# google/libultrahdr

Measured on AMD Instinct MI355X. Metric: Mpixels/s encode+decode (API-1 P010+YUV420, 4K), device-resident round trip, higher is better.
Workload: dtype f32; 1 GPU; API-1 3840x2160 round trip per step: encode (P010 HLG + YCbCr420 -> two-pass 3-ch gain map at scale 1, FDCT q95, Huffman: two JPEG scans) + decode (Huffman, IDCT, applyGainMap -> RGBA_F16 linear); frames resident in HBM

## Files before the change

libultrahdr_amd/csrc/api_context.cpp:

```cpp
#include "api_internal.h"

#include <sys/mman.h>
#include <mutex>
#include <algorithm>

namespace uhdr_api {
uhdr_error_info_t ensure(DeviceBuf& b, size_t bytes) {
  if (b.cap >= bytes) return ok_status();
  if (b.p) (void)hipFree(b.p);
  b.p = nullptr;
  b.cap = 0;
  size_t want = bytes + (bytes >> 3) + 256;
  HIP_TRY(hipMalloc(&b.p, want));
  b.cap = want;
  return ok_status();
}


size_t bytes_per_sample(int fmt) {
  switch (fmt) {
    case UHDR_IMG_FMT_24bppYCbCrP010:
    case UHDR_IMG_FMT_30bppYCbCr444: return 2;
    case UHDR_IMG_FMT_24bppRGB888: return 3;
    case UHDR_IMG_FMT_32bppRGBA8888:
// ... 440 lines not shown
         fmt == UHDR_IMG_FMT_32bppRGBA1010102;
}

uhdr_error_info_t validate_apply(const uhdr_raw_image_t* sdr, const uhdr_raw_image_t* gm,
                                 const uhdr_gainmap_metadata_t* md, uhdr_color_transfer_t out_ct,
                                 const uhdr_raw_image_t* dest) {
  if (dest == nullptr || dest->planes[UHDR_PLANE_PACKED] == nullptr)
    return err_status(UHDR_CODEC_INVALID_PARAM, "apply gainmap method received nullptr for destination image or plane pointer");
  if (dest->stride[UHDR_PLANE_PACKED] < dest->w)
    return err_status(UHDR_CODEC_INVALID_PARAM, "destination stride (%u) cannot be less than image width (%u)",
                      dest->stride[UHDR_PLANE_PACKED], dest->w);
  if (out_ct != UHDR_CT_LINEAR && out_ct != UHDR_CT_HLG && out_ct != UHDR_CT_PQ)
    return err_status(UHDR_CODEC_INVALID_PARAM,
                      "apply gainmap method expects output color transfer to be one of {UHDR_CT_LINEAR, UHDR_CT_HLG, UHDR_CT_PQ}. Received %d", out_ct);
  if ((out_ct == UHDR_CT_LINEAR && dest->fmt != UHDR_IMG_FMT_64bppRGBAHalfFloat) ||
      ((out_ct == UHDR_CT_HLG || out_ct == UHDR_CT_PQ) && dest->fmt != UHDR_IMG_FMT_32bppRGBA1010102))
    return err_status(UHDR_CODEC_INVALID_PARAM, "unsupported destination pixel format %d for output color transfer %d", dest->fmt, out_ct);
  UHDR_TRY(validate_metadata(md));
  if (!sdr || !gm) return err_status(UHDR_CODEC_INVALID_PARAM, "received nullptr for base image or gainmap image");
  if (sdr->fmt != UHDR_IMG_FMT_24bppYCbCr444 && sdr->fmt != UHDR_IMG_FMT_16bppYCbCr422 &&
      sdr->fmt != UHDR_IMG_FMT_12bppYCbCr420 && sdr->fmt != UHDR_IMG_FMT_24bppRGB888 &&
      sdr->fmt != UHDR_IMG_FMT_32bppRGBA8888)
    return err_status(UHDR_CODEC_UNSUPPORTED_FEATURE, "apply gainmap method expects base image color format to be one of "
                      "{UHDR_IMG_FMT_24bppYCbCr444, UHDR_IMG_FMT_16bppYCbCr422, UHDR_IMG_FMT_12bppYCbCr420, "
                      "UHDR_IMG_FMT_24bppRGB888, UHDR_IMG_FMT_32bppRGBA8888}. Received %d", sdr->fmt);
  if (gm->fmt != UHDR_IMG_FMT_8bppYCbCr400 && gm->fmt != UHDR_IMG_FMT_24bppRGB888 && gm->fmt != UHDR_IMG_FMT_32bppRGBA8888)
    return err_status(UHDR_CODEC_UNSUPPORTED_FEATURE, "apply gainmap method expects gainmap image color format to be one of "
                      "{UHDR_IMG_FMT_8bppYCbCr400, UHDR_IMG_FMT_24bppRGB888, UHDR_IMG_FMT_32bppRGBA8888}. Received %d", gm->fmt);
  return ok_status();
}

uhdr_error_info_t get_apply_tables(uhdr_hip_ctx* c, const uhdr_gainmap_metadata_t& md, float weight,
                                   int idw_scale, const float** d_out) {
  std::string key((const char*)&md, sizeof md);
  key.append((const char*)&weight, sizeof weight);
  key.append((const char*)&idw_scale, sizeof idw_scale);
  for (int i = 0; i < kTableSlots; i++)
    if (c->tab_cap[i] && c->tab_key[i] == key) { *d_out = c->d_tab[i]; return ok_status(); }
  const int slot = c->tab_next;
  c->tab_next = (c->tab_next + 1) % kTableSlots;
  std::vector<float> t;
  host::build_apply_tables(md, weight, idw_scale, &t);
  const size_t bytes = t.size() * sizeof(float);
  if (c->tab_cap[slot]) HIP_TRY(hipEventSynchronize(c->tab_ev[slot]));
  if (c->tab_cap[slot] < bytes) {
    HIP_TRY(hipStreamSynchronize(c->stream));
    if (c->h_tab[slot]) (void)hipHostFree(c->h_tab[slot]);
    if (c->d_tab[slot]) (void)hipFree(c->d_tab[slot]);
    c->h_tab[slot] = nullptr; c->d_tab[slot] = nullptr; c->tab_cap[slot] = 0;
    HIP_TRY(hipHostMalloc((void**)&c->h_tab[slot], bytes, hipHostMallocDefault));
    HIP_TRY(hipMalloc((void**)&c->d_tab[slot], bytes));
    if (!c->tab_ev[slot]) HIP_TRY(hipEventCreateWithFlags(&c->tab_ev[slot], hipEventDisableTiming));
    c->tab_cap[slot] = bytes;
  }
  memcpy(c->h_tab[slot], t.data(), bytes);
  HIP_TRY(hipMemcpyAsync(c->d_tab[slot], c->h_tab[slot], bytes, hipMemcpyHostToDevice, c->stream));
  HIP_TRY(hipEventRecord(c->tab_ev[slot], c->stream));
  c->tab_key[slot] = key;
  *d_out = c->d_tab[slot];
  return ok_status();
}
}


const char* uhdr_hip_version(void) { return "libuhdr_hip 0.3 (gfx950; reference libultrahdr 2.0.2 hot path)"; }

int uhdr_hip_device_count(void) {
  int n = 0;
  if (hipGetDeviceCount(&n) != hipSuccess) return 0;
  return n;
}

int uhdr_hip_current_device(void) {
  int d = -1;
  if (hipGetDevice(&d) != hipSuccess) return -1;
  return d;
}

uhdr_hip_ctx_t* uhdr_hip_create(int device, uhdr_error_info_t* err) {
  auto fail = [&](const char* what, hipError_t e) -> uhdr_hip_ctx_t* {
    if (err) *err = err_status(UHDR_CODEC_ERROR, "uhdr_hip_create: %s failed: %s (no CPU fallback exists behind this library)",
                               what, hipGetErrorString(e));
    return nullptr;
  };
  if (err) *err = ok_status();
  int n = 0;
  hipError_t e = hipGetDeviceCount(&n);
  if (e != hipSuccess || n == 0) return fail("hipGetDeviceCount", e == hipSuccess ? hipErrorNoDevice : e);
  if (device < 0) {
    e = hipGetDevice(&device);
    if (e != hipSuccess) return fail("hipGetDevice", e);
  }
  if (device >= n) return fail("device index", hipErrorInvalidDevice);
  e = hipSetDevice(device);
  if (e != hipSuccess) return fail("hipSetDevice", e);
  uhdr_hip_ctx* c = new uhdr_hip_ctx();
  c->device = device;
  {
    const char* e = getenv("UHDR_HIP_HUFF_TWO_PASS");
    c->huff_two_pass = e && atoi(e) != 0;
    e = getenv("UHDR_HIP_HUFF_ROUTE_LOG");
    c->huff_route_log = e && atoi(e) != 0;
  }
  e = hipStreamCreateWithFlags(&c->own_stream, hipStreamNonBlocking);
  if (e != hipSuccess) { delete c; return fail("hipStreamCreate", e); }
  c->stream = c->own_stream;
  uhdr_error_info_t st = upload_lut(&c->d_srgb, host::srgb_inv_oetf_lut(), c->stream);
  if (st.error_code != UHDR_CODEC_OK) {
    if (err) *err = st;
    (void)hipStreamDestroy(c->own_stream);
    delete c;
    return nullptr;
  }
  return c;
}

void uhdr_hip_destroy(uhdr_hip_ctx_t* c) {
  if (!c) return;
  (void)hipSetDevice(c->device);
  (void)hipStreamSynchronize(c->stream);
  for (auto& e : c->prof_entries) { (void)hipEventDestroy(e.a); (void)hipEventDestroy(e.b); }
  float* luts[] = {c->d_srgb, c->d_hlg_inv, c->d_pq_inv, c->d_hlg_oetf, c->d_pq_oetf, c->d_hlg_inv_ootf, (float*)c->d_math,
                   c->d_hlg_buckets, c->d_pq_buckets, c->d_hlg_buckets_pre, c->d_pq_buckets_pre};
  for (float* p : luts) if (p) (void)hipFree(p);
  for (int i = 0; i < kTableSlots; i++) {
    if (c->h_tab[i]) (void)hipHostFree(c->h_tab[i]);
    if (c->d_tab[i]) (void)hipFree(c->d_tab[i]);
    if (c->tab_ev[i]) (void)hipEventDestroy(c->tab_ev[i]);
  }
  for (auto& b : c->scratch) if (b.p) (void)hipFree(b.p);
  for (auto& b : c->jpg) if (b.p) (void)hipFree(b.p);
  for (auto& b : c->enc) if (b.p) (void)hipFree(b.p);
  if (c->huff_slots.p) (void)hipFree(c->huff_slots.p);
  for (auto& r : c->resident) if (r.buf.p) (void)hipFree(r.buf.p);
  if (c->pending.buf.p) (void)hipFree(c->pending.buf.p);
  if (c->pending.tmp.p) (void)hipFree(c->pending.tmp.p);
  if (c->minmax.p) (void)hipFree(c->minmax.p);
  if (c->d_coef_src) (void)hipFree(c->d_coef_src);
  if (c->d_huff) (void)hipFree(c->d_huff);
  if (c->d_srgb8) (void)hipFree(c->d_srgb8);
  for (float* q : c->d_lin10) if (q) (void)hipFree(q);
  for (auto& g : c->gain_tabs) if (g.d) (void)hipFree(g.d);
  uhdr_hip_comm_destroy(c);
  aux_worker_destroy(c);
  if (c->aux) uhdr_hip_destroy(c->aux);
  if (c->exchange.p) (void)hipFree(c->exchange.p);
  if (c->affine.p) (void)hipFree(c->affine.p);
  if (c->d_srgb_of_byte) (void)hipFree(c->d_srgb_of_byte);
  if (c->h_mm) (void)hipHostFree(c->h_mm);
  if (c->aux_ev) (void)hipEventDestroy(c->aux_ev);
  if (c->aux_ev2) (void)hipEventDestroy(c->aux_ev2);
  if (c->md_ev) (void)hipEventDestroy(c->md_ev);
  if (c->md_stream) (void)hipStreamDestroy(c->md_stream);
  if (c->h_flags) (void)hipHostFree(c->h_flags);
  if (c->pin.p) (void)hipHostFree(c->pin.p);
  if (c->pin.ev) (void)hipEventDestroy(c->pin.ev);
  if (c->huff_tabs.dev.p) (void)hipFree(c->huff_tabs.dev.p);
  if (c->own_stream) (void)hipStreamDestroy(c->own_stream);
  delete c;
}

int uhdr_hip_recycle(uhdr_hip_ctx_t* c, size_t keep_bytes) {
  if (!c) return -1;
  (void)hipSetDevice(c->device);
  (void)hipStreamSynchronize(c->stream);
  uhdr_hip_resident_forget(c);
  uhdr_hip_resident_begin(c);
  uhdr_hip_resident_end(c);
  c->sticky = ok_status();
  for (auto& h : c->huff_hint) h = uhdr_hip_ctx::HuffHint();
  c->stats = uhdr_hip_stats_t();
  c->deferred_md.valid = false;
  c->huff_slots_refused = 0;
  std::vector<DeviceBuf*> bufs;
  for (auto& b : c->scratch) bufs.push_back(&b);
  for (auto& b : c->jpg) bufs.push_back(&b);
  for (auto& b : c->enc) bufs.push_back(&b);
  bufs.push_back(&c->huff_slots);
  for (auto& r : c->resident) bufs.push_back(&r.buf);
  bufs.push_back(&c->pending.buf);
  bufs.push_back(&c->pending.tmp);
  size_t total = c->pin.cap;
  for (DeviceBuf* b : bufs) total += b->p ? b->cap : 0;
  std::sort(bufs.begin(), bufs.end(), [](const DeviceBuf* a, const DeviceBuf* b) { return (a->p ? a->cap : 0) > (b->p ? b->cap : 0); });
  for (DeviceBuf* b : bufs) {
    if (total <= keep_bytes) break;
    if (!b->p) continue;
    (void)hipFree(b->p);
    total -= b->cap;
    b->p = nullptr;
    b->cap = 0;
  }
  if (total > keep_bytes && c->pin.p) {
    if (c->pin.ev_pending && c->pin.ev) (void)hipEventSynchronize(c->pin.ev);
    (void)hipHostFree(c->pin.p);
    c->pin.p = nullptr;
    c->pin.cap = c->pin.off = 0;
    c->pin.ev_pending = false;
  }
  if (c->aux) (void)uhdr_hip_recycle(c->aux, keep_bytes);
  return c->device;
}

uhdr_error_info_t uhdr_hip_set_stream(uhdr_hip_ctx_t* c, void* hip_stream) {
  if (!c) return err_status(UHDR_CODEC_INVALID_PARAM, "received nullptr for uhdr_hip context");
  HIP_TRY(hipStreamSynchronize(c->stream));
  c->stream = hip_stream ? (hipStream_t)hip_stream : c->own_stream;
  return ok_status();
}

void* uhdr_hip_get_stream(uhdr_hip_ctx_t* c) { return c ? (void*)c->stream : nullptr; }

uhdr_error_info_t uhdr_hip_synchronize(uhdr_hip_ctx_t* c) {
  if (!c) return err_status(UHDR_CODEC_INVALID_PARAM, "received nullptr for uhdr_hip context");
  HIP_TRY(hipStreamSynchronize(c->stream));
  return ok_status();
}

void uhdr_hip_get_stats(uhdr_hip_ctx_t* c, uhdr_hip_stats_t* out) {
  if (!out) return;
  if (!c) { memset(out, 0, sizeof *out); return; }
  *out = c->stats;
}

namespace {
std::mutex g_seam_mu;
std::vector<uhdr_hip_seam_stage_t> g_seam_rows;
unsigned long long g_seam_seq = 0;
void seam_dump_at_exit() {
  const char* path = getenv("UHDR_HIP_SEAM_STATS_FILE");
  FILE* f = path ? fopen(path, "w") : nullptr;
  if (!f) return;
  std::lock_guard<std::mutex> lk(g_seam_mu);
  fprintf(f, "{");
  for (size_t i = 0; i < g_seam_rows.size(); i++) {
    const auto& r = g_seam_rows[i];
    fprintf(f, "%s\"%s\": {\"device\": %llu, \"reference\": %llu, \"device_ms\": %.3f, \"first_seq\": %llu}", i ? ", " : "", r.name, r.device_calls,
            r.reference_calls, r.device_ms, r.first_seq);
  }
  fprintf(f, "}\n");
  fclose(f);
}
}

void uhdr_hip_seam_note(const char* stage, int on_device, double ms) {
  if (!stage) return;
  static const bool dump = [] { return getenv("UHDR_HIP_SEAM_STATS_FILE") ? (atexit(seam_dump_at_exit), true) : false; }();
  (void)dump;
  std::lock_guard<std::mutex> lk(g_seam_mu);
  uhdr_hip_seam_stage_t* row = nullptr;
  for (auto& r : g_seam_rows)
    if (!strncmp(r.name, stage, sizeof r.name - 1)) { row = &r; break; }
  if (!row) {
    if (g_seam_rows.size() >= 64) return;
    uhdr_hip_seam_stage_t r;
    memset(&r, 0, sizeof r);
    strncpy(r.name, stage, sizeof r.name - 1);
    r.first_seq = g_seam_seq;
    g_seam_rows.push_back(r);
    row = &g_seam_rows.back();
  }
  g_seam_seq++;
  if (on_device) { row->device_calls++; row->device_ms += ms; }
  else row->reference_calls++;
  row->last_ms = ms;
}

int uhdr_hip_seam_stats(uhdr_hip_seam_stage_t* out, int capacity) {
  std::lock_guard<std::mutex> lk(g_seam_mu);
  const int n = (int)g_seam_rows.size();
  for (int i = 0; out && i < n && i < capacity; i++) out[i] = g_seam_rows[i];
  return n;
}

void uhdr_hip_seam_stats_reset(void) {
  std::lock_guard<std::mutex> lk(g_seam_mu);
  g_seam_rows.clear();
  g_seam_seq = 0;
}

void uhdr_hip_profile_enable(uhdr_hip_ctx_t* c, int enable) {
  if (c) c->prof = enable != 0;
}

int uhdr_hip_profile_read(uhdr_hip_ctx_t* c, const char* family, double* total_ms, int reset) {
  if (!c) return 0;
  (void)hipStreamSynchronize(c->stream);
  int n = 0;
  double tot = 0.0;
  std::vector<ProfEntry> keep;
  for (auto& e : c->prof_entries) {
    const bool match = !family || e.family == family;
    if (match) {
      float ms = 0.0f;
      if (hipEventElapsedTime(&ms, e.a, e.b) == hipSuccess) { tot += ms; n++; }
    }
    if (match && reset) { (void)hipEventDestroy(e.a); (void)hipEventDestroy(e.b); }
    else keep.push_back(e);
  }
  if (reset) c->prof_entries.swap(keep);
  if (total_ms) *total_ms = tot;
  return n;
}

void uhdr_hip_profile_mark(uhdr_hip_ctx_t* c) {
  if (!c) return;
// ... 101 lines not shown
```

libultrahdr_amd/csrc/api_entropy.cpp:

```cpp
#include "api_internal.h"

#include <condition_variable>
#include <functional>
#include <mutex>

uhdr_error_info_t uhdr_api::check_scan(const uhdr_hip_jpeg_scan_t* sc, bool need_coef, int* mcus_per_row, int* mcu_rows, int* blocks_per_mcu) {
  if (!sc) return err_status(UHDR_CODEC_INVALID_PARAM, "received nullptr for the scan description");
  if (sc->num_components != 1 && sc->num_components != 3)
    return err_status(UHDR_CODEC_INVALID_PARAM, "a scan has 1 or 3 components, received %d", sc->num_components);
  if (sc->w == 0 || sc->h == 0 || sc->w > 65535 || sc->h > 65535)
    return err_status(UHDR_CODEC_INVALID_PARAM, "image dimensions %ux%u are outside JPEG's 1..65535", sc->w, sc->h);
  int hmax = 1, vmax = 1, bpm = 0;
  for (int i = 0; i < sc->num_components; i++) {
    const int hs = sc->num_components == 1 ? 1 : sc->h_samp[i], vs = sc->num_components == 1 ? 1 : sc->v_samp[i];
    if (hs < 1 || hs > 2 || vs < 1 || vs > 2) return err_status(UHDR_CODEC_INVALID_PARAM, "component %d: sampling factors %dx%d not in {1, 2}", i, hs, vs);
    if (hs > hmax) hmax = hs;
    if (vs > vmax) vmax = vs;
    bpm += hs * vs;
    if (need_coef && (!sc->coef[i] || ((uintptr_t)sc->coef[i] & 15)))
      return err_status(UHDR_CODEC_INVALID_PARAM, "coefficient buffer %d is null or not 16-byte aligned", i);
    if (sc->blocks_w[i] < 1 || sc->blocks_h[i] < 1) return err_status(UHDR_CODEC_INVALID_PARAM, "component %d: empty block grid", i);
  }
  if (sc->num_components == 1) {
    *mcus_per_row = sc->blocks_w[0];
    *mcu_rows = sc->blocks_h[0];
    if ((unsigned)sc->blocks_w[0] != (sc->w + 7) / 8 || (unsigned)sc->blocks_h[0] != (sc->h + 7) / 8)
      return err_status(UHDR_CODEC_INVALID_PARAM, "a %dx%d block grid does not match a %ux%u image", sc->blocks_w[0], sc->blocks_h[0], sc->w, sc->h);
  } else {
    *mcus_per_row = (int)((sc->w + 8u * hmax - 1) / (8u * hmax));
    *mcu_rows = (int)((sc->h + 8u * vmax - 1) / (8u * vmax));
    for (int i = 0; i < 3; i++) {
      const unsigned cw = (sc->w * sc->h_samp[i] + hmax - 1) / hmax, chh = (sc->h * sc->v_samp[i] + vmax - 1) / vmax;
      const int min_w = (int)((cw + 7) / 8), min_h = (int)((chh + 7) / 8);
      if (sc->blocks_w[i] < min_w || sc->blocks_w[i] > *mcus_per_row * sc->h_samp[i] || sc->blocks_h[i] < min_h ||
          sc->blocks_h[i] > *mcu_rows * sc->v_samp[i])
        return err_status(UHDR_CODEC_INVALID_PARAM, "component %d: a %dx%d block grid does not match a %ux%u image at %dx%d sampling", i,
                          sc->blocks_w[i], sc->blocks_h[i], sc->w, sc->h, sc->h_samp[i], sc->v_samp[i]);
    }
  }
  *blocks_per_mcu = bpm;
  return ok_status();
}

static hipError_t wait_stream(uhdr_hip_ctx* c) {
  static const int spin_us = [] { const char* e = getenv("UHDR_HIP_SYNC_SPIN_US"); return e ? atoi(e) : 2000; }();
  if (spin_us > 0) {
    const auto t0 = std::chrono::steady_clock::now();
    for (;;) {
      const hipError_t q = hipStreamQuery(c->stream);
      if (q == hipSuccess) return hipSuccess;
      if (q != hipErrorNotReady) return q;
      if (std::chrono::steady_clock::now() - t0 > std::chrono::microseconds(spin_us)) break;
    }
  }
  return hipStreamSynchronize(c->stream);
}


uhdr_error_info_t uhdr_hip_huffman_encode_dev(uhdr_hip_ctx_t* c, const uhdr_hip_jpeg_scan_t* sc, uint8_t* out, size_t out_capacity,
                                              size_t* out_bytes) {
  if (!c) return err_status(UHDR_CODEC_INVALID_PARAM, "received nullptr for uhdr_hip context");
  if (!out || !out_bytes) return err_status(UHDR_CODEC_INVALID_PARAM, "received nullptr for the output buffer or size");
  int mpr = 0, mrows = 0, bpm = 0;
  UHDR_TRY(check_scan(sc, true, &mpr, &mrows, &bpm));
  const bool stream = sc->restart_interval == 0;
  if (!stream && (sc->restart_interval < 1 || sc->restart_interval > 65535 || sc->restart_interval * bpm > 64))
    return err_status(UHDR_CODEC_UNSUPPORTED_FEATURE, "restart_interval must be 0 (no markers) or in 1..%d for %d blocks per MCU (one wavefront "
                      "encodes one restart interval of at most 64 blocks); received %d", 64 / bpm, bpm, sc->restart_interval);
  if (stream && 2 * bpm > 64) return err_status(UHDR_CODEC_UNSUPPORTED_FEATURE, "%d blocks per MCU: outside the HIP path", bpm);
  HIP_TRY(hipSetDevice(c->device));
  if (!c->d_huff) {
    std::vector<uint32_t> blob(host::jpeg_huff_code_tables());
    blob.resize((size_t)host::kHuffTabWords + 16);
    memcpy(blob.data() + host::kHuffTabWords, host::jpeg_zigzag_to_natural(), 64);
    HIP_TRY(hipMalloc((void**)&c->d_huff, blob.size() * sizeof(uint32_t)));
    HIP_TRY(hipMemcpyAsync(c->d_huff, blob.data(), blob.size() * sizeof(uint32_t), hipMemcpyHostToDevice, c->stream));
    HIP_TRY(hipStreamSynchronize(c->stream));
  }
  HuffArgs a;
  memset(&a, 0, sizeof a);
  a.ncomp = sc->num_components;
  for (int i = 0; i < a.ncomp; i++) {
    a.coef[i] = sc->coef[i];
    a.bw[i] = sc->blocks_w[i]; a.bh[i] = sc->blocks_h[i];
    a.hs[i] = a.ncomp == 1 ? 1 : sc->h_samp[i]; a.vs[i] = a.ncomp == 1 ? 1 : sc->v_samp[i];
  }
  a.mcus_per_row = mpr;
  a.total_mcus = mpr * mrows;
  a.ri = stream ? huff_stream_segment_mcus(bpm) : sc->restart_interval;
  a.blocks_per_mcu = bpm;
  a.nseg = (a.total_mcus + a.ri - 1) / a.ri;
  a.tables = c->d_huff;
  a.zigzag = (const uint8_t*)(c->d_huff + host::kHuffTabWords);
  if (stream) {
    if (out_capacity > 0xFFFFFFF0u) out_capacity = 0xFFFFFFF0u;
    HuffStream t;
    memset(&t, 0, sizeof t);
    t.raw_words = ((uint64_t)out_capacity + 3) / 4 + 1;
    const uint64_t worst_words = (uint64_t)a.total_mcus * bpm * 52 + 2;
    if (t.raw_words > worst_words) t.raw_words = worst_words;
    const int nchunks = huff_stuff_chunks(t.raw_words * 4u);
    UHDR_TRY(ensure(c->scratch[4], (size_t)t.raw_words * 4));
    UHDR_TRY(ensure(c->scratch[5], ((size_t)a.nseg + 2) * sizeof(uint64_t) + (4 + (size_t)a.nseg + (size_t)nchunks) * sizeof(uint32_t)));
    t.raw = (uint32_t*)c->scratch[4].p;
    t.seg_start = (uint64_t*)c->scratch[5].p;
    uint64_t* d_total = t.seg_start + (size_t)a.nseg + 1;
    t.meta = (uint32_t*)(d_total + 1);
    t.seg_bits = t.meta + 4;
    uint32_t* chunk_counts = t.seg_bits + a.nseg;
    if (!c->huff_two_pass) {
      const size_t need = huff_stream_slot_bytes(a.nseg);
      if (c->huff_slots.cap >= need || !c->huff_slots_refused || need < c->huff_slots_refused) {
        if (ensure(c->huff_slots, need).error_code == UHDR_CODEC_OK) {
          t.slots = (uint32_t*)c->huff_slots.p;
        } else {
          (void)hipGetLastError();
          c->huff_slots_refused = need;
          fprintf(stderr, "uhdr_hip: no device memory for %zu bytes of Huffman segment slots: marker-less scans of that size take the two-pass route\n", need);
        }
      }
    }
    if (c->huff_route_log) fprintf(stderr, "uhdr_hip: huffman_encode stream route=%s nseg=%d\n", t.slots ? "one_walk" : "two_pass", a.nseg);
    {
      ProfScope ps(c, "huffman_encode");
      HIP_TRY(launch_huffman_encode_stream(a, t, chunk_counts, d_total, out, (uint64_t)out_capacity, c->stream));
    }
    c->stats.entropy_encode_stream++;
    if (!c->h_flags) HIP_TRY(hipHostMalloc((void**)&c->h_flags, 64 * sizeof(uint32_t), hipHostMallocDefault));
    uint32_t* hp = c->h_flags + 48;
    HIP_TRY(hipMemcpyAsync(hp, d_total, sizeof(uint64_t) + 4 * sizeof(uint32_t), hipMemcpyDeviceToHost, c->stream));
    HIP_TRY(wait_stream(c));
    uint64_t total = 0;
    uint32_t meta[4] = {0, 0, 0, 0};
    memcpy(&total, hp, sizeof total);
    memcpy(meta, hp + 2, sizeof meta);
    if (meta[2]) return err_status(UHDR_CODEC_INVALID_PARAM, "coefficients outside the baseline range (DC difference beyond 11 bits / AC beyond 10 bits)");
    const uint64_t raw_bytes = ((((uint64_t)meta[1] << 32) | meta[0]) + 7) / 8;
    if (raw_bytes > t.raw_words * 4u) total = raw_bytes + raw_bytes / 64 + 64;
    *out_bytes = (size_t)total;
    if (total > out_capacity)
      return err_status(UHDR_CODEC_MEM_ERROR, "entropy-coded data needs %llu bytes, the output buffer holds %zu", (unsigned long long)total, out_capacity);
    return ok_status();
  }
  a.slot_stride = huff_slot_stride();
  UHDR_TRY(ensure(c->scratch[4], (size_t)a.nseg * a.slot_stride));
  const size_t meta = (size_t)a.nseg * sizeof(uint32_t) + 16 + ((size_t)a.nseg + 1) * sizeof(uint64_t) + 16;
  UHDR_TRY(ensure(c->scratch[5], meta));
  a.slots = (uint8_t*)c->scratch[4].p;
  uint64_t* offsets = (uint64_t*)c->scratch[5].p;
  uint32_t* status = (uint32_t*)(offsets + (size_t)a.nseg + 1);
  a.seg_bytes = status + 2;
  {
    ProfScope ps(c, "huffman_encode");
    HIP_TRY(launch_huffman_encode(a, offsets, status, out, (uint64_t)out_capacity, c->stream));
  }
  c->stats.entropy_encode_intervals++;
  uint64_t total = 0;
  uint32_t bad = 0;
  HIP_TRY(hipMemcpyAsync(&total, offsets + a.nseg, sizeof total, hipMemcpyDeviceToHost, c->stream));
  HIP_TRY(hipMemcpyAsync(&bad, status, sizeof bad, hipMemcpyDeviceToHost, c->stream));
  HIP_TRY(wait_stream(c));
  if (bad) return err_status(UHDR_CODEC_INVALID_PARAM, "coefficients outside the baseline range (DC difference beyond 11 bits / AC beyond 10 bits)");
  *out_bytes = (size_t)total;
  if (total > out_capacity)
    return err_status(UHDR_CODEC_MEM_ERROR, "entropy-coded data needs %llu bytes, the output buffer holds %zu", (unsigned long long)total, out_capacity);
  return ok_status();
}

static bool make_dec_table(const uint8_t bits[17], const uint8_t vals[256], HuffDecTable* t) {
  memset(t, 0, sizeof *t);
  int nsym = 0;
  for (int l = 1; l <= 16; l++) nsym += bits[l];
  if (nsym > 256) return false;
  int code = 0, k = 0;
  for (int l = 1; l <= 16; l++) {
    if (bits[l]) {
      t->valoff[l] = k - code;
      for (int i = 0; i < bits[l]; i++, k++, code++) {
        if (code >= (1 << l)) return false;
        if (l <= 9) {
          const int lo = code << (9 - l);
          for (int x = 0; x < (1 << (9 - l)); x++) t->lut[lo + x] = (uint16_t)((l << 8) | vals[k]);
        }
      }
      t->maxcode[l] = code - 1;
    } else {
      t->maxcode[l] = -1;
    }
    code <<= 1;
  }
  t->maxcode[17] = 0x7fffffff;
  memcpy(t->vals, vals, 256);
  return true;
}

static bool make_fast_table(const uint8_t bits[17], const uint8_t vals[256], HuffFastTable* t, int* nsub_out = nullptr) {
  memset(t, 0, sizeof *t);
  int code = 0, k = 0, nsub = 0;
  int sub_of[512];
  for (int i = 0; i < 512; i++) sub_of[i] = -1;
  for (int l = 1; l <= 16; l++) {
    for (int i = 0; i < bits[l]; i++, k++, code++) {
      if (code >= (1 << l) || k >= 256) return false;
      if (l <= 9) {
        const int lo = code << (9 - l);
        for (int x = 0; x < (1 << (9 - l)); x++) t->l1[lo + x] = (uint16_t)((l << 8) | vals[k]);
      } else {
        const int prefix = code >> (l - 9);
// ... 1 lines not shown
          if (nsub >= kHuffL2Max) return false;
          sub_of[prefix] = nsub++;
          t->l1[prefix] = (uint16_t)(0x8000u | (unsigned)sub_of[prefix]);
        }
        const int rest = (code << (16 - l)) & 127;
        for (int x = 0; x < (1 << (16 - l)); x++) t->l2[sub_of[prefix]][rest + x] = (uint16_t)((l << 8) | vals[k]);
      }
    }
    code <<= 1;
  }
  if (nsub_out) *nsub_out = nsub;
  return true;
}

static void make_track_table(const HuffFastTable& f, bool is_dc, HuffFastTable* t) {
  auto conv = [&](uint16_t e) -> uint16_t {
    if (e & 0x8000u) return e;
    unsigned adv, kinc;
    if (e == 0) {
      adv = 16;
      kinc = is_dc ? 1 : 64;
    } else {
      const unsigned len = (e >> 8) & 31u, rs = e & 255u;
      if (is_dc) {
        const unsigned sz = rs > 15u ? 0u : rs;
        adv = len + sz;
        kinc = 1;
      } else {
        const unsigned sz = rs & 15u, run = rs >> 4;
        adv = len + sz;
        kinc = sz ? run + 1 : (run == 15u ? 16u : 64u);
      }
    }
    return (uint16_t)(adv | (kinc << 5));
  };
  for (int i = 0; i < 512; i++) t->l1[i] = conv(f.l1[i]);
  for (int s = 0; s < kHuffL2Max; s++)
    for (int i = 0; i < 128; i++) t->l2[s][i] = conv(f.l2[s][i]);
}

static void make_value_table(const HuffFastTable& f, bool is_dc, uint32_t* out ) {
  auto conv = [&](uint16_t e, bool first_level) -> uint32_t {
    if (first_level && (e & 0x8000u)) return 0x80000000u | (e & 31u);
    unsigned adv, kinc, sz = 0, bad = 0;
    if (e == 0) {
      adv = 16;
      kinc = is_dc ? 1 : 64;
      bad = 1;
    } else {
      const unsigned len = (e >> 8) & 31u, rs = e & 255u;
      if (is_dc) {
        if (rs > 15u) bad = 1; else sz = rs;
        adv = len + sz;
        kinc = 1;
      } else {
        sz = rs & 15u;
        const unsigned run = rs >> 4;
        adv = len + sz;
        kinc = sz ? run + 1 : (run == 15u ? 16u : 64u);
      }
    }
    return adv | (kinc << 5) | (sz << 12) | (bad << 16);
  };
  for (int i = 0; i < 512; i++) out[i] = conv(f.l1[i], true);
  for (int s = 0; s < kHuffL2Max; s++)
    for (int i = 0; i < 128; i++) out[512 + s * 128 + i] = conv(f.l2[s][i], false);
}

static void make_pair_table(const HuffFastTable& f, const HuffFastTable& t, const HuffFastTable& f_ac, const HuffFastTable& t_ac, int l2_base, uint32_t* out ) {
  constexpr int B = kHuffPairBits;
  for (int idx = 0; idx < kHuffPairWords; idx++) {
    const int p9 = idx >> (B - 9);
    const uint16_t e = f.l1[p9];
    uint32_t first;
    bool defined;
    if (e & 0x8000u) {
      const int sub = e & 31, rest = (idx & ((1 << (B - 9)) - 1)) << (16 - B);
      const uint16_t e2 = f.l2[sub][rest];
      if (e2 == 0 || (int)((e2 >> 8) & 31u) > B) {
        out[idx] = 0x80000000u | (uint32_t)(l2_base + sub);
        continue;
      }
      first = t.l2[sub][rest];
      defined = true;
    } else {
      first = t.l1[p9];
      defined = e != 0;
    }
    uint32_t word = first & 0xfffu;
    const int adv1 = (int)(first & 31u), kinc1 = (int)((first >> 5) & 127u);
    if (defined && kinc1 < 64 && adv1 < B) {
      const int r = B - adv1;
      const int next9 = ((idx << adv1) & (kHuffPairWords - 1)) >> (B - 9);
      const uint16_t n = f_ac.l1[next9];
      if (n != 0 && !(n & 0x8000u) && (int)((n >> 8) & 31u) <= r) {
        const uint32_t second = t_ac.l1[next9];
        word |= (second & 31u) << 12 | ((second >> 5) & 127u) << 17;
      }
    }
    out[idx] = word;
  }
}

static void make_pair_value_table(const HuffFastTable& f, const uint32_t* v, const HuffFastTable& f_ac, const uint32_t* v_ac, int l2_base, uint32_t* out ) {
  constexpr int B = kHuffPairBits;
  for (int idx = 0; idx < kHuffPairWords; idx++) {
    const int p9 = idx >> (B - 9);
    const uint16_t e = f.l1[p9];
    uint32_t first;
    bool defined;
    if (e & 0x8000u) {
      const int sub = e & 31, rest = (idx & ((1 << (B - 9)) - 1)) << (16 - B);
      const uint16_t e2 = f.l2[sub][rest];
      if (e2 == 0 || (int)((e2 >> 8) & 31u) > B) {
        out[2 * idx] = 0x80000000u | (uint32_t)(l2_base + sub);
        out[2 * idx + 1] = 0;
        continue;
      }
      first = v[512 + sub * 128 + rest];
      defined = true;
    } else {
      first = v[p9];
      defined = e != 0;
    }
    uint32_t second = 0;
    const int adv1 = (int)(first & 31u), kinc1 = (int)((first >> 5) & 127u);
    if (defined && !((first >> 16) & 1u) && kinc1 < 64 && adv1 < B) {
      const int r = B - adv1;
      const int next9 = ((idx << adv1) & (kHuffPairWords - 1)) >> (B - 9);
      const uint16_t n = f_ac.l1[next9];
      if (n != 0 && !(n & 0x8000u) && (int)((n >> 8) & 31u) <= r) second = v_ac[next9];
    }
    out[2 * idx] = first;
    out[2 * idx + 1] = second;
  }
}

uhdr_error_info_t uhdr_hip_huffman_decode_dev(uhdr_hip_ctx_t* c, const uhdr_hip_jpeg_scan_t* sc, const uhdr_hip_huff_tables_t* tables,
                                              const uint8_t* data, size_t data_bytes) {
  if (!c) return err_status(UHDR_CODEC_INVALID_PARAM, "received nullptr for uhdr_hip context");
  if (!data || data_bytes == 0 || data_bytes > 0xFFFFFFF0ull) return err_status(UHDR_CODEC_INVALID_PARAM, "received no (or more than 4 GiB of) entropy-coded data");
  int mpr = 0, mrows = 0, bpm = 0;
  UHDR_TRY(check_scan(sc, true, &mpr, &mrows, &bpm));
  if (sc->restart_interval < 0 || sc->restart_interval > 65535) return err_status(UHDR_CODEC_INVALID_PARAM, "restart_interval %d out of range", sc->restart_interval);
  HIP_TRY(hipSetDevice(c->device));
  if (!c->d_huff) {
    std::vector<uint32_t> blob(host::jpeg_huff_code_tables());
    blob.resize((size_t)host::kHuffTabWords + 16);
    memcpy(blob.data() + host::kHuffTabWords, host::jpeg_zigzag_to_natural(), 64);
    HIP_TRY(hipMalloc((void**)&c->d_huff, blob.size() * sizeof(uint32_t)));
    HIP_TRY(hipMemcpyAsync(c->d_huff, blob.data(), blob.size() * sizeof(uint32_t), hipMemcpyHostToDevice, c->stream));
    HIP_TRY(hipStreamSynchronize(c->stream));
  }
  const DbgClock dbg;
  constexpr size_t kTabDec = 0, kTabFast = (sizeof(HuffDecTable) * 4 + 255) & ~(size_t)255,
                   kTabVal = (kTabFast + sizeof(HuffFastTable) * 8 + 255) & ~(size_t)255, kTabPair = kTabVal + (size_t)4 * kHuffValWords * 4,
                   kTabPairVal = kTabPair + (size_t)kHuffPairBlobWords * 4, kTabBytes = kTabPairVal + (size_t)kHuffPairValBlobWords * 4;
  {
    uint8_t key[4 * (17 + 256)];
    for (int t = 0; t < 4; t++) {
      uint8_t* bits = key + (size_t)t * (17 + 256);
      uint8_t* vals = bits + 17;
      if (tables) {
        memcpy(bits, tables->bits[t], 17);
        memcpy(vals, tables->vals[t], 256);
      } else {
        memset(bits, 0, 17 + 256);
        host::jpeg_std_huff_table(t & 1, t >> 1, bits, vals);
      }
    }
    uhdr_hip_ctx::HuffTabCache& hc = c->huff_tabs;
    if (!hc.valid || memcmp(hc.key, key, sizeof key) != 0) {
      hc.valid = false;
      std::vector<HuffDecTable> tabs(4);
      std::vector<HuffFastTable> ftabs(8);
      std::vector<uint32_t> vtabs((size_t)4 * kHuffValWords), ptabs((size_t)kHuffPairBlobWords), pvtabs((size_t)kHuffPairValBlobWords);
      bool fast_ok = true;
      int l2_count[4] = {0, 0, 0, 0};
      for (int t = 0; t < 4; t++) {
        const uint8_t* bits = key + (size_t)t * (17 + 256);
        if (!make_dec_table(bits, bits + 17, &tabs[(size_t)t])) return err_status(UHDR_CODEC_INVALID_PARAM, "Huffman table %d is not a valid DHT table", t);
        fast_ok = make_fast_table(bits, bits + 17, &ftabs[(size_t)t], &l2_count[t]) && fast_ok;
      }
      int l2_base[4] = {0, 0, 0, 0};
      for (int t = 1; t < 4; t++) l2_base[t] = l2_base[t - 1] + l2_count[t - 1];
      if (l2_base[3] + l2_count[3] > kHuffL2Total) fast_ok = false;
      if (fast_ok)
        for (int t = 0; t < 4; t++) {
          make_track_table(ftabs[(size_t)t], (t & 1) == 0, &ftabs[(size_t)t + 4]);
          make_value_table(ftabs[(size_t)t], (t & 1) == 0, vtabs.data() + (size_t)t * kHuffValWords);
        }
      if (fast_ok)
        for (int t = 0; t < 4; t++)
        {
          make_pair_table(ftabs[(size_t)t], ftabs[(size_t)t + 4], ftabs[(size_t)(t | 1)], ftabs[(size_t)(t | 1) + 4], l2_base[t], ptabs.data() + (size_t)t * kHuffPairWords);
          make_pair_value_table(ftabs[(size_t)t], vtabs.data() + (size_t)t * kHuffValWords, ftabs[(size_t)(t | 1)], vtabs.data() + (size_t)(t | 1) * kHuffValWords,
                                l2_base[t], pvtabs.data() + (size_t)t * 2 * kHuffPairWords);
          uint16_t* l2t = (uint16_t*)(ptabs.data() + (size_t)4 * kHuffPairWords) + (size_t)l2_base[t] * 128;
          uint16_t* l2v = (uint16_t*)(pvtabs.data() + (size_t)8 * kHuffPairWords) + (size_t)l2_base[t] * 128;
          for (int i = 0; i < l2_count[t] * 128; i++) {
            l2t[i] = ftabs[(size_t)t + 4].l2[i / 128][i % 128];
            const uint32_t v = vtabs[(size_t)t * kHuffValWords + 512 + (size_t)i];
            l2v[i] = (uint16_t)(((v >> 16) & 1u) ? 0u : (v & 0xffffu));
          }
        }
      UHDR_TRY(ensure(hc.dev, kTabBytes));
      HIP_TRY(hipStreamSynchronize(c->stream));
      HIP_TRY(hipMemcpy((uint8_t*)hc.dev.p + kTabDec, tabs.data(), sizeof(HuffDecTable) * 4, hipMemcpyHostToDevice));
      HIP_TRY(hipMemcpy((uint8_t*)hc.dev.p + kTabFast, ftabs.data(), sizeof(HuffFastTable) * 8, hipMemcpyHostToDevice));
      HIP_TRY(hipMemcpy((uint8_t*)hc.dev.p + kTabVal, vtabs.data(), vtabs.size() * 4, hipMemcpyHostToDevice));
      HIP_TRY(hipMemcpy((uint8_t*)hc.dev.p + kTabPair, ptabs.data(), ptabs.size() * 4, hipMemcpyHostToDevice));
      HIP_TRY(hipMemcpy((uint8_t*)hc.dev.p + kTabPairVal, pvtabs.data(), pvtabs.size() * 4, hipMemcpyHostToDevice));
      memcpy(hc.key, key, sizeof key);
      hc.fast_ok = fast_ok;
      hc.valid = true;
    }
  }
  const bool fast_ok = c->huff_tabs.fast_ok;
  const uint8_t* tabs_dev = (const uint8_t*)c->huff_tabs.dev.p;
  if (!c->h_flags) HIP_TRY(hipHostMalloc((void**)&c->h_flags, 64 * sizeof(uint32_t), hipHostMallocDefault));
  HuffDecArgs a;
  memset(&a, 0, sizeof a);
  a.ncomp = sc->num_components;
  size_t zero_bytes[3] = {0, 0, 0};
  for (int i = 0; i < a.ncomp; i++) {
    a.coef[i] = const_cast<int16_t*>(sc->coef[i]);
    a.bw[i] = sc->blocks_w[i]; a.bh[i] = sc->blocks_h[i];
    a.hs[i] = a.ncomp == 1 ? 1 : sc->h_samp[i]; a.vs[i] = a.ncomp == 1 ? 1 : sc->v_samp[i];
    zero_bytes[i] = (size_t)a.bw[i] * a.bh[i] * 64 * sizeof(int16_t);
  }
  a.mcus_per_row = mpr;
  a.total_mcus = mpr * mrows;
  a.ri = sc->restart_interval;
  a.nseg = a.ri > 0 ? (a.total_mcus + a.ri - 1) / a.ri : 1;
  a.data = data;
  a.nbytes = (uint32_t)data_bytes;
  a.zigzag = (const uint8_t*)(c->d_huff + host::kHuffTabWords);
  const int nchunks = huff_marker_chunks(data_bytes);
  const size_t need = 16 + ((size_t)nchunks + 2 * (size_t)a.nseg) * sizeof(uint32_t);
  UHDR_TRY(ensure(c->scratch[5], need));
  uint8_t* base = (uint8_t*)c->scratch[5].p;
  a.tabs = (const HuffDecTable*)(tabs_dev + kTabDec);
  a.status = (uint32_t*)base;
  uint32_t* counts = a.status + 4;
  uint32_t* starts = counts + nchunks;
  uint32_t* ends = starts + a.nseg;
  a.starts = starts;
  a.ends = ends;
  dbg.mark("huffman_decode_dev: tables ready");
  const bool rst_sync = a.nseg > 1 && data_bytes / (size_t)a.nseg >= 320 && !getenv("UHDR_HIP_HUFF_RST_INTERVALS");
  const bool try_sync = (a.nseg == 1 || rst_sync) && data_bytes >= 4096 && data_bytes < ((size_t)1 << 29) && fast_ok && !getenv("UHDR_HIP_HUFF_SERIAL") && bpm <= 16;
  const int write_form = [] { const char* e = getenv("UHDR_HIP_HUFF_WRITE"); return e ? atoi(e) : 2; }();
  const bool form2 = try_sync && !rst_sync && write_form != 1;
  bool coef_zeroed = !form2;
  if (!form2)
    for (int i = 0; i < a.ncomp; i++) HIP_TRY(hipMemsetAsync(a.coef[i], 0, zero_bytes[i], c->stream));
  bool sync_done = false;
  if (try_sync) {
    struct Attempt { uint32_t sub_bits; int levels; };
    std::vector<Attempt> attempts;
    bool sparse = false;
    {
      const char* eb = getenv("UHDR_HIP_HUFF_SUB_BITS");
      const char* el = getenv("UHDR_HIP_HUFF_LEVELS");
      const int vb = eb ? atoi(eb) : 0;
      const bool vb_ok = vb >= 256 && vb <= 4096 && (vb & (vb - 1)) == 0;
      if (vb_ok || el) {
        const uint32_t sbits = vb_ok ? (uint32_t)vb : 1024u;
        const int lv = el ? atoi(el) : (sbits <= 512 ? 7 : 4);
        if (lv >= 1 && lv <= 15 && bpm * (lv + 1) <= kHuffHypSlots) attempts.push_back({sbits, lv});
        attempts.push_back({sbits, 0});
      } else {
        const uint64_t bits_per_block = (uint64_t)data_bytes * 8u / (uint64_t)((uint64_t)a.total_mcus * (uint64_t)bpm);
        const int lv_fit = kHuffHypSlots / bpm - 1;
        const int lv = lv_fit >= 15 ? 15 : (lv_fit >= 11 ? 11 : (lv_fit >= 7 ? 7 : (lv_fit >= 4 ? 4 : 0)));
        sparse = bits_per_block < 64;
        uint32_t first = bits_per_block < 64 ? 1024u : (bits_per_block < 200 ? 512u : (bits_per_block < 400 ? 2048u : 4096u));
        const uhdr_hip_ctx::HuffHint& hint = c->huff_hint[bpm & 15];
        if (hint.sub_bits > first && bits_per_block * 4 >= hint.bits_per_block * 3 && bits_per_block * 4 <= hint.bits_per_block * 5) first = hint.sub_bits;
        if (lv > 0)
          for (uint32_t sbits = first; sbits <= 4096u; sbits <<= 1) attempts.push_back({sbits, lv});
        attempts.push_back({1024u, 0});
      }
    }
    uint32_t sub_bits = attempts[0].sub_bits;
    bool use_hyp = false;
    for (const Attempt& t : attempts) { if (t.sub_bits < sub_bits) sub_bits = t.sub_bits; use_hyp = use_hyp || t.levels > 0; }
    const int max_rounds = 40;
    const int nch = huff_sync_chunks(data_bytes);
    const uint32_t nsub = huff_sync_max_subsequences(data_bytes, sub_bits);
    const uint32_t total_blocks = (uint32_t)a.total_mcus * (uint32_t)bpm;
    size_t off = 0;
    auto take = [&](size_t bytes) { const size_t o = off; off += (bytes + 255) & ~(size_t)255; return o; };
    const size_t rst_words = data_bytes / 32 + 2;
    const size_t o_clean = take(data_bytes + 16), o_cnt = take((size_t)nch * 4);
    const size_t o_flags = take(128), o_nblk = take((size_t)nsub * 4 + 4), o_dcd = take((size_t)total_blocks * 4), o_rm = rst_sync ? take(rst_words * 4) : 0;
    const size_t zero_bytes_sync = off - o_flags;
    const size_t o_s0 = take((size_t)nsub * 8), o_hm = use_hyp ? take((size_t)nsub * kHuffHypSlots) : 0;
    const size_t ff_bytes = off - o_s0;
    const size_t o_s1 = take((size_t)nsub * 8), o_c0 = take(nsub), o_c1 = take(nsub), o_dcp = take((size_t)((total_blocks + 255) / 256) * 12 + 16),
                 o_ft = take(sizeof(HuffFastTable) * 8),
                 o_st = take(((size_t)nsub / 2048 + 2) * 4), o_vt = take((size_t)4 * kHuffValWords * 4);
    const size_t o_hs = use_hyp ? take((size_t)nsub * kHuffHypSlots * 8) : 0, o_hc = use_hyp ? take((size_t)nsub * kHuffHypSlots * 2) : 0;
    size_t chain_tiles_off = 0;
    const size_t o_ch = use_hyp ? take(huff_hyp_chain_bytes(data_bytes, sub_bits, &chain_tiles_off)) : 0;
    (void)chain_tiles_off;
    const size_t o_ds = rst_sync ? take((size_t)a.nseg * 12) : 0, o_rp = rst_sync ? take((size_t)nch * 12) : 0;
    const size_t o_sl = use_hyp ? take((size_t)nsub * (size_t)bpm * 8) : 0;
    const int max_pieces = [&] {
      const char* e = getenv("UHDR_HIP_HUFF_PIECES");
      const int v = e ? atoi(e) : 4;
      return (use_hyp && form2 && !rst_sync && v >= 1 && v <= 4) ? v : 1;
    }();
    const size_t o_ms = max_pieces > 1 ? take((size_t)nsub * kHuffHypSlots * (size_t)(max_pieces - 1) * 8) : 0;
    const size_t o_mc = max_pieces > 1 ? take((size_t)nsub * kHuffHypSlots * (size_t)(max_pieces - 1) * 2) : 0;
    const size_t o_pe = max_pieces > 1 ? take((size_t)nsub * (size_t)max_pieces * 8 + 64) : 0;
    const size_t o_pc = max_pieces > 1 ? take(((size_t)nsub * (size_t)max_pieces + 4) * 4) : 0;
    const size_t o_st2 = max_pieces > 1 ? take(((size_t)nsub * (size_t)max_pieces / 2048 + 4) * 4) : 0;
    const size_t scan_bytes = form2 ? (size_t)total_blocks * 64 * sizeof(int16_t) : 0;
    const size_t o_cs = form2 ? take(scan_bytes + 256) : 0;
    UHDR_TRY(ensure(c->scratch[6], off));
    uint8_t* sb = (uint8_t*)c->scratch[6].p;
    HuffSyncArgs y;
    memset(&y, 0, sizeof y);
    y.clean = sb + o_clean;
    y.nbytes = (uint32_t)data_bytes;
    y.flags = (uint32_t*)(sb + o_flags);
    y.nstuffed = y.flags + 8;
    y.sub_bits = sub_bits;
    y.state[0] = (uint64_t*)(sb + o_s0); y.state[1] = (uint64_t*)(sb + o_s1);
    y.changed[0] = sb + o_c0; y.changed[1] = sb + o_c1;
    y.nblk = (uint32_t*)(sb + o_nblk);
    y.scan_tmp = (uint32_t*)(sb + o_st);
    y.dcd = (int*)(sb + o_dcd);
    y.total_blocks = total_blocks;
    y.blocks_per_mcu = bpm; y.ncomp = a.ncomp; y.mcus_per_row = a.mcus_per_row;
    uint32_t* rst_map = nullptr;
    if (rst_sync) {
      rst_map = (uint32_t*)(sb + o_rm);
      y.rst_map = rst_map;
      y.rst_blocks = (uint32_t)a.ri * (uint32_t)bpm;
      y.dc_seg = (int*)(sb + o_ds);
      y.rst_partial = (uint32_t*)(sb + o_rp);
      y.rst_chunks = (uint32_t)nch;
    }
    int j = 0;
    for (int i = 0; i < a.ncomp; i++) {
      y.bw[i] = a.bw[i]; y.bh[i] = a.bh[i]; y.hs[i] = a.hs[i]; y.vs[i] = a.vs[i]; y.coef[i] = a.coef[i];
      y.first_blk[i] = j;
      for (int k = 0; k < a.hs[i] * a.vs[i] && j < 16; k++) y.comp_of[j++] = (uint8_t)i;
    }
    y.ftabs = (const HuffFastTable*)(tabs_dev + kTabFast);
    y.ttabs = y.ftabs + 4;
    y.vtabs = (const uint32_t*)(tabs_dev + kTabVal);
    y.ptabs = (const uint32_t*)(tabs_dev + kTabPair);
    y.pvtabs = (const uint32_t*)(tabs_dev + kTabPairVal);
    y.zigzag = a.zigzag;
    (void)o_ft; (void)o_vt;
    if (use_hyp) {
      y.strag_list = (uint32_t*)(sb + o_sl);
      y.strag_cap = nsub * (uint32_t)bpm;
    }
    if (form2) y.coef_scan = (int16_t*)(sb + o_cs);
    const int main_levels_env = [&] { const char* e = getenv("UHDR_HIP_HUFF_MAIN_LEVELS"); return e ? atoi(e) : (sparse ? 1 : 2); }();
    if (j == bpm && bpm <= 16) {
      const bool fills_in_unstuff = attempts[0].levels > 0 && zero_bytes_sync % 16 == 0 && ff_bytes % 16 == 0 && zero_bytes_sync / 16 < 0xFFFFFFFFull &&
                                    ff_bytes / 16 < 0xFFFFFFFFull && !getenv("UHDR_HIP_HUFF_FILL_LAUNCHES");
      HuffInitFill init_fill;
      memset(&init_fill, 0, sizeof init_fill);
      if (fills_in_unstuff) {
        init_fill.zero_ptr = (uint4*)y.flags;
        init_fill.zero_vec = (uint32_t)(zero_bytes_sync / 16);
        init_fill.ff_ptr = (uint4*)y.state[0];
        init_fill.ff_vec = (uint32_t)(ff_bytes / 16);
      } else {
        HIP_TRY(hipMemsetAsync(y.flags, 0, zero_bytes_sync, c->stream));
      }
      auto pass0_zeroes = [&](const Attempt& t) { return form2 && t.levels > 0 && scan_bytes % 16 == 0 && scan_bytes / 16 < 0xFFFFFFFFull; };
      if (form2 && !pass0_zeroes(attempts[0])) HIP_TRY(hipMemsetAsync(y.coef_scan, 0, scan_bytes, c->stream));
      dbg.mark("huffman_decode_dev: fills enqueued");
      int final_buf = 0;
      uint32_t* fl = c->h_flags;
      for (int q = 0; q < 24; q++) fl[q] = 0;
      bool hyp_done = false, unstuffed = false, rounds_ran = false;
      auto start_over = [&](const Attempt& next) -> uhdr_error_info_t {
        HIP_TRY(hipMemsetAsync(y.flags, 0, 32, c->stream));
        HIP_TRY(hipMemsetAsync(y.flags + kHuffFlagStragglers, 0, 4, c->stream));
        HIP_TRY(hipMemsetAsync(y.nblk, 0, (size_t)nsub * 4 + 4, c->stream));
        if (form2) {
          if (!pass0_zeroes(next)) HIP_TRY(hipMemsetAsync(y.coef_scan, 0, scan_bytes, c->stream));
        } else {
          HIP_TRY(hipMemsetAsync(y.dcd, 0, (size_t)total_blocks * 4, c->stream));
          for (int i = 0; i < a.ncomp; i++) HIP_TRY(hipMemsetAsync(a.coef[i], 0, zero_bytes[i], c->stream));
        }
        return ok_status();
      };
      for (size_t ti = 0; ti < attempts.size() && !hyp_done && !rounds_ran; ti++) {
        const Attempt& t = attempts[ti];
        if (ti > 0) UHDR_TRY(start_over(t));
        y.sub_bits = t.sub_bits;
        y.zero_ptr = pass0_zeroes(t) ? (uint4*)y.coef_scan : nullptr;
        y.zero_vec = pass0_zeroes(t) ? (uint32_t)(scan_bytes / 16) : 0u;
        const uint32_t nsub_t = huff_sync_max_subsequences(data_bytes, t.sub_bits);
        if (t.levels > 0) {
          y.hyp_h = bpm;
          y.hyp_levels = t.levels;
          y.hyp_main_levels = rst_sync ? 0 : main_levels_env;
          y.strag_levels = [&] { const char* e = getenv("UHDR_HIP_HUFF_STRAG_LEVELS"); return e ? atoi(e) : t.levels; }();
          y.hyp_state = (uint64_t*)(sb + o_hs);
          y.hyp_map = sb + o_hm;
          y.hyp_cnt = (uint16_t*)(sb + o_hc);
          y.hyp_hist = getenv("UHDR_HIP_HUFF_DEBUG") ? 1 : 0;
          {
            int q = t.sub_bits >= 1024u ? (int)(t.sub_bits / 256u) : 1;
            if (getenv("UHDR_HIP_HUFF_PIECES_ALL")) q = (int)(t.sub_bits / 256u);
            if (q > max_pieces) q = max_pieces;
            if (q < 1) q = 1;
            while (q > 1 && (t.sub_bits % (uint32_t)q || (t.sub_bits / (uint32_t)q) % 32u)) q--;
            if (q == 3) q = 2;
            if (getenv("UHDR_HIP_HUFF_QMERGE") && atoi(getenv("UHDR_HIP_HUFF_QMERGE")) == 0) q = 1;
            y.pieces = q;
            y.mid_state = q > 1 ? (uint64_t*)(sb + o_ms) : nullptr;
            y.mid_cnt = q > 1 ? (uint16_t*)(sb + o_mc) : nullptr;
            y.pend = q > 1 ? (uint64_t*)(sb + o_pe) : nullptr;
            y.pcnt = q > 1 ? (uint32_t*)(sb + o_pc) : nullptr;
            y.scan_tmp = q > 1 ? (uint32_t*)(sb + o_st2) : (uint32_t*)(sb + o_st);
          }
          if (!(fills_in_unstuff && ti == 0)) HIP_TRY(hipMemsetAsync(y.state[0], 0xff, ff_bytes, c->stream));
          size_t tiles_off = 0;
          (void)huff_hyp_chain_bytes(data_bytes, t.sub_bits, &tiles_off);
          {
            ProfScope ps(c, "huffman_decode");
            if (!unstuffed)
              HIP_TRY(launch_huffman_unstuff(data, (uint32_t)data_bytes, (uint32_t*)(sb + o_cnt), y.flags + 8, sb + o_clean, c->stream, rst_map, y.rst_partial,
                                             fills_in_unstuff && ti == 0 ? &init_fill : nullptr));
            unstuffed = true;
            HIP_TRY(launch_huffman_decode_hyp(y, (int*)(sb + o_dcp), sb + o_ch, sb + o_ch + tiles_off, c->stream));
          }
          dbg.mark("huffman_decode_dev: hypothesis attempt enqueued");
          HIP_TRY(hipMemcpyAsync(fl, y.flags, 24 * sizeof(uint32_t), hipMemcpyDeviceToHost, c->stream));
          HIP_TRY(wait_stream(c));
          dbg.mark("huffman_decode_dev: hypothesis attempt finished");
          hyp_done = fl[2] == 0;
          if (hyp_done && ti > 0) {
            uhdr_hip_ctx::HuffHint& hint = c->huff_hint[bpm & 15];
            hint.sub_bits = t.sub_bits;
            hint.bits_per_block = (uint32_t)((uint64_t)data_bytes * 8u / ((uint64_t)a.total_mcus * (uint64_t)bpm));
          }
          if (getenv("UHDR_HIP_HUFF_DEBUG")) {
            uint32_t hist[32] = {};
            (void)hipMemcpy(hist, y.flags, sizeof hist, hipMemcpyDeviceToHost);
            fprintf(stderr, "uhdr_hip: hypothesis decode of %zu bytes, %u subsequences of %u bits x %d: merges per level %u %u %u %u %u %u+, %u paths unmerged after %d levels (%d in lockstep, %u paths handed to the straggler waves), true path %s\n",
                    data_bytes, nsub_t, t.sub_bits, bpm, hist[10], hist[11], hist[12], hist[13], hist[14], hist[15], fl[3], t.levels, y.hyp_main_levels, fl[kHuffFlagStragglers], hyp_done ? "resolved" : "LOST (next attempt)");
            fprintf(stderr, "uhdr_hip: the stragglers' merges at level 2 .. 10, 11+: %u %u %u %u %u %u %u %u %u %u\n", hist[22], hist[23], hist[24], hist[25], hist[26], hist[27], hist[28], hist[29],
                    hist[30], hist[31]);
          }
        } else {
          y.pieces = 1;
          y.scan_tmp = (uint32_t*)(sb + o_st);
          {
            ProfScope ps(c, "huffman_decode");
            if (!unstuffed) HIP_TRY(launch_huffman_unstuff(data, (uint32_t)data_bytes, (uint32_t*)(sb + o_cnt), y.flags + 8, sb + o_clean, c->stream, rst_map, y.rst_partial));
            unstuffed = true;
            HIP_TRY(launch_huffman_decode_sync(y, max_rounds, (int*)(sb + o_dcp), &final_buf, c->stream));
          }
          HIP_TRY(hipMemcpyAsync(fl, y.flags, 24 * sizeof(uint32_t), hipMemcpyDeviceToHost, c->stream));
          HIP_TRY(wait_stream(c));
          rounds_ran = true;
        }
      }
      const bool settled = hyp_done || fl[4 + max_rounds % 3] == 0;
      if (rst_sync && getenv("UHDR_HIP_HUFF_DEBUG"))
        fprintf(stderr, "uhdr_hip: restart file through the parallel decoder: %s, status bits %#x, %u markers dropped (%d expected), sequence sums %s\n",
                settled ? "settled" : "NOT settled", fl[1], fl[9], a.nseg - 1, fl[0] == fl[16] && fl[7] == fl[17] ? "equal" : "DIFFERENT");
      if (settled && rst_sync && ((fl[1] & 14u) != 0 || fl[9] != (uint32_t)(a.nseg - 1) || fl[0] != fl[16] || fl[7] != fl[17])) {
        for (int i = 0; i < a.ncomp; i++) HIP_TRY(hipMemsetAsync(a.coef[i], 0, zero_bytes[i], c->stream));
        coef_zeroed = true;
      } else if (settled) {
        if (fl[1] & 8u) return err_status(UHDR_CODEC_INVALID_PARAM, "corrupt entropy-coded data (the scan ends before its last block)");
        if (fl[1] & 2u) return err_status(UHDR_CODEC_INVALID_PARAM, "corrupt entropy-coded data (undefined Huffman code or a run past the end of a block)");
        sync_done = true;
      } else {
        if (a.nseg == 1 && !c->huff_serial_ok && data_bytes > (256u << 10)) {
          c->stats.entropy_decode_declined++;
          return err_status(UHDR_CODEC_UNSUPPORTED_FEATURE, "the parallel entropy decode did not settle in %d rounds; %zu bytes on one lane would take longer than the CPU", max_rounds, data_bytes);
        }
        for (int i = 0; i < a.ncomp; i++) HIP_TRY(hipMemsetAsync(a.coef[i], 0, zero_bytes[i], c->stream));
        coef_zeroed = true;
      }
    }
  }
  if (sync_done) {
    c->stats.entropy_decode_parallel++;
    return ok_status();
  }
  if (a.nseg == 1 && !c->huff_serial_ok && data_bytes > (256u << 10)) {
    c->stats.entropy_decode_declined++;
    return err_status(UHDR_CODEC_UNSUPPORTED_FEATURE, "a %zu-byte scan without restart markers that the parallel decoder does not take (Huffman tables outside its two-level form)", data_bytes);
  }
  if (!coef_zeroed)
    for (int i = 0; i < a.ncomp; i++) HIP_TRY(hipMemsetAsync(a.coef[i], 0, zero_bytes[i], c->stream));
  HIP_TRY(hipMemsetAsync(a.status, 0, 16, c->stream));
  {
    ProfScope ps(c, "huffman_decode");
    HIP_TRY(launch_huffman_decode(a, counts, starts, ends, c->stream));
  }
  if (a.nseg == 1) c->stats.entropy_decode_single_lane++;
  else c->stats.entropy_decode_intervals++;
  uint32_t st[2] = {0, 0};
  HIP_TRY(hipMemcpyAsync(st, a.status, sizeof st, hipMemcpyDeviceToHost, c->stream));
  HIP_TRY(wait_stream(c));
  if (st[1] != (uint32_t)(a.nseg - 1))
    return err_status(UHDR_CODEC_INVALID_PARAM, "found %u restart markers, a restart interval of %d MCUs over %d MCUs needs %d", st[1], a.ri,
                      a.total_mcus, a.nseg - 1);
  if (st[0] & 4u) return err_status(UHDR_CODEC_INVALID_PARAM, "restart markers out of sequence");
  if (st[0] & 2u) return err_status(UHDR_CODEC_INVALID_PARAM, "corrupt entropy-coded data (undefined Huffman code or a run past the end of a block)");
  return ok_status();
}

uhdr_error_info_t uhdr_api::aux_context(uhdr_hip_ctx* c, uhdr_hip_ctx** out) {
  if (!c->aux) {
    uhdr_error_info_t e = ok_status();
    c->aux = uhdr_hip_create(c->device, &e);
    if (!c->aux) return e.error_code != UHDR_CODEC_OK ? e : err_status(UHDR_CODEC_ERROR, "could not create the auxiliary context");
  }
  c->aux->prof = c->prof;
  c->aux->huff_serial_ok = c->huff_serial_ok;
  c->aux->huff_route_log = c->huff_route_log;
  c->aux->huff_two_pass = c->huff_two_pass;
  *out = c->aux;
  return ok_status();
}
void uhdr_api::aux_merge(uhdr_hip_ctx* c) {
  if (!c->aux) return;
  uhdr_hip_ctx* x = c->aux;
  c->stats.entropy_decode_parallel += x->stats.entropy_decode_parallel;
  c->stats.entropy_decode_intervals += x->stats.entropy_decode_intervals;
  c->stats.entropy_decode_single_lane += x->stats.entropy_decode_single_lane;
  c->stats.entropy_decode_declined += x->stats.entropy_decode_declined;
  c->stats.entropy_encode_stream += x->stats.entropy_encode_stream;
  c->stats.entropy_encode_intervals += x->stats.entropy_encode_intervals;
  x->stats = uhdr_hip_stats_t();
  for (auto& e : x->prof_entries) c->prof_entries.push_back(e);
  x->prof_entries.clear();
}

struct AuxWorker {
  static constexpr int kSpinUs = 300;
  std::thread th;
  std::mutex mu;
  std::condition_variable cv;
  std::function<void()> job;
  std::atomic<int> state{0};
  std::atomic<bool> busy{false};
  static bool spin_until(const std::function<bool()>& pred, int us) {
    const auto t0 = std::chrono::steady_clock::now();
    while (!pred()) {
      if (std::chrono::steady_clock::now() - t0 > std::chrono::microseconds(us)) return pred();
#if defined(__x86_64__)
      __builtin_ia32_pause();
#endif
    }
    return true;
  }
  AuxWorker() {
    th = std::thread([this] {
      for (;;) {
        if (!spin_until([this] { return state.load(std::memory_order_acquire) != 0; }, kSpinUs)) {
          std::unique_lock<std::mutex> lk(mu);
          cv.wait(lk, [this] { return state.load(std::memory_order_acquire) != 0; });
        }
        if (state.load(std::memory_order_acquire) == 2) return;
        std::function<void()> j;
        {
          std::lock_guard<std::mutex> lk(mu);
          j = std::move(job);
          state.store(0, std::memory_order_release);
        }
        j();
        {
          std::lock_guard<std::mutex> lk(mu);
          busy.store(false, std::memory_order_release);
        }
        cv.notify_all();
      }
    });
  }
  void run(std::function<void()> j) {
    {
      std::lock_guard<std::mutex> lk(mu);
      job = std::move(j);
      busy.store(true, std::memory_order_release);
      state.store(1, std::memory_order_release);
    }
    cv.notify_all();
  }
  void wait() {
    if (spin_until([this] { return !busy.load(std::memory_order_acquire); }, kSpinUs)) return;
    std::unique_lock<std::mutex> lk(mu);
    cv.wait(lk, [this] { return !busy.load(std::memory_order_acquire); });
  }
  ~AuxWorker() {
    {
      std::lock_guard<std::mutex> lk(mu);
      state.store(2, std::memory_order_release);
    }
    cv.notify_all();
    if (th.joinable()) th.join();
  }
};
void aux_worker_destroy(uhdr_hip_ctx* c) {
  if (c && c->aux_worker) {
    delete c->aux_worker;
    c->aux_worker = nullptr;
  }
}
bool uhdr_api::aux_post(uhdr_hip_ctx* c, std::function<void()> job) {
  static const bool no_thread = getenv("UHDR_HIP_NO_AUX_THREAD") != nullptr;
  if (no_thread) return false;
  if (!c->aux_worker) {
    try {
      c->aux_worker = new AuxWorker();
    } catch (...) {
      c->aux_worker = nullptr;
    }
  }
  if (!c->aux_worker) return false;
  c->aux_worker->run(std::move(job));
  return true;
}
void uhdr_api::aux_wait(uhdr_hip_ctx* c) {
  if (c->aux_worker) c->aux_worker->wait();
}
namespace {
template <typename FA, typename FB>
void run_pair(uhdr_hip_ctx* c, FA&& job_a, FB&& job_b) {
  static const bool no_thread = getenv("UHDR_HIP_NO_AUX_THREAD") != nullptr;
  if (!c->aux_worker && !no_thread) {
    try {
      c->aux_worker = new AuxWorker();
    } catch (...) {
      c->aux_worker = nullptr;
    }
  }
  if (c->aux_worker) {
    c->aux_worker->run(job_b);
    job_a();
    c->aux_worker->wait();
  } else {
    job_a();
    job_b();
  }
}
}

uhdr_error_info_t uhdr_hip_huffman_encode2_dev(uhdr_hip_ctx_t* c, const uhdr_hip_jpeg_scan_t* scan_a, uint8_t* out_a, size_t cap_a, size_t* bytes_a,
                                               const uhdr_hip_jpeg_scan_t* scan_b, uint8_t* out_b, size_t cap_b, size_t* bytes_b) {
  if (!c) return err_status(UHDR_CODEC_INVALID_PARAM, "received nullptr for uhdr_hip context");
  HIP_TRY(hipSetDevice(c->device));
  uhdr_hip_ctx* x = nullptr;
  UHDR_TRY(aux_context(c, &x));
  if (!c->aux_ev) HIP_TRY(hipEventCreateWithFlags(&c->aux_ev, hipEventDisableTiming));
  HIP_TRY(hipEventRecord(c->aux_ev, c->stream));
  HIP_TRY(hipStreamWaitEvent(x->stream, c->aux_ev, 0));
  uhdr_error_info_t ra = ok_status(), rb = ok_status();
  const int dev = c->device;
  run_pair(c, [&] { ra = uhdr_hip_huffman_encode_dev(c, scan_a, out_a, cap_a, bytes_a); },
           [&, dev] { (void)hipSetDevice(dev); rb = uhdr_hip_huffman_encode_dev(x, scan_b, out_b, cap_b, bytes_b); });
  aux_merge(c);
  return ra.error_code != UHDR_CODEC_OK ? ra : rb;
}

uhdr_error_info_t uhdr_hip_huffman_decode2_dev(uhdr_hip_ctx_t* c, const uhdr_hip_jpeg_scan_t* scan_a, const uhdr_hip_huff_tables_t* tables_a, const uint8_t* data_a,
                                               size_t bytes_a, const uhdr_hip_jpeg_scan_t* scan_b, const uhdr_hip_huff_tables_t* tables_b,
                                               const uint8_t* data_b, size_t bytes_b) {
  if (!c) return err_status(UHDR_CODEC_INVALID_PARAM, "received nullptr for uhdr_hip context");
  HIP_TRY(hipSetDevice(c->device));
  uhdr_hip_ctx* x = nullptr;
  UHDR_TRY(aux_context(c, &x));
  if (!c->aux_ev) HIP_TRY(hipEventCreateWithFlags(&c->aux_ev, hipEventDisableTiming));
  HIP_TRY(hipEventRecord(c->aux_ev, c->stream));
  HIP_TRY(hipStreamWaitEvent(x->stream, c->aux_ev, 0));
// ... 8 lines not shown
```

libultrahdr_amd/csrc/api_internal.h:

```cpp
#ifndef UHDR_HIP_API_INTERNAL_H
#define UHDR_HIP_API_INTERNAL_H

#pragma GCC visibility push(default)
#include "uhdr_hip.h"
#pragma GCC visibility pop

#include <cfloat>
#include <chrono>
#include <cmath>
#include <cstdarg>
#include <cstdio>
#include <cstring>
#include <atomic>
#include <functional>
#include <map>
#include <memory>
#include <string>
#include <thread>
#include <vector>
#include "exact_math.h"
#include "host_tables.h"
#include "uhdr_types.h"
#include "rccl_bind.h"

using namespace uhdr;

inline uhdr_error_info_t ok_status() {
  uhdr_error_info_t s;
  s.error_code = UHDR_CODEC_OK;
  s.has_detail = 0;
  s.detail[0] = 0;
  return s;
}
inline uhdr_error_info_t err_status(uhdr_codec_err_t code, const char* fmt, ...) {
  uhdr_error_info_t s;
  s.error_code = code;
  s.has_detail = 1;
  va_list ap;
  va_start(ap, fmt);
  vsnprintf(s.detail, sizeof s.detail, fmt, ap);
  va_end(ap);
  return s;
}
#define HIP_TRY(expr)                                                                      \
  do {                                                                                     \
    hipError_t e_ = (expr);                                                                \
    if (e_ != hipSuccess)                                                                  \
      return err_status(e_ == hipErrorOutOfMemory ? UHDR_CODEC_MEM_ERROR : UHDR_CODEC_ERROR, \
                        "HIP error '%s' at %s:%d", hipGetErrorString(e_), __FILE__, __LINE__); \
  } while (0)
#define UHDR_TRY(expr)                                 \
  do {                                                 \
    uhdr_error_info_t s_ = (expr);                     \
    if (s_.error_code != UHDR_CODEC_OK) return s_;     \
  } while (0)

struct DbgClock {
  bool on;
  std::chrono::steady_clock::time_point t0;
  DbgClock() : on(getenv("UHDR_HIP_CLOCK_DEBUG") != nullptr), t0(std::chrono::steady_clock::now()) {}
  void mark(const char* what) const {
    if (on) fprintf(stderr, "uhdr_hip:   [%7.1f us] %s\n", std::chrono::duration<double, std::micro>(std::chrono::steady_clock::now() - t0).count(), what);
  }
};

struct ProfEntry {
  hipEvent_t a, b;
  std::string family;
};

constexpr int kTableSlots = 4;

struct DeviceBuf {
  void* p = nullptr;
  size_t cap = 0;
};

struct uhdr_hip_ctx {
  int device = 0;
  hipStream_t own_stream = nullptr;
  hipStream_t stream = nullptr;
  float* d_srgb = nullptr;
  float* d_hlg_inv = nullptr;
  float* d_pq_inv = nullptr;
  float* d_hlg_oetf = nullptr;
  float* d_pq_oetf = nullptr;
  float* d_hlg_buckets = nullptr;
  float* d_pq_buckets = nullptr;
  float* d_hlg_buckets_pre = nullptr;
  float* d_pq_buckets_pre = nullptr;
  float* d_hlg_inv_ootf = nullptr;
  double* d_math = nullptr;
  float* h_tab[kTableSlots] = {};
  float* d_tab[kTableSlots] = {};
  size_t tab_cap[kTableSlots] = {};
  hipEvent_t tab_ev[kTableSlots] = {};
  std::string tab_key[kTableSlots];
  int tab_next = 0;
  DeviceBuf scratch[8];
  uhdr_hip_stats_t stats = {};
  bool huff_serial_ok = true;
  DeviceBuf huff_slots;
  bool huff_two_pass = false;
  bool huff_route_log = false;
  size_t huff_slots_refused = 0;
  DeviceBuf enc[3];
  uhdr_hip_ctx* aux = nullptr;
  struct AuxWorker* aux_worker = nullptr;
  DeviceBuf jpg[6];
  struct Resident {
    DeviceBuf buf;
    bool valid = false;
    uhdr_img_fmt_t fmt = UHDR_IMG_FMT_UNSPECIFIED;
    unsigned int w = 0, h = 0;
    const void* host[3] = {};
    unsigned int host_stride[3] = {};
    size_t off[3] = {};
    unsigned int dev_stride[3] = {};
    unsigned int prows[3] = {}, pcols[3] = {};
    bool host_unwritten = false;
    bool adopted = false;
    void* adopt_dst = nullptr;
    unsigned int adopt_stride = 0, adopt_w = 0, adopt_h = 0;
    bool adopt_expand = false;
  } resident[2];
  struct HuffHint { uint32_t sub_bits = 0, bits_per_block = 0; } huff_hint[16];
  struct HuffTabCache {
    bool valid = false, fast_ok = false;
    uint8_t key[4 * (17 + 256)] = {};
    DeviceBuf dev;
  } huff_tabs;
  struct PinArena {
    void* p = nullptr;
    size_t cap = 0, off = 0;
    hipEvent_t ev = nullptr;
    bool ev_pending = false;
  } pin;
  uint32_t* h_flags = nullptr;
  bool resident_on = false;
  bool resident_lazy = false;
  uhdr_error_info_t sticky = {};
  unsigned int resident_next = 0;
  struct PendingCopy {
    DeviceBuf buf;
    bool on = false;
    size_t off = 0, pitch = 0, dst_pitch = 0;
    unsigned int w = 0, h = 0, bps = 0;
    bool expand = false;
    void* dst = nullptr;
    DeviceBuf tmp;
  } pending;
  struct MallEntry { const void* p; uint64_t stamp; };
  std::vector<MallEntry> mall;
  uint64_t mall_clock = 0;
  DeviceBuf minmax;
  uint32_t* d_huff = nullptr;
  CoefSrc* d_coef_src = nullptr;
  unsigned int coef_src_next = 0;
  CoefSrc* coef_src_last_slot = nullptr;
  std::vector<uint8_t> coef_src_last;
  float* d_srgb8 = nullptr;
  StepTab srgb8_meta = {};
  float* d_lin10[5] = {};
  struct GainTab { float mn, mx; float* d; StepTab meta; };
  std::vector<GainTab> gain_tabs;
  void* comm = nullptr;
  int comm_rank = 0, comm_size = 0;
  bool comm_custom = false;
  uhdr_hip_comm_ops_t comm_ops = {};
  DeviceBuf exchange;
  DeviceBuf affine;
  float* d_srgb_of_byte = nullptr;
  float* h_mm = nullptr;
  bool defer_md = false;
  hipStream_t md_stream = nullptr;
  hipEvent_t md_ev = nullptr;
  std::function<void()> on_side_launched;
  bool side_job_posted = false;
  struct DeferredMd { bool valid = false, run = false; uhdr_hip_encode_cfg_t cfg; uhdr_color_transfer_t hdr_ct; int use_base_cg = 1; } deferred_md;
  hipEvent_t aux_ev = nullptr;
  hipEvent_t aux_ev2 = nullptr;
  bool prof = false;
  std::vector<ProfEntry> prof_entries;
};

struct ProfScope {
  uhdr_hip_ctx* c;
  ProfEntry e;
  bool on;
  ProfScope(uhdr_hip_ctx* ctx, const char* family) : c(ctx), on(ctx->prof) {
    if (!on) return;
    e.family = family;
    if (hipEventCreate(&e.a) != hipSuccess || hipEventCreate(&e.b) != hipSuccess) { on = false; return; }
    (void)hipEventRecord(e.a, c->stream);
  }
  ~ProfScope() {
    if (!on) return;
    (void)hipEventRecord(e.b, c->stream);
    c->prof_entries.push_back(e);
  }
};

namespace uhdr_api {
uhdr_error_info_t ensure(DeviceBuf& b, size_t bytes);
size_t bytes_per_sample(int fmt);
bool plane_geom(const uhdr_raw_image_t* im, int pl, size_t* rows, size_t* width);
size_t plane_bytes(const uhdr_raw_image_t* im, int pl);
uhdr_error_info_t validate_image(const uhdr_raw_image_t* im, const char* what);
ImageView view_of(const uhdr_raw_image_t* im);
ImageViewMut view_mut_of(const uhdr_raw_image_t* im);
uhdr_error_info_t adopted_copy_out(uhdr_hip_ctx* c, const void* src, size_t src_pitch, unsigned int bps, bool expand, unsigned int w, unsigned int h,
                                   void* dst, size_t dst_pitch);
uhdr_error_info_t resident_write_back(uhdr_hip_ctx* c, uhdr_hip_ctx::Resident& r);
uhdr_error_info_t resident_write_back_all(uhdr_hip_ctx* c);
void resident_retire(uhdr_hip_ctx* c, uhdr_hip_ctx::Resident& r, bool host_is_rewritten);
void resident_drop(uhdr_hip_ctx* c, const void* host_plane);
uhdr_error_info_t fast_h2d(uhdr_hip_ctx* c, void* dst, const void* src, size_t bytes);
uhdr_error_info_t stage_in(uhdr_hip_ctx* c, int slot, const uhdr_raw_image_t* host, uhdr_raw_image_t* dev, bool upload);
bool resident_keeps(int fmt);
uhdr_error_info_t resident_keep(uhdr_hip_ctx* c, const uhdr_raw_image_t* dev, const uhdr_raw_image_t* host, bool host_unwritten = false);
uhdr_error_info_t stage_out(uhdr_hip_ctx* c, const uhdr_raw_image_t* dev, uhdr_raw_image_t* host);
uhdr_error_info_t upload_lut(float** dst, const std::vector<float>& src, hipStream_t s);
uhdr_error_info_t upload_math(uhdr_hip_ctx* c);
uhdr_error_info_t upload_step_table(const host::OetfBuckets& b, float** slot, StepTab* meta, hipStream_t s);
uhdr_error_info_t gain_step_table(uhdr_hip_ctx* c, const GenParams& p, StepTab* out);
uhdr_error_info_t select_hdr_lut(uhdr_hip_ctx* c, uhdr_color_transfer_t ct, const float** lut, int* n);
uhdr_error_info_t validate_metadata(const uhdr_gainmap_metadata_t* m);
bool is_rgb_fmt_host(int fmt);
uhdr_error_info_t validate_apply(const uhdr_raw_image_t* sdr, const uhdr_raw_image_t* gm, const uhdr_gainmap_metadata_t* md, uhdr_color_transfer_t out_ct,
                                 const uhdr_raw_image_t* dest);
uhdr_error_info_t get_apply_tables(uhdr_hip_ctx* c, const uhdr_gainmap_metadata_t& md, float weight, int idw_scale, const float** d_out);
uhdr_error_info_t fill_gen_params(uhdr_hip_ctx* c, const uhdr_raw_image_t* sdr, const uhdr_raw_image_t* hdr, const uhdr_hip_encode_cfg_t* cfg, GenParams* p,
                                  int* use_base_cg, float* hdr_white_nits_out, bool sdr_in_registers = false);
void fill_finalize(MinmaxTableParams* t, const uhdr_hip_encode_cfg_t* cfg);
void fill_gainmap_desc(const uhdr_raw_image_t* hdr, const GenParams& p, uhdr_raw_image_t* gm);
uhdr_error_info_t generate_gainmap_finalize_md(const uhdr_hip_encode_cfg_t* cfg, uhdr_color_transfer_t hdr_ct, int use_base_cg, const float mm[6], uhdr_gainmap_metadata_t* md);
void note_table_stats(uhdr_hip_ctx* c, const uhdr_hip_encode_cfg_t* cfg);
uhdr_error_info_t two_pass_tail(uhdr_hip_ctx* c, const GenParams& p, int n_partials, const uhdr_hip_encode_cfg_t* cfg, uhdr_raw_image_t* gm);
uhdr_error_info_t fill_tone_map_params(uhdr_hip_ctx* c, const uhdr_raw_image_t* hdr, ToneMapParams* pp);
uhdr_error_info_t comm_all_reduce_min(uhdr_hip_ctx* c, float* buf, size_t n);
uhdr_error_info_t check_scan(const uhdr_hip_jpeg_scan_t* sc, bool need_coef, int* mcus_per_row, int* mcu_rows, int* blocks_per_mcu);
uhdr_error_info_t aux_context(uhdr_hip_ctx* c, uhdr_hip_ctx** out);
void aux_merge(uhdr_hip_ctx* c);
bool aux_post(uhdr_hip_ctx* c, std::function<void()> job);
void aux_wait(uhdr_hip_ctx* c);
}
using namespace uhdr_api;

void aux_worker_destroy(uhdr_hip_ctx* c);

#endif
```

libultrahdr_amd/csrc/api_jpeg.cpp:

```cpp
#include "api_internal.h"

void uhdr_hip_jpeg_quant_table(int quality, int is_chroma, uint16_t qt[64]) { host::jpeg_quant_table(quality, is_chroma, qt); }

int uhdr_hip_oetf_code_thresholds(uhdr_color_transfer_t ct, float thresholds[1024]) {
  if ((ct != UHDR_CT_HLG && ct != UHDR_CT_PQ) || !thresholds) return -1;
  const std::vector<float>& t = host::oetf_code_thresholds(ct);
  for (int i = 0; i < 1024; i++) thresholds[i] = t[(size_t)i];
  return 0;
}

uhdr_error_info_t uhdr_hip_selftest(uhdr_hip_ctx_t* c, int which, unsigned int arg0, unsigned int arg1, unsigned int seed, const float mm[6],
                                    unsigned long long out[8]) {
  if (!c) return err_status(UHDR_CODEC_INVALID_PARAM, "received nullptr for uhdr_hip context");
  if (!out || which < 0 || which > 4 || (which == 4 && (!mm || arg0 > 2 || arg1 < 1 || arg1 > 3 || arg0 >= arg1)) || (which == 2 && (arg0 < 1 || arg1 > 254 || arg0 > arg1)))
    return err_status(UHDR_CODEC_INVALID_PARAM, "bad self-test arguments");
  HIP_TRY(hipSetDevice(c->device));
  UHDR_TRY(upload_math(c));
  UHDR_TRY(ensure(c->affine, kAffineDevBytes));
  UHDR_TRY(ensure(c->exchange, 256));
  unsigned long long* d_out = (unsigned long long*)c->exchange.p;
  HIP_TRY(hipMemsetAsync(d_out, 0, 64, c->stream));
  if (which == 4) {
    MinmaxTableParams t;
    memset(&t, 0, sizeof t);
// ... 988 lines not shown
    rgb.w = sc.w;
    rgb.h = sc.h;
    const size_t pitch_px = ((size_t)sc.w + 63) & ~(size_t)63;
    UHDR_TRY(ensure(*out_buf, pitch_px * (size_t)out_channels * sc.h));
    rgb.planes[0] = out_buf->p;
    rgb.stride[0] = (unsigned int)pitch_px;
    UHDR_TRY(uhdr_hip_idct_dequant_rgb_dev(c, sc.coef[0], sc.coef[1], sc.coef[2], sc.blocks_w[0], sc.blocks_h[0], hdr->qtable[0], hdr->qtable[1], variant, &rgb));
    if (!lazy)
      HIP_TRY(hipMemcpy2DAsync(planes[0], (size_t)hstride[0] * out_channels, out_buf->p, pitch_px * out_channels, (size_t)sc.w * out_channels, sc.h,
                               hipMemcpyDeviceToHost, c->stream));
    if (res) {
      res->fmt = rgb.fmt; res->w = sc.w; res->h = sc.h;
      res->host[0] = planes[0]; res->host_stride[0] = hstride[0]; res->off[0] = 0; res->dev_stride[0] = (unsigned int)pitch_px;
      res->prows[0] = sc.h; res->pcols[0] = sc.w;
      res->valid = true;
      res->host_unwritten = lazy;
    }
  }
  if (lazy) c->stats.lazy_downloads_skipped++;
  dbg.mark("jpeg_decode_scan: IDCT (and download) enqueued");
  if (!lazy) HIP_TRY(hipStreamSynchronize(c->stream));
  dbg.mark("jpeg_decode_scan: done");
  return ok_status();
}

static bool is_420(const uhdr_hip_jpeg_scan_t& sc) {
  return sc.num_components == 3 && sc.h_samp[0] == 2 && sc.v_samp[0] == 2 && sc.h_samp[1] == 1 && sc.v_samp[1] == 1 && sc.h_samp[2] == 1 &&
         sc.v_samp[2] == 1;
}

static uhdr_error_info_t idct_upsample_rgb_impl(uhdr_hip_ctx_t* c, const int16_t* const coef[3], const int bw[3], const int bh[3],
                                                const uint16_t* const qt[3], int variant, uhdr_raw_image_t* rgb) {
  if (bw[1] != bw[2] || bh[1] != bh[2]) return err_status(UHDR_CODEC_UNSUPPORTED_FEATURE, "Cb and Cr block grids differ");
  for (int k = 0; k < 3; k++)
    for (int i = 0; i < 64; i++)
      if (qt[k][i] == 0) return err_status(UHDR_CODEC_INVALID_PARAM, "quantization table %d entry %d is zero", k, i);
  uint8_t* scratch = nullptr;
  if (variant == 0) {
    UHDR_TRY(ensure(c->jpg[5], upsample420_scratch_bytes(bw, bh)));
    scratch = (uint8_t*)c->jpg[5].p;
  }
  rgb->range = UHDR_CR_FULL_RANGE;
  ProfScope ps(c, "idct_upsample_rgb");
  HIP_TRY(launch_idct_upsample_rgb(coef, bw, bh, qt, variant, view_mut_of(rgb), scratch, c->stream));
  return ok_status();
}

uhdr_error_info_t uhdr_hip_idct_upsample_rgb_dev(uhdr_hip_ctx_t* c, const int16_t* coef_y, const int16_t* coef_cb, const int16_t* coef_cr,
                                                 unsigned int w, unsigned int h, const uint16_t qt_y[64], const uint16_t qt_cb[64],
                                                 const uint16_t qt_cr[64], int variant, uhdr_raw_image_t* rgb) {
  if (!c) return err_status(UHDR_CODEC_INVALID_PARAM, "received nullptr for uhdr_hip context");
  if (!coef_y || !coef_cb || !coef_cr || !qt_y || !qt_cb || !qt_cr || !rgb || !rgb->planes[0])
    return err_status(UHDR_CODEC_INVALID_PARAM, "received bad argument for idct_upsample_rgb");
  if (rgb->fmt != UHDR_IMG_FMT_24bppRGB888 && rgb->fmt != UHDR_IMG_FMT_32bppRGBA8888)
    return err_status(UHDR_CODEC_UNSUPPORTED_FEATURE, "idct_upsample_rgb expects UHDR_IMG_FMT_24bppRGB888 or UHDR_IMG_FMT_32bppRGBA8888. Received %d", rgb->fmt);
  if (variant != 0 && variant != 1) return err_status(UHDR_CODEC_INVALID_PARAM, "unknown libjpeg variant %d", variant);
  if (w == 0 || h == 0 || w > 65535 || h > 65535) return err_status(UHDR_CODEC_INVALID_PARAM, "image dimensions %ux%u are outside JPEG's 1..65535", w, h);
  if (rgb->w != w || rgb->h != h) return err_status(UHDR_CODEC_INVALID_PARAM, "destination is %ux%u, the image %ux%u", rgb->w, rgb->h, w, h);
  if (rgb->stride[0] < w) return err_status(UHDR_CODEC_INVALID_PARAM, "stride (%u) cannot be less than width (%u)", rgb->stride[0], w);
  if (((uintptr_t)coef_y | (uintptr_t)coef_cb | (uintptr_t)coef_cr) & 15)
    return err_status(UHDR_CODEC_INVALID_PARAM, "coefficient buffers must be 16-byte aligned");
  HIP_TRY(hipSetDevice(c->device));
  const int16_t* coef[3] = {coef_y, coef_cb, coef_cr};
  const int bw[3] = {(int)((w + 7) / 8), (int)((w + 15) / 16), (int)((w + 15) / 16)};
  const int bh[3] = {(int)((h + 7) / 8), (int)((h + 15) / 16), (int)((h + 15) / 16)};
  const uint16_t* qt[3] = {qt_y, qt_cb, qt_cr};
  return idct_upsample_rgb_impl(c, coef, bw, bh, qt, variant, rgb);
}

static uhdr_error_info_t jpeg_decode_rgb_impl(uhdr_hip_ctx_t* c, const uhdr_hip_jpeg_header_t* hdr, const uint8_t* scan_data, size_t scan_bytes,
                                              int out_channels, int variant, uint8_t* rgb, unsigned int stride_px) {
  if (!c) return err_status(UHDR_CODEC_INVALID_PARAM, "received nullptr for uhdr_hip context");
  if (!hdr || !scan_data || !rgb) return err_status(UHDR_CODEC_INVALID_PARAM, "received nullptr argument for jpeg_decode_rgb");
  if (out_channels != 3 && out_channels != 4) return err_status(UHDR_CODEC_INVALID_PARAM, "out_channels is 3 (RGB888) or 4 (RGBA8888), received %d", out_channels);
  if (variant != 0 && variant != 1) return err_status(UHDR_CODEC_INVALID_PARAM, "unknown libjpeg variant %d", variant);
  uhdr_hip_jpeg_scan_t sc = hdr->scan;
  int mpr = 0, mrows = 0, bpm = 0;
  UHDR_TRY(check_scan(&sc, false, &mpr, &mrows, &bpm));
  if (stride_px < sc.w) return err_status(UHDR_CODEC_INVALID_PARAM, "stride (%u) cannot be less than width (%u)", stride_px, sc.w);
  const bool s444 = sc.num_components == 3 && sc.h_samp[0] == 1 && sc.v_samp[0] == 1 && sc.h_samp[1] == 1 && sc.v_samp[1] == 1 &&
                    sc.h_samp[2] == 1 && sc.v_samp[2] == 1;
  if (s444) {
    uint8_t* planes[3] = {rgb, nullptr, nullptr};
    const unsigned int hs[3] = {stride_px, 0, 0}, vs[3] = {sc.h, 0, 0};
    return jpeg_decode_scan_impl(c, hdr, scan_data, scan_bytes, out_channels, variant, planes, hs, vs);
  }
  if (!is_420(sc))
    return err_status(UHDR_CODEC_UNSUPPORTED_FEATURE, "RGB output on the device takes 4:2:0 or 4:4:4 files; received %d components at %dx%d / %dx%d / %dx%d",
                      sc.num_components, sc.h_samp[0], sc.v_samp[0], sc.h_samp[1], sc.v_samp[1], sc.h_samp[2], sc.v_samp[2]);
  if (sc.blocks_w[1] != sc.blocks_w[2] || sc.blocks_h[1] != sc.blocks_h[2]) return err_status(UHDR_CODEC_UNSUPPORTED_FEATURE, "Cb and Cr block grids differ");
  const DbgClock dbg;
  UHDR_TRY(jpeg_scan_to_coefficients(c, hdr, scan_data, scan_bytes, dbg, sc));
  resident_drop(c, rgb);
  uhdr_raw_image_t img;
  memset(&img, 0, sizeof img);
  img.fmt = out_channels == 3 ? UHDR_IMG_FMT_24bppRGB888 : UHDR_IMG_FMT_32bppRGBA8888;
  img.w = sc.w;
  img.h = sc.h;
  const size_t pitch_px = ((size_t)sc.w + 63) & ~(size_t)63;
  UHDR_TRY(ensure(c->jpg[4], pitch_px * (size_t)out_channels * sc.h));
  img.planes[0] = c->jpg[4].p;
  img.stride[0] = (unsigned int)pitch_px;
  const uint16_t* qt[3] = {hdr->qtable[0], hdr->qtable[1], hdr->qtable[2]};
  UHDR_TRY(idct_upsample_rgb_impl(c, sc.coef, sc.blocks_w, sc.blocks_h, qt, variant, &img));
  HIP_TRY(hipMemcpy2DAsync(rgb, (size_t)stride_px * out_channels, c->jpg[4].p, pitch_px * out_channels, (size_t)sc.w * out_channels, sc.h,
                           hipMemcpyDeviceToHost, c->stream));
  HIP_TRY(hipStreamSynchronize(c->stream));
  dbg.mark("jpeg_decode_rgb: done");
  return ok_status();
}

uhdr_error_info_t uhdr_hip_jpeg_decode_rgb(uhdr_hip_ctx_t* c, const uhdr_hip_jpeg_header_t* hdr, const uint8_t* scan_data, size_t scan_bytes,
                                           int out_channels, int variant, uint8_t* rgb, unsigned int stride_px) {
  const auto t0 = std::chrono::steady_clock::now();
  const uhdr_error_info_t r = jpeg_decode_rgb_impl(c, hdr, scan_data, scan_bytes, out_channels, variant, rgb, stride_px);
  if (c) c->stats.last_jpeg_decode_rgb_ns = (unsigned long long)std::chrono::duration_cast<std::chrono::nanoseconds>(std::chrono::steady_clock::now() - t0).count();
  return r;
}

uhdr_error_info_t uhdr_hip_decode_api1_scans_dev(uhdr_hip_ctx_t* c, const uhdr_hip_jpeg_header_t* base, const uint8_t* base_data, size_t base_bytes,
                                                 uhdr_color_gamut_t base_cg, const uhdr_hip_jpeg_header_t* map, const uint8_t* map_data, size_t map_bytes,
                                                 uhdr_color_gamut_t map_cg, int libjpeg_variant, const uhdr_gainmap_metadata_t* md,
                                                 uhdr_color_transfer_t output_ct, uhdr_img_fmt_t output_format, float max_display_boost,
                                                 uhdr_raw_image_t* dest) {
  if (!c) return err_status(UHDR_CODEC_INVALID_PARAM, "received nullptr for uhdr_hip context");
  if (!base || !base_data || !map || !map_data || !md || !dest) return err_status(UHDR_CODEC_INVALID_PARAM, "received nullptr argument for decode_api1_scans");
  if (libjpeg_variant != 0 && libjpeg_variant != 1) return err_status(UHDR_CODEC_INVALID_PARAM, "unknown libjpeg variant %d", libjpeg_variant);
  uhdr_hip_jpeg_scan_t sb = base->scan, sm = map->scan;
  int mpr = 0, mrows = 0, bpm = 0;
  UHDR_TRY(check_scan(&sb, false, &mpr, &mrows, &bpm));
  if (sb.num_components != 3 || sb.h_samp[0] != 2 || sb.v_samp[0] != 2 || sb.h_samp[1] != 1 || sb.v_samp[1] != 1 || sb.h_samp[2] != 1 || sb.v_samp[2] != 1)
    return err_status(UHDR_CODEC_UNSUPPORTED_FEATURE, "decode_api1_scans takes a 4:2:0 base image (the form JpegR writes); decode the scans with uhdr_hip_jpeg_decode_scan");
  UHDR_TRY(check_scan(&sm, false, &mpr, &mrows, &bpm));
  const int nm = sm.num_components;
  if (nm == 3 && (bpm != 3 || memcmp(map->qtable[1], map->qtable[2], sizeof map->qtable[1])))
    return err_status(UHDR_CODEC_UNSUPPORTED_FEATURE, "a three-channel gain map is a 4:4:4 scan with one chroma quantization table here");
  if (base_bytes == 0 || map_bytes == 0 || base_bytes > 0xFFFFFFF0ull || map_bytes > 0xFFFFFFF0ull) return err_status(UHDR_CODEC_INVALID_PARAM, "received no (or too much) entropy-coded data");
  HIP_TRY(hipSetDevice(c->device));
  for (int i = 0; i < 3; i++) {
    UHDR_TRY(ensure(c->jpg[1 + i], (size_t)sb.blocks_w[i] * sb.blocks_h[i] * 128));
    sb.coef[i] = (const int16_t*)c->jpg[1 + i].p;
  }
  size_t off = 0, o_map[3] = {0, 0, 0};
  for (int i = 0; i < nm; i++) { o_map[i] = off; off += ((size_t)sm.blocks_w[i] * sm.blocks_h[i] * 128 + 255) & ~(size_t)255; }
  UHDR_TRY(ensure(c->enc[0], off));
  for (int i = 0; i < nm; i++) sm.coef[i] = (const int16_t*)((const uint8_t*)c->enc[0].p + o_map[i]);
  c->huff_serial_ok = false;
  auto tables_of = [](const uhdr_hip_jpeg_header_t* h) -> const uhdr_hip_huff_tables_t* {
    for (int t = 0; t < 4; t++)
      for (int l = 0; l < 17; l++)
        if (h->tables.bits[t][l]) return &h->tables;
    return nullptr;
  };
  const uhdr_error_info_t hs = uhdr_hip_huffman_decode2_dev(c, &sb, tables_of(base), base_data, base_bytes, &sm, tables_of(map), map_data, map_bytes);
  c->huff_serial_ok = true;
  if (hs.error_code != UHDR_CODEC_OK) return hs;
  uhdr_raw_image_t gm;
  memset(&gm, 0, sizeof gm);
  gm.cg = map_cg;
  gm.ct = UHDR_CT_UNSPECIFIED;
  gm.range = UHDR_CR_FULL_RANGE;
  gm.w = sm.w;
  gm.h = sm.h;
  const size_t pitch_px = ((size_t)sm.w + 63) & ~(size_t)63;
  if (nm == 3) {
    gm.fmt = UHDR_IMG_FMT_32bppRGBA8888;
    UHDR_TRY(ensure(c->jpg[4], pitch_px * 4 * sm.h));
    gm.planes[0] = c->jpg[4].p;
    gm.stride[0] = (unsigned int)pitch_px;
    UHDR_TRY(uhdr_hip_idct_dequant_rgb_dev(c, sm.coef[0], sm.coef[1], sm.coef[2], sm.blocks_w[0], sm.blocks_h[0], map->qtable[0], map->qtable[1], libjpeg_variant, &gm));
  } else {
    gm.fmt = UHDR_IMG_FMT_8bppYCbCr400;
    const size_t pitch = ((size_t)sm.blocks_w[0] * 8 + 63) & ~(size_t)63;
    UHDR_TRY(ensure(c->jpg[4], pitch * (size_t)sm.blocks_h[0] * 8));
    gm.planes[0] = c->jpg[4].p;
    gm.stride[0] = (unsigned int)pitch;
    UHDR_TRY(uhdr_hip_idct_dequant_dev(c, sm.coef[0], sm.blocks_w[0], sm.blocks_h[0], map->qtable[0], (uint8_t*)c->jpg[4].p, pitch));
  }
  uhdr_hip_jpeg_coefficients_t bc;
  memset(&bc, 0, sizeof bc);
  for (int i = 0; i < 3; i++) {
    bc.coef[i] = sb.coef[i];
    bc.blocks_w[i] = sb.blocks_w[i];
    bc.blocks_h[i] = sb.blocks_h[i];
    memcpy(bc.qtable[i], base->qtable[i], sizeof bc.qtable[i]);
  }
  uhdr_error_info_t ap = uhdr_hip_apply_gainmap_coef_dev(c, &bc, sb.w, sb.h, base_cg, &gm, md, output_ct, output_format, max_display_boost, dest);
  if (ap.error_code != UHDR_CODEC_UNSUPPORTED_FEATURE) return ap;
  size_t ppitch[3], poff[3], total = 0;
  for (int i = 0; i < 3; i++) {
    ppitch[i] = ((size_t)sb.blocks_w[i] * 8 + 63) & ~(size_t)63;
    poff[i] = total;
    total += ppitch[i] * (size_t)sb.blocks_h[i] * 8;
  }
  UHDR_TRY(ensure(c->jpg[0], total));
  uhdr_raw_image_t bi;
  memset(&bi, 0, sizeof bi);
  bi.fmt = UHDR_IMG_FMT_12bppYCbCr420;
  bi.cg = base_cg;
  bi.ct = UHDR_CT_SRGB;
  bi.range = UHDR_CR_FULL_RANGE;
  bi.w = sb.w;
  bi.h = sb.h;
  for (int i = 0; i < 3; i++) {
    uint8_t* d = (uint8_t*)c->jpg[0].p + poff[i];
    UHDR_TRY(uhdr_hip_idct_dequant_dev(c, sb.coef[i], sb.blocks_w[i], sb.blocks_h[i], base->qtable[i], d, ppitch[i]));
    bi.planes[i] = d;
    bi.stride[i] = (unsigned int)ppitch[i];
  }
  return uhdr_hip_apply_gainmap_dev(c, &bi, &gm, md, output_ct, output_format, max_display_boost, dest, 0, 0);
}

size_t uhdr_hip_jpeg_assemble(const uhdr_hip_jpeg_scan_t* sc, const uint16_t qt_luma[64], const uint16_t qt_chroma[64], const uint8_t* scan_data,
                              size_t scan_bytes, uint8_t* out, size_t cap) {
  int mpr = 0, mrows = 0, bpm = 0;
  if (check_scan(sc, false, &mpr, &mrows, &bpm).error_code != UHDR_CODEC_OK || !qt_luma || !scan_data || !out) return 0;
  if (sc->num_components > 1 && !qt_chroma) return 0;
  const int nc = sc->num_components, ntab = nc > 1 ? 2 : 1;
  const uint8_t* zz = host::jpeg_zigzag_to_natural();
  std::vector<uint8_t> v;
  v.reserve(scan_bytes + 1024);
  auto put = [&](unsigned b) { v.push_back((uint8_t)b); };
  auto put16 = [&](unsigned x) { put(x >> 8); put(x & 0xff); };
  put(0xff); put(0xd8);
  put(0xff); put(0xe0); put16(16); for (char ch : {'J', 'F', 'I', 'F'}) put((unsigned char)ch); put(0); put(1); put(1); put(0); put16(1); put16(1); put(0); put(0);
  for (int t = 0; t < ntab; t++) {
    const uint16_t* q = t ? qt_chroma : qt_luma;
    put(0xff); put(0xdb); put16(67); put(t);
    for (int i = 0; i < 64; i++) {
      if (q[zz[i]] == 0 || q[zz[i]] > 255) return 0;
      put(q[zz[i]]);
    }
  }
  put(0xff); put(0xc0); put16(8 + 3 * nc); put(8); put16(sc->h); put16(sc->w); put(nc);
  for (int i = 0; i < nc; i++) { put(i + 1); put(((nc == 1 ? 1 : sc->h_samp[i]) << 4) | (nc == 1 ? 1 : sc->v_samp[i])); put(i ? 1 : 0); }
  for (int t = 0; t < ntab; t++) {
    for (int ac = 0; ac < 2; ac++) {
      uint8_t bits[17], vals[256];
      const int nv = host::jpeg_std_huff_table(ac, t, bits, vals);
      put(0xff); put(0xc4); put16(2 + 1 + 16 + nv); put((ac << 4) | t);
      for (int i = 1; i <= 16; i++) put(bits[i]);
      for (int i = 0; i < nv; i++) put(vals[i]);
    }
  }
  if (sc->restart_interval > 0) { put(0xff); put(0xdd); put16(4); put16((unsigned)sc->restart_interval); }
  put(0xff); put(0xda); put16(6 + 2 * nc); put(nc);
  for (int i = 0; i < nc; i++) { put(i + 1); put(i ? 0x11 : 0x00); }
  put(0); put(63); put(0);
  v.insert(v.end(), scan_data, scan_data + scan_bytes);
  put(0xff); put(0xd9);
  if (v.size() > cap) return 0;
  memcpy(out, v.data(), v.size());
  return v.size();
}
```

libultrahdr_amd/csrc/huffman_decode_sync.hip:

```cpp
#include <cstdio>
#include <cstdlib>
#include <cstring>

#include "lds_copy.h"
#include "wg_scan.h"
#include "uhdr_types.h"

namespace uhdr {
namespace {

constexpr int kChunk = 4096;
constexpr int kSyncBlock = 64;

__device__ __forceinline__ uint32_t rst_weight1(uint32_t at) { return (at * 2654435761u + 0x9e3779b9u) | 1u; }
__device__ __forceinline__ uint32_t rst_weight2(uint32_t at) { return ((at ^ (at >> 15)) * 0x85ebca6bu + 0xc2b2ae35u) | 1u; }
__device__ __forceinline__ bool is_stuffed(const uint8_t* __restrict__ d, uint32_t i) { return i > 0 && d[i] == 0 && d[i - 1] == 0xffu; }
__device__ __forceinline__ bool is_rst_first(const uint8_t* __restrict__ d, uint32_t i, uint32_t n) {
  return d[i] == 0xffu && i + 1 < n && (d[i + 1] & 0xf8u) == 0xd0u;
}
template <bool RST>
__device__ __forceinline__ bool is_dropped(const uint8_t* __restrict__ d, uint32_t i, uint32_t n) {
  if (is_stuffed(d, i)) return true;
  if (!RST) return false;
  return is_rst_first(d, i, n) || (i > 0 && (d[i] & 0xf8u) == 0xd0u && d[i - 1] == 0xffu);
// ... 1202 lines not shown
__device__ __forceinline__ void chain_entry_walk(const HuffSyncArgs& a, const uint8_t* __restrict__ tile_map, uint8_t* __restrict__ tile_entry,
                                                 uint8_t (*s_tiles)[kMapPitch], uint8_t (*s_gmap)[kMapPitch], uint32_t* s_gentry ) {
  const int tid = (int)threadIdx.x;
  const uint32_t nclean = a.nbytes - *a.nstuffed, nbits = nclean * 8u;
  const int nlinks = (int)((nbits + a.sub_bits - 1) / a.sub_bits) - 1;
  const int ntiles = (nlinks + kChainTile - 1) / kChainTile;
  const int grp = tid / kHuffHypSlots, s = tid - grp * kHuffHypSlots;
  uint32_t carry = 0;
  for (int c0 = 0; c0 < ntiles; c0 += kChainTile) {
    chain_stage_rows(s_tiles, tid, tile_map, c0, ntiles);
    __syncthreads();
    {
      uint32_t cur = (uint32_t)s;
#pragma unroll
      for (int k = 0; k < kChainGroup; k++) cur = chain_step(s_tiles[grp * kChainGroup + k], cur);
      s_gmap[grp][s] = (uint8_t)cur;
    }
    __syncthreads();
    if (tid == 0) {
      uint32_t c = carry;
      for (int g = 0; g < kChainGroups; g++) {
        s_gentry[g] = c;
        c = chain_step(s_gmap[g], c);
      }
      s_gentry[kChainGroups] = c;
    }
    __syncthreads();
    if (tid < kChainGroups) {
      uint32_t cur = s_gentry[tid];
      for (int k = 0; k < kChainGroup; k++) {
        const int tl = c0 + tid * kChainGroup + k;
        if (tl < ntiles) tile_entry[tl] = (uint8_t)cur;
        cur = chain_step(s_tiles[tid * kChainGroup + k], cur);
      }
    }
    carry = s_gentry[kChainGroups];
    __syncthreads();
  }
}
__global__ __launch_bounds__(kChainWg) void hyp_chain_tiles_kernel(const HuffSyncArgs a, uint8_t* __restrict__ prefix ,
                                                                   uint8_t* __restrict__ tile_map ) {
  __shared__ __attribute__((aligned(16))) uint8_t s_links[kChainTile][kMapPitch];
  __shared__ __attribute__((aligned(16))) uint8_t s_gmap[kChainGroups][kMapPitch];
  __shared__ __attribute__((aligned(16))) uint8_t s_gpre[kChainGroups][kMapPitch];
  const int tid = (int)threadIdx.x;
  const uint32_t nclean = a.nbytes - *a.nstuffed, nbits = nclean * 8u;
  const int nsub = (int)((nbits + a.sub_bits - 1) / a.sub_bits);
  const int nlinks = nsub - 1;
  const int base = (int)blockIdx.x * kChainTile;
  if (base < nlinks) {
    chain_stage_rows(s_links, tid, a.hyp_map, base, nlinks);
    __syncthreads();
    const int grp = tid / kHuffHypSlots, s = tid - grp * kHuffHypSlots;
    {
      uint32_t cur = (uint32_t)s;
#pragma unroll
      for (int k = 0; k < kChainGroup; k++) cur = chain_step(s_links[grp * kChainGroup + k], cur);
      s_gmap[grp][s] = (uint8_t)cur;
    }
    __syncthreads();
    if (tid < kHuffHypSlots) {
      uint32_t c = (uint32_t)tid;
#pragma unroll
      for (int g = 0; g < kChainGroups; g++) {
        s_gpre[g][tid] = (uint8_t)c;
        c = chain_step(s_gmap[g], c);
      }
      tile_map[(size_t)blockIdx.x * kHuffHypSlots + tid] = (uint8_t)c;
    }
    __syncthreads();
    uint32_t cur = s_gpre[grp][s];
#pragma unroll
    for (int k = 0; k < kChainGroup; k++) {
      const int link = grp * kChainGroup + k, i = base + link;
      if (i < nlinks) prefix[(size_t)i * kHuffHypSlots + s] = (uint8_t)cur;
      cur = chain_step(s_links[link], cur);
    }
  }
}
__global__ __launch_bounds__(kChainWg) void hyp_chain_entry_kernel(const HuffSyncArgs a, const uint8_t* __restrict__ tile_map, uint8_t* __restrict__ tile_entry) {
  __shared__ __attribute__((aligned(16))) uint8_t s_tiles[kChainTile][kMapPitch];
  __shared__ __attribute__((aligned(16))) uint8_t s_gmap[kChainGroups][kMapPitch];
  __shared__ uint32_t s_gentry[kChainGroups + 1];
  chain_entry_walk(a, tile_map, tile_entry, s_tiles, s_gmap, s_gentry);
}
__global__ __launch_bounds__(kChainThreads) void hyp_chain_walk_kernel(const HuffSyncArgs a, const uint8_t* __restrict__ prefix,
                                                                       const uint8_t* __restrict__ tile_entry) {
  const int tid = (int)threadIdx.x;
  const uint32_t nclean = a.nbytes - *a.nstuffed, nbits = nclean * 8u;
  const int nsub = (int)((nbits + a.sub_bits - 1) / a.sub_bits);
  const int nlinks = nsub - 1;
  const int i = (int)blockIdx.x * kChainTile + tid;
  bool lost = false;
  if (i < nlinks) {
    uint32_t g = tile_entry[blockIdx.x];
    if (g != 0xffu) g = prefix[(size_t)i * kHuffHypSlots + g];
    if (g == 0xffu) {
      lost = true;
    } else {
      const size_t at = (size_t)i * kHuffHypSlots + g;
      const uint64_t end_i = a.hyp_state[at];
      const uint32_t cnt_next = a.hyp_cnt[at];
      a.state[0][i] = end_i;
      a.nblk[i + 1] = cnt_next;
      if (a.pieces > 1) {
        const uint32_t Q = (uint32_t)a.pieces;
        a.pend[(size_t)i * Q + (Q - 1u)] = end_i;
        const size_t mo = at * (size_t)(Q - 1u);
        uint32_t sum = 0;
        for (uint32_t q = 0; q + 1u < Q; q++) {
          const uint32_t cq = a.mid_cnt[mo + q];
          a.pend[(size_t)(i + 1) * Q + q] = a.mid_state[mo + q];
          a.pcnt[(size_t)(i + 1) * Q + q] = cq;
          sum += cq;
        }
        a.pcnt[(size_t)(i + 1) * Q + (Q - 1u)] = cnt_next - sum;
      }
      if (i == nlinks - 1 && a.hyp_map[at] == 0xffu) lost = true;
    }
  }
  const uint64_t m = __builtin_amdgcn_ballot_w64(lost);
  if (m != 0 && (uint32_t)(tid & 63) == (uint32_t)__builtin_ctzll(m)) atomicOr(a.flags + 2, 1u);
}

__device__ __forceinline__ void dc_block_scan(int v[3], int* s_sum , int) {
  int x[3] = {v[0], v[1], v[2]}, all[3];
  wg_incl_scan<1024, 3>(x, s_sum, all);
  v[0] = x[0]; v[1] = x[1]; v[2] = x[2];
}
__global__ __launch_bounds__(1024) void dc_partial_kernel(const HuffSyncArgs a, int* __restrict__ partial) {
  __shared__ int s_sum[3 * 16];
  const int tid = (int)threadIdx.x;
  const uint32_t t = blockIdx.x * 1024u + (uint32_t)tid;
  int v[3] = {0, 0, 0};
  if (t < a.total_blocks) v[a.comp_of[t % (uint32_t)a.blocks_per_mcu]] = a.dcd[t];
  dc_block_scan(v, s_sum, tid);
  if (tid == 1023) { partial[blockIdx.x * 3] = v[0]; partial[blockIdx.x * 3 + 1] = v[1]; partial[blockIdx.x * 3 + 2] = v[2]; }
}
constexpr int kPlaceChunk = 256;
__device__ __forceinline__ void dc_chunk_scan(int v[3], int* s_sum , int) {
  int x[3] = {v[0], v[1], v[2]}, all[3];
  wg_incl_scan<kPlaceChunk, 3>(x, s_sum, all);
  v[0] = x[0]; v[1] = x[1]; v[2] = x[2];
}
__global__ __launch_bounds__(kPlaceChunk) void dc_partial2_kernel(const HuffSyncArgs a, int* __restrict__ partial) {
  __shared__ int s_sum[3 * (kPlaceChunk / 64)];
  const int tid = (int)threadIdx.x;
  const uint32_t t = blockIdx.x * (uint32_t)kPlaceChunk + (uint32_t)tid;
  int v[3] = {0, 0, 0};
  if (t < a.total_blocks) v[a.comp_of[t % (uint32_t)a.blocks_per_mcu]] = a.coef_scan[(size_t)t * 64];
  dc_chunk_scan(v, s_sum, tid);
  if (tid == kPlaceChunk - 1) { partial[blockIdx.x * 3] = v[0]; partial[blockIdx.x * 3 + 1] = v[1]; partial[blockIdx.x * 3 + 2] = v[2]; }
}
constexpr int kPlaceSelfPrefix = 4096;
__global__ __launch_bounds__(kPlaceChunk) void coef_place_kernel(const HuffSyncArgs a, const int* __restrict__ partial, int self_prefix) {
  __shared__ int s_sum[3 * (kPlaceChunk / 64)];
  __shared__ int16_t s_dc[kPlaceChunk];
  __shared__ uint32_t s_dst[kPlaceChunk];
  __shared__ uint8_t s_inv[64];
  const int tid = (int)threadIdx.x;
  const uint32_t t0 = blockIdx.x * (uint32_t)kPlaceChunk, t = t0 + (uint32_t)tid;
  const uint32_t bpm = (uint32_t)a.blocks_per_mcu;
  if (tid < 64) s_inv[a.zigzag[tid]] = (uint8_t)tid;
  int v[3] = {0, 0, 0};
  int c = 0;
  uint32_t where = 0xffffffffu;
  if (t < a.total_blocks) {
    const uint32_t m = t / bpm, j = t - m * bpm;
    c = a.comp_of[j];
    v[c] = a.coef_scan[(size_t)t * 64];
    const int my = (int)(m / (uint32_t)a.mcus_per_row), mx = (int)(m - (uint32_t)my * (uint32_t)a.mcus_per_row);
    const int jj = (int)j - a.first_blk[c];
    const int by = my * a.vs[c] + jj / a.hs[c], bx = mx * a.hs[c] + jj % a.hs[c];
    if (by < a.bh[c] && bx < a.bw[c]) where = ((uint32_t)c << 30) | ((uint32_t)by * (uint32_t)a.bw[c] + (uint32_t)bx);
  }
  s_dst[tid] = where;
  int carry[3];
  if (self_prefix) {
    int part[3] = {0, 0, 0};
    for (uint32_t i = (uint32_t)tid; i < blockIdx.x; i += (uint32_t)kPlaceChunk) {
      part[0] += partial[i * 3];
      part[1] += partial[i * 3 + 1];
      part[2] += partial[i * 3 + 2];
    }
    wg_incl_scan<kPlaceChunk, 3>(part, s_sum, carry);
  } else {
    carry[0] = partial[blockIdx.x * 3];
    carry[1] = partial[blockIdx.x * 3 + 1];
    carry[2] = partial[blockIdx.x * 3 + 2];
  }
  dc_chunk_scan(v, s_sum, tid);
  s_dc[tid] = (int16_t)((c == 0 ? carry[0] : (c == 1 ? carry[1] : carry[2])) + v[c]);
  __syncthreads();
  const uint32_t lane = (uint32_t)tid & 63u, wv = (uint32_t)tid >> 6;
  const uint32_t half = lane >> 5, n0 = (lane & 31u) * 2u;
  const uint32_t z0 = s_inv[n0], z1 = s_inv[n0 + 1u];
  int16_t* const c0 = a.coef[0];
  int16_t* const c1 = a.coef[1];
  int16_t* const c2 = a.coef[2];
#pragma unroll 4
  for (uint32_t s = 0; s < 32u; s++) {
    const uint32_t loc = wv * 64u + s * 2u + half;
    const uint32_t ent = s_dst[loc];
    if (ent == 0xffffffffu) continue;
    const int16_t* src = a.coef_scan + (size_t)(t0 + loc) * 64;
    uint32_t lo = (uint16_t)src[z0];
    const uint32_t hi = (uint16_t)src[z1];
    if (n0 == 0) lo = (uint16_t)s_dc[loc];
    const uint32_t cc = ent >> 30;
    int16_t* base = cc == 0 ? c0 : (cc == 1 ? c1 : c2);
    uint32_t* dst = (uint32_t*)(base + (size_t)(ent & 0x3fffffffu) * 64);
    dst[lane & 31u] = lo | (hi << 16);
  }
}
__global__ __launch_bounds__(1024) void dc_scan_partials_kernel(int* __restrict__ partial, int nchunks) {
  __shared__ int s_sum[3 * 16];
  const int tid = (int)threadIdx.x;
  const int per = (nchunks + 1023) / 1024, lo = min(tid * per, nchunks), hi = min(lo + per, nchunks);
  int v[3] = {0, 0, 0};
  for (int i = lo; i < hi; i++)
    for (int c = 0; c < 3; c++) v[c] += partial[i * 3 + c];
  int own[3] = {v[0], v[1], v[2]};
  dc_block_scan(v, s_sum, tid);
  int run[3] = {v[0] - own[0], v[1] - own[1], v[2] - own[2]};
  for (int i = lo; i < hi; i++)
    for (int c = 0; c < 3; c++) {
      const int x = partial[i * 3 + c];
      partial[i * 3 + c] = run[c];
      run[c] += x;
    }
}
__global__ __launch_bounds__(1024) void dc_apply_kernel(const HuffSyncArgs a, const int* __restrict__ partial) {
  __shared__ int s_sum[3 * 16];
  const int tid = (int)threadIdx.x;
  const uint32_t t = blockIdx.x * 1024u + (uint32_t)tid;
  const uint32_t bpm = (uint32_t)a.blocks_per_mcu;
  int v[3] = {0, 0, 0};
  int c = 0;
  uint32_t m = 0, j = 0;
  if (t < a.total_blocks) {
    m = t / bpm;
    j = t - m * bpm;
    c = a.comp_of[j];
    v[c] = a.dcd[t];
  }
  dc_block_scan(v, s_sum, tid);
  if (t >= a.total_blocks) return;
  const int dc = partial[blockIdx.x * 3 + c] + v[c];
  if (a.rst_map) {
    a.dcd[t] = dc;
    if ((t + 1u) % a.rst_blocks == 0 && t + 1u < a.total_blocks) {
      int* g = a.dc_seg + (size_t)((t + 1u) / a.rst_blocks) * 3;
      for (int cc = 0; cc < 3; cc++) g[cc] = partial[blockIdx.x * 3 + cc] + v[cc];
    }
    return;
  }
  const int my = (int)(m / (uint32_t)a.mcus_per_row), mx = (int)(m - (uint32_t)my * (uint32_t)a.mcus_per_row);
  const int jj = (int)j - a.first_blk[c];
  const int by = my * a.vs[c] + jj / a.hs[c], bx = mx * a.hs[c] + jj % a.hs[c];
  if (by < a.bh[c] && bx < a.bw[c]) a.coef[c][((size_t)by * a.bw[c] + bx) * 64] = (int16_t)dc;
}
__global__ __launch_bounds__(256) void dc_restart_kernel(const HuffSyncArgs a) {
  if (blockIdx.x == 0) {
    __shared__ uint32_t s_acc[3];
    if (threadIdx.x < 3) s_acc[threadIdx.x] = 0;
    __syncthreads();
    uint32_t v[3] = {0, 0, 0};
    for (uint32_t i = threadIdx.x; i < a.rst_chunks; i += 256u)
      for (int k = 0; k < 3; k++) v[k] += a.rst_partial[i * 3 + k];
    for (int k = 0; k < 3; k++)
      if (v[k]) atomicAdd(&s_acc[k], v[k]);
    __syncthreads();
    if (threadIdx.x == 0) { a.flags[9] = s_acc[0]; a.flags[16] = s_acc[1]; a.flags[17] = s_acc[2]; }
  }
  const uint32_t t = blockIdx.x * 256u + threadIdx.x;
  if (t >= a.total_blocks) return;
  const uint32_t bpm = (uint32_t)a.blocks_per_mcu;
  const uint32_t m = t / bpm, j = t - m * bpm, seg = t / a.rst_blocks;
  const int c = a.comp_of[j];
  const int dc = a.dcd[t] - (seg ? a.dc_seg[(size_t)seg * 3 + c] : 0);
  const int my = (int)(m / (uint32_t)a.mcus_per_row), mx = (int)(m - (uint32_t)my * (uint32_t)a.mcus_per_row);
  const int jj = (int)j - a.first_blk[c];
  const int by = my * a.vs[c] + jj / a.hs[c], bx = mx * a.hs[c] + jj % a.hs[c];
  if (by < a.bh[c] && bx < a.bw[c]) a.coef[c][((size_t)by * a.bw[c] + bx) * 64] = (int16_t)dc;
}

}

static void launch_write(const HuffSyncArgs& a, uint32_t nsub, int final_buf, hipStream_t s) {
  const size_t per_wave = (size_t)64 * ((a.sub_bits >> 3) + 4) + 64;
  const int waves = per_wave * 4 <= (20u << 10) ? 4 : (per_wave * 2 <= (20u << 10) ? 2 : 1);
  const size_t lds = per_wave * waves;
  const int threads = 64 * waves;
  const int grid = (int)((nsub + threads - 1) / threads);
  if (lds > (20u << 10)) (void)hipFuncSetAttribute((const void*)sync_write_kernel, hipFuncAttributeMaxDynamicSharedMemorySize, (int)lds);
  hipLaunchKernelGGL(sync_write_kernel, dim3(grid), dim3(threads), lds, s, a, final_buf);
}

int huff_sync_chunks(uint64_t nbytes) { return (int)((nbytes + kChunk - 1) / kChunk); }

namespace {
__global__ __launch_bounds__(256) void stray_marker_kernel(const uint8_t* __restrict__ data, uint32_t n, uint32_t* __restrict__ flag) {
  const uint32_t base = (blockIdx.x * 256u + threadIdx.x) * 16u;
  if (base >= n) return;
  bool found = false;
  if (base + 17u <= n && ((uintptr_t)(data + base) & 15u) == 0) {
    const uint4 v = *(const uint4*)(data + base);
    const uint32_t w[5] = {v.x, v.y, v.z, v.w, (uint32_t)data[base + 16u]};
#pragma unroll
    for (uint32_t i = 0; i < 16; i++) {
      const uint32_t c0 = (w[i >> 2] >> (8u * (i & 3u))) & 0xffu, c1 = (w[(i + 1u) >> 2] >> (8u * ((i + 1u) & 3u))) & 0xffu;
      found = found || (c0 == 0xffu && c1 != 0u && c1 != 0xffu && (c1 & 0xf8u) != 0xd0u);
    }
  } else {
    for (uint32_t i = base; i < base + 16u && i + 1u < n; i++) {
      const uint32_t c0 = data[i], c1 = data[i + 1u];
      found = found || (c0 == 0xffu && c1 != 0u && c1 != 0xffu && (c1 & 0xf8u) != 0xd0u);
    }
  }
  if (found) *(volatile uint32_t*)flag = 1u;
}
}
hipError_t launch_stray_marker_check(const uint8_t* data, uint32_t nbytes, uint32_t* flag, hipStream_t s) {
  const int grid = (int)((nbytes + 4095u) / 4096u);
  hipLaunchKernelGGL(stray_marker_kernel, dim3(grid), dim3(256), 0, s, data, nbytes, flag);
  return hipGetLastError();
}

hipError_t launch_huffman_unstuff(const uint8_t* data, uint32_t nbytes, uint32_t* chunk_counts, uint32_t* nstuffed_dev, uint8_t* clean, hipStream_t s,
                                  uint32_t* rst_map, uint32_t* rst_partial, const HuffInitFill* fill) {
  const int nchunks = huff_sync_chunks(nbytes);
  HuffInitFill f;
  memset(&f, 0, sizeof f);
  if (fill) f = *fill;
  if (rst_map) hipLaunchKernelGGL(unstuff_count_kernel<true>, dim3(nchunks), dim3(256), 0, s, data, nbytes, chunk_counts, f);
  else hipLaunchKernelGGL(unstuff_count_kernel<false>, dim3(nchunks), dim3(256), 0, s, data, nbytes, chunk_counts, f);
  uint32_t* total = nstuffed_dev;
  if (nchunks > kUnstuffSelfPrefix) {
    hipLaunchKernelGGL(sync_scan_kernel, dim3(1), dim3(1024), 0, s, chunk_counts, nchunks, nstuffed_dev);
    total = nullptr;
  }
  if (rst_map) hipLaunchKernelGGL(unstuff_compact_kernel<true>, dim3(nchunks), dim3(256), 0, s, data, nbytes, (const uint32_t*)chunk_counts, clean, rst_map, rst_partial, total);
  else hipLaunchKernelGGL(unstuff_compact_kernel<false>, dim3(nchunks), dim3(256), 0, s, data, nbytes, (const uint32_t*)chunk_counts, clean, rst_map, rst_partial, total);
  return hipGetLastError();
}
static void launch_write2(const HuffSyncArgs& a, uint32_t nsub, int final_buf, hipStream_t s) {
  const size_t per_wave = (size_t)64 * ((a.sub_bits >> 3) + 4) + 64;
  const int waves = per_wave * 4 <= (20u << 10) ? 4 : (per_wave * 2 <= (20u << 10) ? 2 : 1);
  const size_t lds = sizeof(Write2Lds) + per_wave * waves;
  const int threads = 64 * waves;
  const int grid = (int)((nsub + threads - 1) / threads);
  static size_t opted = 0;
  if (lds > opted) {
    (void)hipFuncSetAttribute((const void*)sync_write2_kernel, hipFuncAttributeMaxDynamicSharedMemorySize, (int)lds);
    opted = lds;
  }
  hipLaunchKernelGGL(sync_write2_kernel, dim3(grid), dim3(threads), lds, s, a, final_buf);
}
static void launch_place(const HuffSyncArgs& a, int* dc_partial, hipStream_t s) {
  const int nch = (int)((a.total_blocks + kPlaceChunk - 1) / kPlaceChunk);
  hipLaunchKernelGGL(dc_partial2_kernel, dim3(nch), dim3(kPlaceChunk), 0, s, a, dc_partial);
  const int self_prefix = nch <= kPlaceSelfPrefix ? 1 : 0;
  if (!self_prefix) hipLaunchKernelGGL(dc_scan_partials_kernel, dim3(1), dim3(1024), 0, s, dc_partial, nch);
  hipLaunchKernelGGL(coef_place_kernel, dim3(nch), dim3(kPlaceChunk), 0, s, a, (const int*)dc_partial, self_prefix);
}
int huff_place_chunk() { return kPlaceChunk; }
static void launch_dc(const HuffSyncArgs& a, int* dc_partial, hipStream_t s) {
  const int nch = (int)((a.total_blocks + 1023) / 1024);
  hipLaunchKernelGGL(dc_partial_kernel, dim3(nch), dim3(1024), 0, s, a, dc_partial);
  hipLaunchKernelGGL(dc_scan_partials_kernel, dim3(1), dim3(1024), 0, s, dc_partial, nch);
  hipLaunchKernelGGL(dc_apply_kernel, dim3(nch), dim3(1024), 0, s, a, (const int*)dc_partial);
  if (a.rst_map) hipLaunchKernelGGL(dc_restart_kernel, dim3((a.total_blocks + 255) / 256), dim3(256), 0, s, a);
}

uint32_t huff_sync_max_subsequences(uint64_t nbytes, uint32_t sub_bits) { return (uint32_t)((nbytes * 8 + sub_bits - 1) / sub_bits); }

hipError_t launch_huffman_decode_sync(const HuffSyncArgs& a, int max_rounds, int* dc_partial, int* final_buf, hipStream_t s) {
  const uint32_t nsub = huff_sync_max_subsequences(a.nbytes, a.sub_bits);
  const int grid = (int)((nsub + kSyncBlock - 1) / kSyncBlock);
  const size_t lds = (size_t)kSyncBlock * ((a.sub_bits >> 3) + 4) + 64;
  for (int r = 0; r <= max_rounds; r++) hipLaunchKernelGGL(sync_round_kernel, dim3(grid), dim3(kSyncBlock), lds, s, a, r);
  *final_buf = 0;
  {
    const int nt = (int)((nsub + kScanTile - 1) / kScanTile);
    hipLaunchKernelGGL(scan_tiles_kernel, dim3(nt), dim3(kScanThreads), 0, s, a.nblk, (int)nsub, a.scan_tmp);
  }
  if (a.coef_scan && !a.rst_map) {
    launch_write2(a, nsub, *final_buf, s);
    launch_place(a, dc_partial, s);
  } else {
    launch_write(a, nsub, *final_buf, s);
    launch_dc(a, dc_partial, s);
  }
  return hipGetLastError();
}

size_t huff_hyp_chain_bytes(uint64_t nbytes, uint32_t sub_bits, size_t* tiles_offset) {
  const size_t nsub = huff_sync_max_subsequences(nbytes, sub_bits), ntiles = (nsub + kChainTile - 1) / kChainTile;
  const size_t pre = ntiles * kChainThreads * kHuffHypSlots;
  if (tiles_offset) *tiles_offset = pre;
  return pre + ntiles * kHuffHypSlots + ((ntiles + 255) & ~(size_t)255);
}

hipError_t launch_huffman_decode_hyp(const HuffSyncArgs& a, int* dc_partial, uint8_t* chain_prefix, uint8_t* chain_tiles, hipStream_t s) {
  const uint32_t nsub = huff_sync_max_subsequences(a.nbytes, a.sub_bits);
  const int grid = (int)((nsub + 63) / 64);
  const int threads = 64 * a.hyp_h;
  const size_t lds0 = (size_t)64 * ((a.sub_bits >> 3) + 4) + 64;
  const size_t lds1_stage = ((((size_t)(64 + a.hyp_levels) * ((a.sub_bits >> 3) + 4) + 16 + 7) >> 2) + 1 & ~(size_t)1) * 4;
  const size_t lds1 = lds1_stage + (size_t)threads * 10 + 16;
  {
    static size_t opted = 0;
    if (lds1 + sizeof(PairLds) + 64 > (64u << 10) && lds1 > opted) {
      const hipError_t e1 = hipFuncSetAttribute((const void*)hyp_pass1q_kernel, hipFuncAttributeMaxDynamicSharedMemorySize, (int)lds1);
      if (e1 != hipSuccess) return e1;
      opted = lds1;
    }
  }
  const bool dbg = getenv("UHDR_HIP_HUFF_DEBUG") != nullptr;
  hipEvent_t ev[9];
  int nev = 0;
  auto mark = [&]() {
    if (dbg && nev < 9) {
      (void)hipEventCreate(&ev[nev]);
      (void)hipEventRecord(ev[nev], s);
      nev++;
    }
  };
  mark();
  static const bool qmerge = !(getenv("UHDR_HIP_HUFF_QMERGE") && atoi(getenv("UHDR_HIP_HUFF_QMERGE")) == 0);
  static const bool no_fused = getenv("UHDR_HIP_HUFF_NO_FUSED_PASSES") != nullptr;
  const size_t lds01 = (((((size_t)64 * ((a.sub_bits >> 3) + 4) + 16 + 7) >> 2) + 1) & ~(size_t)1) * 4 + (size_t)64 * a.hyp_h * 8 + (size_t)threads * 2 + 16;
  if (qmerge && !no_fused && a.hyp_main_levels == 1 && a.hyp_levels > 1 && !a.rst_map && lds01 + sizeof(PairLds) + 64 <= (64u << 10)) {
    hipLaunchKernelGGL(hyp_pass01_kernel, dim3((nsub + kFusedStride - 1) / kFusedStride), dim3(threads), lds01, s, a);
    mark();
  } else {
    hipLaunchKernelGGL(hyp_pass0_kernel, dim3(grid), dim3(threads), lds0, s, a);
    mark();
    if (qmerge) hipLaunchKernelGGL(hyp_pass1q_kernel, dim3(grid), dim3(threads), lds1, s, a);
    else hipLaunchKernelGGL(hyp_pass1_kernel, dim3(grid), dim3(threads), lds1, s, a);
  }
  {
    const hipError_t e1 = hipGetLastError();
    if (e1 != hipSuccess) return e1;
  }
  if (qmerge && a.hyp_main_levels > 0 && a.hyp_main_levels < a.hyp_levels) {
    static const int smul = [] { const char* e = getenv("UHDR_HIP_HUFF_STRAG_MUL"); const int v = e ? atoi(e) : 1; return v >= 1 && v <= 16 ? v : 1; }();
    int sgrid = (int)((nsub * (uint32_t)a.hyp_h / 16u + kStragWaves - 1) / kStragWaves) * smul;
    if (sgrid < 64) sgrid = 64;
    if (sgrid > 4096) sgrid = 4096;
    hipLaunchKernelGGL(hyp_straggler_kernel, dim3(sgrid), dim3(64 * kStragWaves), 0, s, a);
  }
  mark();
  const int ntiles = (int)((nsub + kChainTile - 1) / kChainTile);
  uint8_t* chain_entry = chain_tiles + (size_t)ntiles * kHuffHypSlots;
  hipLaunchKernelGGL(hyp_chain_tiles_kernel, dim3(ntiles), dim3(kChainWg), 0, s, a, chain_prefix, chain_tiles);
  hipLaunchKernelGGL(hyp_chain_entry_kernel, dim3(1), dim3(kChainWg), 0, s, a, (const uint8_t*)chain_tiles, chain_entry);
  hipLaunchKernelGGL(hyp_chain_walk_kernel, dim3(ntiles), dim3(kChainThreads), 0, s, a, (const uint8_t*)chain_prefix, (const uint8_t*)chain_entry);
  mark();
  HuffSyncArgs w = a;
  uint32_t nw = nsub;
  if (a.pieces > 1 && a.coef_scan && !a.rst_map) {
    w.sub_bits = a.sub_bits / (uint32_t)a.pieces;
    w.state[0] = a.pend;
    w.nblk = a.pcnt;
    nw = nsub * (uint32_t)a.pieces;
  }
  {
    const int nt = (int)((nw + kScanTile - 1) / kScanTile);
    hipLaunchKernelGGL(scan_tiles_kernel, dim3(nt), dim3(kScanThreads), 0, s, w.nblk, (int)nw, w.scan_tmp);
  }
  mark();
  if (a.coef_scan && !a.rst_map) {
    launch_write2(w, nw, 0, s);
    mark();
    launch_place(a, dc_partial, s);
  } else {
    launch_write(a, nsub, 0, s);
    mark();
    launch_dc(a, dc_partial, s);
  }
  mark();
  if (dbg) {
    (void)hipStreamSynchronize(s);
    static const char* names[] = {"pass0", "pass1 (+ stragglers)", "chain x3", "nblk scan", "write", "dc x3 / place", "-"};
    fprintf(stderr, "uhdr_hip: hypothesis decode kernels:");
    for (int i = 0; i + 1 < nev; i++) {
      float ms = 0;
      (void)hipEventElapsedTime(&ms, ev[i], ev[i + 1]);
      fprintf(stderr, " %s %.0f us,", names[i], ms * 1e3f);
    }
    fprintf(stderr, "\n");
    for (int i = 0; i < nev; i++) (void)hipEventDestroy(ev[i]);
  }
  return hipGetLastError();
}

}
```

libultrahdr_amd/csrc/idct_core.h:

```cpp
#pragma once
#include "uhdr_types.h"

namespace uhdr {
namespace idct {

#define FIX_0_298631336 2446
#define FIX_0_390180644 3196
#define FIX_0_541196100 4433
#define FIX_0_765366865 6270
#define FIX_0_899976223 7373
#define FIX_1_175875602 9633
#define FIX_1_501321110 12299
#define FIX_1_847759065 15137
#define FIX_1_961570560 16069
#define FIX_2_053119869 16819
#define FIX_2_562915447 20995
#define FIX_3_072711026 25172

template <bool M24>
__device__ __forceinline__ int mulc(int a, int c) {
  if constexpr (M24) return __mul24(a, c);
  else return (int)((uint32_t)a * (uint32_t)c);
}
template <int PASS, bool M24>
__device__ __forceinline__ void idct_1d(const int in[8], int out[8]) {
  constexpr int sh = PASS == 0 ? 13 - 2 : 13 + 2 + 3;
  constexpr uint32_t fudge = (1u << (sh - 1)) + (PASS == 1 ? (512u << 18) : 0u);
  int z2 = in[2], z3 = in[6];
  int z1 = mulc<M24>(z2 + z3, FIX_0_541196100);
  int tmp2 = z1 + mulc<M24>(z3, -FIX_1_847759065);
  int tmp3 = z1 + mulc<M24>(z2, FIX_0_765366865);
  z2 = in[0]; z3 = in[4];
  int tmp0 = (int)(((uint32_t)(z2 + z3) << 13) + fudge);
  int tmp1 = (int)(((uint32_t)(z2 - z3) << 13) + fudge);
  const int tmp10 = tmp0 + tmp3, tmp13 = tmp0 - tmp3, tmp11 = tmp1 + tmp2, tmp12 = tmp1 - tmp2;
  tmp0 = in[7]; tmp1 = in[5]; tmp2 = in[3]; tmp3 = in[1];
  z1 = tmp0 + tmp3; z2 = tmp1 + tmp2; z3 = tmp0 + tmp2;
  int z4 = tmp1 + tmp3;
  const int z5 = mulc<M24>(z3 + z4, FIX_1_175875602);
  tmp0 = mulc<M24>(tmp0, FIX_0_298631336);
  tmp1 = mulc<M24>(tmp1, FIX_2_053119869);
  tmp2 = mulc<M24>(tmp2, FIX_3_072711026);
  tmp3 = mulc<M24>(tmp3, FIX_1_501321110);
  z1 = mulc<M24>(z1, -FIX_0_899976223);
  z2 = mulc<M24>(z2, -FIX_2_562915447);
  z3 = mulc<M24>(z3, -FIX_1_961570560);
  z4 = mulc<M24>(z4, -FIX_0_390180644);
  z3 += z5; z4 += z5;
  tmp0 += z1 + z3; tmp1 += z2 + z4; tmp2 += z2 + z3; tmp3 += z1 + z4;
  const int sum[8] = {tmp10 + tmp3, tmp11 + tmp2, tmp12 + tmp1, tmp13 + tmp0, tmp13 - tmp0, tmp12 - tmp1, tmp11 - tmp2, tmp10 - tmp3};
#pragma unroll
  for (int k = 0; k < 8; k++) {
    if constexpr (PASS == 0) {
      out[k] = sum[k] >> sh;
    } else {
      const int t = (int)(((uint32_t)sum[k] >> 18) & 1023u) - 384;
      out[k] = min(max(t, 0), 255);
    }
  }
}

__device__ __forceinline__ void load_dequant_row(const int16_t* __restrict__ coef, int bw, int by, int bx, int rr,
                                                 const int q[8], int v[8], int& big, bool row_ok = true) {
  if (bx < bw && row_ok) {
    const uint4 raw = *(const uint4*)(coef + ((size_t)by * bw + bx) * 64 + rr * 8);
    const uint32_t w4[4] = {raw.x, raw.y, raw.z, raw.w};
#pragma unroll
    for (int c = 0; c < 4; c++) {
      v[2 * c] = __mul24((int)(int16_t)(w4[c] & 0xffff), q[2 * c]);
      v[2 * c + 1] = __mul24((int)(int16_t)(w4[c] >> 16), q[2 * c + 1]);
    }
    const int mx = max(max(max(v[0], v[1]), max(v[2], v[3])), max(max(v[4], v[5]), max(v[6], v[7])));
    const int mn = min(min(min(v[0], v[1]), min(v[2], v[3])), min(min(v[4], v[5]), min(v[6], v[7])));
    big |= (int)(mx > 8191) | (int)(mn < -8191);
  } else {
#pragma unroll
    for (int c = 0; c < 8; c++) v[c] = 0;
  }
}

__device__ __forceinline__ void idct_wave(int* ws, const int v[8], int big, int rr, int rb, uint32_t s[8]) {
  const int cb = rr, cc = rb;
  const bool fast = __builtin_amdgcn_ballot_w64(big != 0) == 0;
#pragma unroll
  for (int c = 0; c < 8; c++) ws[rb * 72 + rr * 9 + c] = v[c];
  __builtin_amdgcn_wave_barrier();
  __builtin_amdgcn_s_waitcnt(0xc07f);
  int in[8], out[8];
#pragma unroll
  for (int r = 0; r < 8; r++) in[r] = ws[cb * 72 + r * 9 + cc];
  if (fast) idct_1d<0, true>(in, out); else idct_1d<0, false>(in, out);
  __builtin_amdgcn_wave_barrier();
#pragma unroll
  for (int r = 0; r < 8; r++) ws[cb * 72 + r * 9 + cc] = out[r];
  __builtin_amdgcn_wave_barrier();
  __builtin_amdgcn_s_waitcnt(0xc07f);
#pragma unroll
  for (int c = 0; c < 8; c++) in[c] = ws[rb * 72 + rr * 9 + c];
  if (fast) idct_1d<1, true>(in, out); else idct_1d<1, false>(in, out);
#pragma unroll
  for (int c = 0; c < 8; c++) s[c] = (uint32_t)out[c];
  __builtin_amdgcn_wave_barrier();
}

}
}
```

libultrahdr_amd/csrc/jpeg_decode.hip:

```cpp
#include "idct_core.h"
#include "uhdr_types.h"

namespace uhdr {
namespace {

using namespace idct;

constexpr int kBlock = 256;

struct DequantArgs {
  uint16_t q[64];
};

__global__ __launch_bounds__(kBlock) void idct_dequant_kernel(const int16_t* __restrict__ coef, int bw, int bh,
                                                              const DequantArgs qa, uint8_t* __restrict__ plane,
                                                              size_t stride) {
  __shared__ int s_ws[kBlock / 64][8 * 8 * 9];
  const int lane = threadIdx.x & 63, wv = threadIdx.x >> 6;
  int* ws = s_ws[wv];
  const int groups_x = (bw + 7) >> 3, total = groups_x * bh;
  const int gwave = blockIdx.x * (kBlock / 64) + wv, nwaves = gridDim.x * (kBlock / 64);
  const int rr = lane >> 3, rb = lane & 7;
  int q[8];
#pragma unroll
  for (int c = 0; c < 8; c++) q[c] = qa.q[rr * 8 + c];
  const bool vec_store = ((stride | (uintptr_t)plane) & 7) == 0;

  for (int t = gwave; t < total; t += nwaves) {
    const int by = t / groups_x, gx = t - by * groups_x;
    const int bx = gx * 8 + rb;
    int v[8];
    int big = 0;
    load_dequant_row(coef, bw, by, bx, rr, q, v, big);
    uint32_t s[8];
    idct_wave(ws, v, big, rr, rb, s);
    if (bx < bw) {
      const uint32_t lo = s[0] | (s[1] << 8) | (s[2] << 16) | (s[3] << 24);
      const uint32_t hi = s[4] | (s[5] << 8) | (s[6] << 16) | (s[7] << 24);
      uint8_t* dst = plane + (size_t)(by * 8 + rr) * stride + (size_t)bx * 8;
      if (vec_store) {
        *(uint2*)dst = make_uint2(lo, hi);
      } else {
#pragma unroll
        for (int c = 0; c < 4; c++) { dst[c] = (uint8_t)(lo >> (8 * c)); dst[4 + c] = (uint8_t)(hi >> (8 * c)); }
      }
    }
  }
}

#define FIX16(x) ((int)((x) * 65536.0 + 0.5))

__device__ __forceinline__ void rgb_to_ycc_px(uint32_t r, uint32_t g, uint32_t b, uint32_t& y, uint32_t& cb, uint32_t& cr) {
  const int half = 1 << 15, off = 128 << 16;
  const int ri = (int)r, gi = (int)g, bi = (int)b;
  y = (uint32_t)((FIX16(0.29900) * ri + FIX16(0.58700) * gi + FIX16(0.11400) * bi + half) >> 16);
  cb = (uint32_t)(((-FIX16(0.16874)) * ri + (-FIX16(0.33126)) * gi + FIX16(0.50000) * bi + off + half - 1) >> 16);
  cr = (uint32_t)((FIX16(0.50000) * ri + (-FIX16(0.41869)) * gi + (-FIX16(0.08131)) * bi + off + half - 1) >> 16);
}

struct JpegColorParams {
  const uint8_t* rgb;
  uint8_t* rgb_out;
  const uint8_t* p[3];
  uint8_t* po[3];
  uint32_t w, h, rgb_stride_px, stride[3];
  int bpp;
  int k_cr_g, k_cb_g;
};

template <int BPP, bool VEC>
__global__ __launch_bounds__(kBlock) void jpeg_rgb_to_ycc_kernel(const JpegColorParams p) {
  const uint32_t per_row = VEC ? p.w / 4 : p.w;
  const uint32_t tiles_x = (per_row + kBlock - 1) / kBlock, tiles = tiles_x * p.h;
  for (uint32_t t = blockIdx.x; t < tiles; t += gridDim.x) {
    const uint32_t y = t / tiles_x, j = (t - y * tiles_x) * kBlock + threadIdx.x;
    if (j >= per_row) continue;
    const uint8_t* src = p.rgb + (size_t)y * p.rgb_stride_px * BPP;
    if constexpr (VEC) {
      uint32_t r[4], g[4], b[4];
      if constexpr (BPP == 4) {
        const uint4 v = *(const uint4*)(src + j * 16);
        const uint32_t w4[4] = {v.x, v.y, v.z, v.w};
#pragma unroll
        for (int k = 0; k < 4; k++) { r[k] = w4[k] & 0xff; g[k] = (w4[k] >> 8) & 0xff; b[k] = (w4[k] >> 16) & 0xff; }
      } else {
        const uint32_t* s3 = (const uint32_t*)(src + j * 12);
        const uint32_t a = s3[0], bq = s3[1], c = s3[2];
        r[0] = a & 0xff; g[0] = (a >> 8) & 0xff; b[0] = (a >> 16) & 0xff;
        r[1] = a >> 24; g[1] = bq & 0xff; b[1] = (bq >> 8) & 0xff;
        r[2] = (bq >> 16) & 0xff; g[2] = bq >> 24; b[2] = c & 0xff;
        r[3] = (c >> 8) & 0xff; g[3] = (c >> 16) & 0xff; b[3] = c >> 24;
      }
      uint32_t yo = 0, cbo = 0, cro = 0;
#pragma unroll
      for (int k = 0; k < 4; k++) {
        uint32_t yy, cb, cr;
        rgb_to_ycc_px(r[k], g[k], b[k], yy, cb, cr);
        yo |= yy << (8 * k); cbo |= cb << (8 * k); cro |= cr << (8 * k);
      }
      *(uint32_t*)(p.po[0] + (size_t)y * p.stride[0] + j * 4) = yo;
      *(uint32_t*)(p.po[1] + (size_t)y * p.stride[1] + j * 4) = cbo;
      *(uint32_t*)(p.po[2] + (size_t)y * p.stride[2] + j * 4) = cro;
    } else {
      uint32_t yy, cb, cr;
      rgb_to_ycc_px(src[j * BPP], src[j * BPP + 1], src[j * BPP + 2], yy, cb, cr);
      p.po[0][(size_t)y * p.stride[0] + j] = (uint8_t)yy;
      p.po[1][(size_t)y * p.stride[1] + j] = (uint8_t)cb;
      p.po[2][(size_t)y * p.stride[2] + j] = (uint8_t)cr;
    }
  }
}

__device__ __forceinline__ uint32_t clamp255(int v) { return (uint32_t)min(max(v, 0), 255); }
__device__ __forceinline__ uint32_t ycc_to_rgb_px(uint32_t y, uint32_t cb, uint32_t cr, int k_cr_g, int k_cb_g) {
  const int half = 1 << 15;
  const int yy = (int)y, u = (int)cb - 128, v = (int)cr - 128;
  const uint32_t r = clamp255(yy + ((FIX16(1.40200) * v + half) >> 16));
  const uint32_t g = clamp255(yy + (((-k_cb_g) * u + half + (-k_cr_g) * v) >> 16));
  const uint32_t b = clamp255(yy + ((FIX16(1.77200) * u + half) >> 16));
  return r | (g << 8) | (b << 16) | (255u << 24);
}

template <int BPP, bool VEC>
__global__ __launch_bounds__(kBlock) void jpeg_ycc_to_rgb_kernel(const JpegColorParams p) {
  const uint32_t per_row = VEC ? p.w / 4 : p.w;
  const uint32_t tiles_x = (per_row + kBlock - 1) / kBlock, tiles = tiles_x * p.h;
  for (uint32_t t = blockIdx.x; t < tiles; t += gridDim.x) {
    const uint32_t y = t / tiles_x, j = (t - y * tiles_x) * kBlock + threadIdx.x;
    if (j >= per_row) continue;
    uint8_t* dst = p.rgb_out + (size_t)y * p.rgb_stride_px * BPP;
    if constexpr (VEC) {
      const uint32_t yv = *(const uint32_t*)(p.p[0] + (size_t)y * p.stride[0] + j * 4);
      const uint32_t uv = *(const uint32_t*)(p.p[1] + (size_t)y * p.stride[1] + j * 4);
      const uint32_t vv = *(const uint32_t*)(p.p[2] + (size_t)y * p.stride[2] + j * 4);
      uint32_t px[4];
#pragma unroll
      for (int k = 0; k < 4; k++)
        px[k] = ycc_to_rgb_px((yv >> (8 * k)) & 0xff, (uv >> (8 * k)) & 0xff, (vv >> (8 * k)) & 0xff, p.k_cr_g, p.k_cb_g);
      if constexpr (BPP == 4) {
        *(uint4*)(dst + j * 16) = make_uint4(px[0], px[1], px[2], px[3]);
      } else {
        uint32_t* d3 = (uint32_t*)(dst + j * 12);
        d3[0] = (px[0] & 0xffffff) | (px[1] << 24);
        d3[1] = ((px[1] >> 8) & 0xffff) | (px[2] << 16);
        d3[2] = ((px[2] >> 16) & 0xff) | (px[3] << 8);
      }
    } else {
      const uint32_t px = ycc_to_rgb_px(p.p[0][(size_t)y * p.stride[0] + j], p.p[1][(size_t)y * p.stride[1] + j],
                                        p.p[2][(size_t)y * p.stride[2] + j], p.k_cr_g, p.k_cb_g);
      dst[j * BPP] = (uint8_t)px; dst[j * BPP + 1] = (uint8_t)(px >> 8); dst[j * BPP + 2] = (uint8_t)(px >> 16);
      if constexpr (BPP == 4) dst[j * BPP + 3] = 255;
    }
  }
}

struct IdctRgbArgs {
  const int16_t* coef[3];
  uint8_t* rgb;
  size_t pitch;
  uint32_t w, h;
  int bw, bh;
  int k_cr_g, k_cb_g;
  uint16_t q[2][64];
};

template <int BPP>
__global__ __launch_bounds__(kBlock) void idct_dequant_rgb_kernel(const IdctRgbArgs a) {
  __shared__ int s_ws[kBlock / 64][8 * 8 * 9];
  const int lane = threadIdx.x & 63, wv = threadIdx.x >> 6;
  int* ws = s_ws[wv];
  const int bw = a.bw;
  const int groups_x = (bw + 7) >> 3, total = groups_x * a.bh;
  const int gwave = blockIdx.x * (kBlock / 64) + wv, nwaves = gridDim.x * (kBlock / 64);
  const int rr = lane >> 3, rb = lane & 7;
  int ql[8], qc[8];
#pragma unroll
  for (int c = 0; c < 8; c++) { ql[c] = a.q[0][rr * 8 + c]; qc[c] = a.q[1][rr * 8 + c]; }
  const bool vec_ok = ((a.pitch | (uintptr_t)a.rgb) & (BPP == 4 ? 15 : 7)) == 0;

  for (int t = gwave; t < total; t += nwaves) {
    const int by = t / groups_x, gx = t - by * groups_x;
    const int bx = gx * 8 + rb;
    int vy[8], vb[8], vr[8];
    int big_y = 0, big_b = 0, big_r = 0;
    load_dequant_row(a.coef[0], bw, by, bx, rr, ql, vy, big_y);
    load_dequant_row(a.coef[1], bw, by, bx, rr, qc, vb, big_b);
    load_dequant_row(a.coef[2], bw, by, bx, rr, qc, vr, big_r);
    uint32_t sy[8], sb[8], sr[8];
    idct_wave(ws, vy, big_y, rr, rb, sy);
    idct_wave(ws, vb, big_b, rr, rb, sb);
    idct_wave(ws, vr, big_r, rr, rb, sr);
    const uint32_t y = (uint32_t)(by * 8 + rr), x0 = (uint32_t)bx * 8;
    if (bx < bw && y < a.h && x0 < a.w) {
      uint32_t px[8];
#pragma unroll
      for (int c = 0; c < 8; c++) px[c] = ycc_to_rgb_px(sy[c], sb[c], sr[c], a.k_cr_g, a.k_cb_g);
      uint8_t* dst = a.rgb + (size_t)y * a.pitch + (size_t)x0 * BPP;
      if (vec_ok && x0 + 8 <= a.w) {
        if constexpr (BPP == 4) {
          *(uint4*)dst = make_uint4(px[0], px[1], px[2], px[3]);
          *(uint4*)(dst + 16) = make_uint4(px[4], px[5], px[6], px[7]);
        } else {
          uint32_t d[6];
#pragma unroll
          for (int h = 0; h < 2; h++) {
            const uint32_t* q4 = px + 4 * h;
            d[3 * h + 0] = (q4[0] & 0xffffff) | (q4[1] << 24);
            d[3 * h + 1] = ((q4[1] >> 8) & 0xffff) | (q4[2] << 16);
            d[3 * h + 2] = ((q4[2] >> 16) & 0xff) | (q4[3] << 8);
          }
          *(uint2*)dst = make_uint2(d[0], d[1]);
          *(uint2*)(dst + 8) = make_uint2(d[2], d[3]);
          *(uint2*)(dst + 16) = make_uint2(d[4], d[5]);
        }
      } else {
#pragma unroll
        for (int c = 0; c < 8; c++) {
          if (x0 + c < a.w) {
            dst[c * BPP] = (uint8_t)px[c]; dst[c * BPP + 1] = (uint8_t)(px[c] >> 8); dst[c * BPP + 2] = (uint8_t)(px[c] >> 16);
            if constexpr (BPP == 4) dst[c * BPP + 3] = 255;
          }
        }
      }
    }
  }
}

int resident_grid(uint32_t tiles, int per_cu) {
  static const int cus = [] {
    int dev = 0, n = 0;
    if (hipGetDevice(&dev) != hipSuccess) return 256;
    if (hipDeviceGetAttribute(&n, hipDeviceAttributeMultiprocessorCount, dev) != hipSuccess || n <= 0) n = 256;
    return n;
  }();
  const uint32_t r = (uint32_t)(cus * per_cu);
  return (int)(tiles < r ? (tiles ? tiles : 1u) : r);
}

inline bool al(const void* p, size_t a) { return ((uintptr_t)p % a) == 0; }

}

hipError_t launch_idct_dequant(const int16_t* coef, int bw, int bh, const uint16_t* qt_host, uint8_t* plane,
                               size_t stride, hipStream_t s) {
  DequantArgs qa;
  for (int i = 0; i < 64; i++) qa.q[i] = qt_host[i];
  const int total = ((bw + 7) / 8) * bh;
  const int grid = resident_grid((uint32_t)(total + 3) / 4, 8);
  hipLaunchKernelGGL(idct_dequant_kernel, dim3(grid), dim3(kBlock), 0, s, coef, bw, bh, qa, plane, stride);
  return hipGetLastError();
}

hipError_t launch_idct_dequant_rgb(const int16_t* coef_y, const int16_t* coef_cb, const int16_t* coef_cr, int bw, int bh,
                                   const uint16_t* qt_luma_host, const uint16_t* qt_chroma_host, int variant,
                                   const ImageViewMut& rgb, hipStream_t s) {
  IdctRgbArgs a = {};
  a.coef[0] = coef_y; a.coef[1] = coef_cb; a.coef[2] = coef_cr;
  a.rgb = (uint8_t*)rgb.p[0];
  const int bpp = rgb.fmt == UHDR_IMG_FMT_32bppRGBA8888 ? 4 : 3;
  a.pitch = (size_t)rgb.stride[0] * bpp;
  a.w = rgb.w; a.h = rgb.h; a.bw = bw; a.bh = bh;
  a.k_cr_g = variant ? FIX16(0.714136286) : FIX16(0.71414);
  a.k_cb_g = variant ? FIX16(0.344136286) : FIX16(0.34414);
  for (int i = 0; i < 64; i++) { a.q[0][i] = qt_luma_host[i]; a.q[1][i] = qt_chroma_host[i]; }
  const int total = ((bw + 7) / 8) * bh;
  const int grid = resident_grid((uint32_t)(total + 3) / 4, 8);
  if (bpp == 4) hipLaunchKernelGGL((idct_dequant_rgb_kernel<4>), dim3(grid), dim3(kBlock), 0, s, a);
  else hipLaunchKernelGGL((idct_dequant_rgb_kernel<3>), dim3(grid), dim3(kBlock), 0, s, a);
  return hipGetLastError();
}

hipError_t launch_jpeg_rgb_to_ycc(const ImageView& rgb, const ImageViewMut& ycc, hipStream_t s) {
  JpegColorParams p = {};
  p.rgb = (const uint8_t*)rgb.p[0];
  p.w = rgb.w; p.h = rgb.h; p.rgb_stride_px = rgb.stride[0];
  p.bpp = rgb.fmt == UHDR_IMG_FMT_32bppRGBA8888 ? 4 : 3;
  for (int c = 0; c < 3; c++) { p.po[c] = (uint8_t*)ycc.p[c]; p.stride[c] = ycc.stride[c]; }
  const bool vec = (p.w % 4 == 0) && al(p.rgb, p.bpp == 4 ? 16 : 4) && ((size_t)p.rgb_stride_px * p.bpp) % (p.bpp == 4 ? 16 : 4) == 0 &&
                   al(p.po[0], 4) && al(p.po[1], 4) && al(p.po[2], 4) && p.stride[0] % 4 == 0 && p.stride[1] % 4 == 0 && p.stride[2] % 4 == 0;
  const uint32_t per_row = vec ? p.w / 4 : p.w;
  const int grid = resident_grid(((per_row + kBlock - 1) / kBlock) * p.h, 8);
  if (p.bpp == 4) {
    if (vec) hipLaunchKernelGGL((jpeg_rgb_to_ycc_kernel<4, true>), dim3(grid), dim3(kBlock), 0, s, p);
    else hipLaunchKernelGGL((jpeg_rgb_to_ycc_kernel<4, false>), dim3(grid), dim3(kBlock), 0, s, p);
  } else {
    if (vec) hipLaunchKernelGGL((jpeg_rgb_to_ycc_kernel<3, true>), dim3(grid), dim3(kBlock), 0, s, p);
    else hipLaunchKernelGGL((jpeg_rgb_to_ycc_kernel<3, false>), dim3(grid), dim3(kBlock), 0, s, p);
  }
  return hipGetLastError();
}

hipError_t launch_jpeg_ycc_to_rgb(const ImageView& ycc, const ImageViewMut& rgb, int variant, hipStream_t s) {
  JpegColorParams p = {};
  p.rgb_out = (uint8_t*)rgb.p[0];
  p.w = ycc.w; p.h = ycc.h; p.rgb_stride_px = rgb.stride[0];
  p.bpp = rgb.fmt == UHDR_IMG_FMT_32bppRGBA8888 ? 4 : 3;
  for (int c = 0; c < 3; c++) { p.p[c] = (const uint8_t*)ycc.p[c]; p.stride[c] = ycc.stride[c]; }
  p.k_cr_g = variant ? FIX16(0.714136286) : FIX16(0.71414);
  p.k_cb_g = variant ? FIX16(0.344136286) : FIX16(0.34414);
  const bool vec = (p.w % 4 == 0) && al(p.rgb_out, p.bpp == 4 ? 16 : 4) && ((size_t)p.rgb_stride_px * p.bpp) % (p.bpp == 4 ? 16 : 4) == 0 &&
                   al(p.p[0], 4) && al(p.p[1], 4) && al(p.p[2], 4) && p.stride[0] % 4 == 0 && p.stride[1] % 4 == 0 && p.stride[2] % 4 == 0;
  const uint32_t per_row = vec ? p.w / 4 : p.w;
  const int grid = resident_grid(((per_row + kBlock - 1) / kBlock) * p.h, 8);
  if (p.bpp == 4) {
    if (vec) hipLaunchKernelGGL((jpeg_ycc_to_rgb_kernel<4, true>), dim3(grid), dim3(kBlock), 0, s, p);
    else hipLaunchKernelGGL((jpeg_ycc_to_rgb_kernel<4, false>), dim3(grid), dim3(kBlock), 0, s, p);
  } else {
    if (vec) hipLaunchKernelGGL((jpeg_ycc_to_rgb_kernel<3, true>), dim3(grid), dim3(kBlock), 0, s, p);
    else hipLaunchKernelGGL((jpeg_ycc_to_rgb_kernel<3, false>), dim3(grid), dim3(kBlock), 0, s, p);
  }
  return hipGetLastError();
}

}
```

libultrahdr_amd/csrc/uhdr_types.h:

```cpp
#pragma once
#include <hip/hip_runtime.h>
#include <stdint.h>

#include "device_math.h"
#include "uhdr_hip.h"

namespace uhdr {

struct ImageView {
  const void* p[3];
  uint32_t stride[3];
  uint32_t w, h;
  int fmt;
  int range;
};
struct ImageViewMut {
  void* p[3];
  uint32_t stride[3];
  uint32_t w, h;
  int fmt;
  int range;
};

constexpr int kSrgbN = 1024;
// ... 172 lines not shown
struct RgbToYcbcrParams {
  ImageView src;
  ImageViewMut dst;
  Rgb2Yuv k;
};

hipError_t launch_apply_gainmap(const ApplyParams& p, hipStream_t s);
hipError_t launch_apply_gainmap_coef(const ApplyParams& p, hipStream_t s);
int apply_quad_mode(const ApplyParams& p);
hipError_t launch_generate_gainmap(const GenParams& p, bool two_pass, hipStream_t s);
hipError_t launch_affine_map(const AffineParams& p, hipStream_t s);
hipError_t launch_minmax_table(const MinmaxTableParams& p, hipStream_t s);
hipError_t launch_map_blocks(const float* ratio, const AffineDev* dev, const double* math_tab, int nch, int bw, int bh, const uint16_t* qt_luma,
                             const uint16_t* qt_chroma, int16_t* const coef[3], uint8_t* map_out, uint32_t out_stride, hipStream_t s);
hipError_t launch_base_blocks(const ImageView& yuv420, const Mat3* c, const uint16_t* qt_luma, const uint16_t* qt_chroma, int16_t* const coef[3],
                              hipStream_t s);
hipError_t launch_selftest(int which, unsigned long long* out, uint32_t arg0, uint32_t arg1, uint32_t seed, const double* math_tab, const AffineDev* dev,
                           hipStream_t s);
int gen_partials_count(const GenParams& p);
hipError_t launch_encode_api0_fused(const FusedParams& p, bool two_pass, int* grid_out, hipStream_t s);
hipError_t launch_tone_map(const ToneMapParams& p, hipStream_t s);
hipError_t launch_transform_yuv(const YuvXformParams& p, hipStream_t s);
hipError_t launch_rgb_to_ycbcr(const RgbToYcbcrParams& p, hipStream_t s);
struct FdctEdge {
  int on, w, h, col_mode, fill, mcu_rows;
};
hipError_t launch_fdct_quant(const uint8_t* plane, size_t stride, int bw, int bh,
                             const uint16_t* qt_host, int16_t* coef, hipStream_t s, const FdctEdge* edge = nullptr);

hipError_t launch_fdct_quant_rgb(const uint8_t* rgb, size_t pitch, int bpp, int bw, int bh, const uint16_t* qt_luma_host,
                                 const uint16_t* qt_chroma_host, int16_t* coef_y, int16_t* coef_cb, int16_t* coef_cr, hipStream_t s, int vw = 0,
                                 int vh = 0);
hipError_t launch_repack(int mode, const void* src, size_t src_pitch, void* dst, size_t dst_pitch, uint32_t w, uint32_t h,
                         hipStream_t s);
struct EffectPlane {
  const void* src;
  void* dst;
  uint32_t elem;
  uint32_t src_w, src_h, src_stride;
  uint32_t dst_w, dst_h, dst_stride;
  uint32_t mode;
  uint32_t a0, a1;
};
hipError_t launch_effect_plane(const EffectPlane& p, hipStream_t s);

struct HuffArgs {
  const int16_t* coef[3];
  int bw[3], bh[3];
  int hs[3], vs[3];
  int ncomp;
  int mcus_per_row, total_mcus;
  int ri;
  int blocks_per_mcu;
  int nseg;
  const uint32_t* tables;
  const uint8_t* zigzag;
  uint8_t* slots;
  uint32_t slot_stride;
  uint32_t* seg_bytes;
};
uint32_t huff_slot_stride();
struct HuffStream {
  uint32_t* seg_bits;
  uint64_t* seg_start;
  uint32_t* raw;
  uint64_t raw_words;
  uint32_t* meta;
  uint32_t* slots;
};
int huff_stream_segment_mcus(int blocks_per_mcu);
size_t huff_stream_slot_bytes(int nseg);
int huff_stuff_chunks(uint64_t raw_bytes);
hipError_t launch_huffman_encode_stream(const HuffArgs& a, const HuffStream& t, uint32_t* chunk_counts, uint64_t* out_bytes, uint8_t* out, uint64_t cap,
                                        hipStream_t s);
hipError_t launch_huffman_encode(const HuffArgs& a, uint64_t* offsets, uint32_t* status, uint8_t* out, uint64_t cap, hipStream_t s);

struct HuffDecTable {
  uint16_t lut[512];
  int maxcode[18];
  int valoff[17];
  uint8_t vals[256];
};
struct HuffDecArgs {
  const uint8_t* data;
  uint32_t nbytes;
  const uint32_t* starts;
  const uint32_t* ends;
  int nseg, ri, total_mcus, mcus_per_row, ncomp;
  int bw[3], bh[3], hs[3], vs[3];
  int16_t* coef[3];
  const HuffDecTable* tabs;
  const uint8_t* zigzag;
  uint32_t* status;
};
constexpr int kHuffL2Max = 16;
struct HuffFastTable {
  uint16_t l1[512];
  uint16_t l2[kHuffL2Max][128];
};
constexpr int kHuffValWords = 512 + kHuffL2Max * 128;
constexpr int kHuffPairBits = 10, kHuffPairWords = 1 << kHuffPairBits;
constexpr int kHuffL2Total = 32;
constexpr int kHuffPairBlobWords = 4 * kHuffPairWords + kHuffL2Total * 128 / 2;
constexpr int kHuffPairValBlobWords = 8 * kHuffPairWords + kHuffL2Total * 128 / 2;
struct HuffSyncArgs {
  const uint8_t* clean;
  uint32_t nbytes;
  const uint32_t* nstuffed;
  uint32_t sub_bits;
  uint64_t* state[2];
  uint8_t* changed[2];
  uint32_t* nblk;
  uint32_t* scan_tmp;
  uint32_t* flags;
  int* dcd;
  uint32_t total_blocks;
  int blocks_per_mcu, ncomp, mcus_per_row;
  int bw[3], bh[3], hs[3], vs[3], first_blk[3];
  uint8_t comp_of[16];
  int16_t* coef[3];
  const HuffFastTable* ftabs;
  const HuffFastTable* ttabs;
  const uint32_t* vtabs;
  const uint32_t* ptabs;
  const uint32_t* pvtabs;
  const uint8_t* zigzag;
  int hyp_h, hyp_levels;
  uint64_t* hyp_state;
  uint8_t* hyp_map;
  uint16_t* hyp_cnt;
  int hyp_hist;
  int hyp_main_levels;
  int strag_levels;
  uint32_t* strag_list;
  uint32_t strag_cap;
  int16_t* coef_scan;
  uint4* zero_ptr;
  uint32_t zero_vec;
  int pieces;
  uint64_t* mid_state;
  uint16_t* mid_cnt;
  uint64_t* pend;
  uint32_t* pcnt;
  const uint32_t* rst_map;
  uint32_t rst_blocks;
  int* dc_seg;
  uint32_t* rst_partial;
  uint32_t rst_chunks;
};
constexpr int kHuffHypSlots = 48;
constexpr int kHuffFlagStragglers = 20;
constexpr int kHuffFlagStray = 21;
size_t huff_hyp_chain_bytes(uint64_t nbytes, uint32_t sub_bits, size_t* tiles_offset);
hipError_t launch_huffman_decode_hyp(const HuffSyncArgs& a, int* dc_partial, uint8_t* chain_prefix, uint8_t* chain_tiles, hipStream_t s);
int huff_sync_chunks(uint64_t nbytes);
uint32_t huff_sync_max_subsequences(uint64_t nbytes, uint32_t sub_bits);
struct HuffInitFill {
  uint4* zero_ptr;
  uint32_t zero_vec;
  uint4* ff_ptr;
  uint32_t ff_vec;
};
hipError_t launch_huffman_unstuff(const uint8_t* data, uint32_t nbytes, uint32_t* chunk_counts, uint32_t* nstuffed_dev, uint8_t* clean, hipStream_t s,
                                  uint32_t* rst_map, uint32_t* rst_partial, const HuffInitFill* fill = nullptr);
hipError_t launch_huffman_decode_sync(const HuffSyncArgs& a, int max_rounds, int* dc_partial, int* final_buf, hipStream_t s);
void launch_profile_mark(hipStream_t s);
int huff_marker_chunks(uint64_t nbytes);
int huff_place_chunk();
hipError_t launch_stray_marker_check(const uint8_t* data, uint32_t nbytes, uint32_t* flag, hipStream_t s);
hipError_t launch_huffman_decode(const HuffDecArgs& a, uint32_t* counts, uint32_t* starts, uint32_t* ends, hipStream_t s);

hipError_t launch_idct_dequant(const int16_t* coef, int bw, int bh, const uint16_t* qt_host, uint8_t* plane,
                               size_t stride, hipStream_t s);
hipError_t launch_idct_dequant_rgb(const int16_t* coef_y, const int16_t* coef_cb, const int16_t* coef_cr, int bw, int bh,
                                   const uint16_t* qt_luma_host, const uint16_t* qt_chroma_host, int variant,
                                   const ImageViewMut& rgb, hipStream_t s);
size_t upsample420_scratch_bytes(const int bw[3], const int bh[3]);
hipError_t launch_idct_upsample_rgb(const int16_t* const coef[3], const int bw[3], const int bh[3], const uint16_t* const qt_host[3],
                                    int variant, const ImageViewMut& rgb, uint8_t* chroma_scratch, hipStream_t s);
hipError_t launch_jpeg_rgb_to_ycc(const ImageView& rgb, const ImageViewMut& ycc, hipStream_t s);
hipError_t launch_jpeg_ycc_to_rgb(const ImageView& ycc, const ImageViewMut& rgb, int variant, hipStream_t s);

}
```

Before: 12110 Mpixels/s.

## Fuse gain-map coefficient placement with IDCT and color conversion; poll status early

```diff
diff --git a/libultrahdr_amd/csrc/api_context.cpp b/libultrahdr_amd/csrc/api_context.cpp
--- a/libultrahdr_amd/csrc/api_context.cpp
+++ b/libultrahdr_amd/csrc/api_context.cpp
@@ -616,6 +616,7 @@
   if (c->aux_ev2) (void)hipEventDestroy(c->aux_ev2);
   if (c->md_ev) (void)hipEventDestroy(c->md_ev);
   if (c->md_stream) (void)hipStreamDestroy(c->md_stream);
+  if (c->huff_ev) (void)hipEventDestroy(c->huff_ev);
   if (c->h_flags) (void)hipHostFree(c->h_flags);
   if (c->pin.p) (void)hipHostFree(c->pin.p);
   if (c->pin.ev) (void)hipEventDestroy(c->pin.ev);
diff --git a/libultrahdr_amd/csrc/api_entropy.cpp b/libultrahdr_amd/csrc/api_entropy.cpp
--- a/libultrahdr_amd/csrc/api_entropy.cpp
+++ b/libultrahdr_amd/csrc/api_entropy.cpp
@@ -54,6 +54,19 @@
     }
   }
   return hipStreamSynchronize(c->stream);
+}
+static hipError_t wait_side_stream(hipStream_t s) {
+  static const int spin_us = [] { const char* e = getenv("UHDR_HIP_SYNC_SPIN_US"); return e ? atoi(e) : 2000; }();
+  if (spin_us > 0) {
+    const auto t0 = std::chrono::steady_clock::now();
+    for (;;) {
+      const hipError_t q = hipStreamQuery(s);
+      if (q == hipSuccess) return hipSuccess;
+      if (q != hipErrorNotReady) return q;
+      if (std::chrono::steady_clock::now() - t0 > std::chrono::microseconds(spin_us)) break;
+    }
+  }
+  return hipStreamSynchronize(s);
 }
 
 
@@ -361,6 +374,7 @@
     HIP_TRY(hipMemcpyAsync(c->d_huff, blob.data(), blob.size() * sizeof(uint32_t), hipMemcpyHostToDevice, c->stream));
     HIP_TRY(hipStreamSynchronize(c->stream));
   }
+  c->huff_pix_taken = false;
   const DbgClock dbg;
   constexpr size_t kTabDec = 0, kTabFast = (sizeof(HuffDecTable) * 4 + 255) & ~(size_t)255,
                    kTabVal = (kTabFast + sizeof(HuffFastTable) * 8 + 255) & ~(size_t)255, kTabPair = kTabVal + (size_t)4 * kHuffValWords * 4,
@@ -503,11 +517,19 @@
     auto take = [&](size_t bytes) { const size_t o = off; off += (bytes + 255) & ~(size_t)255; return o; };
     const size_t rst_words = data_bytes / 32 + 2;
     const size_t o_clean = take(data_bytes + 16), o_cnt = take((size_t)nch * 4);
+    const int max_pieces = [&] {
+      const char* e = getenv("UHDR_HIP_HUFF_PIECES");
+      const int v = e ? atoi(e) : 4;
+      return (use_hyp && form2 && !rst_sync && v >= 1 && v <= 4) ? v : 1;
+    }();
     const size_t o_flags = take(128), o_nblk = take((size_t)nsub * 4 + 4), o_dcd = take((size_t)total_blocks * 4), o_rm = rst_sync ? take(rst_words * 4) : 0;
+    const size_t pc_bytes = ((size_t)nsub * (size_t)max_pieces + 4) * 4;
+    const size_t o_pc = max_pieces > 1 ? take(pc_bytes) : 0;
     const size_t zero_bytes_sync = off - o_flags;
     const size_t o_s0 = take((size_t)nsub * 8), o_hm = use_hyp ? take((size_t)nsub * kHuffHypSlots) : 0;
+    const size_t o_pe = max_pieces > 1 ? take((size_t)nsub * (size_t)max_pieces * 8 + 64) : 0;
     const size_t ff_bytes = off - o_s0;
-    const size_t o_s1 = take((size_t)nsub * 8), o_c0 = take(nsub), o_c1 = take(nsub), o_dcp = take((size_t)((total_blocks + 255) / 256) * 12 + 16),
+    const size_t o_s1 = take((size_t)nsub * 8), o_c0 = take(nsub), o_c1 = take(nsub), o_dcp = take((size_t)((total_blocks + kPlaceRgbChunk - 1) / kPlaceRgbChunk) * 12 + 16),
                  o_ft = take(sizeof(HuffFastTable) * 8),
                  o_st = take(((size_t)nsub / 2048 + 2) * 4), o_vt = take((size_t)4 * kHuffValWords * 4);
     const size_t o_hs = use_hyp ? take((size_t)nsub * kHuffHypSlots * 8) : 0, o_hc = use_hyp ? take((size_t)nsub * kHuffHypSlots * 2) : 0;
@@ -516,15 +538,8 @@
     (void)chain_tiles_off;
     const size_t o_ds = rst_sync ? take((size_t)a.nseg * 12) : 0, o_rp = rst_sync ? take((size_t)nch * 12) : 0;
     const size_t o_sl = use_hyp ? take((size_t)nsub * (size_t)bpm * 8) : 0;
-    const int max_pieces = [&] {
-      const char* e = getenv("UHDR_HIP_HUFF_PIECES");
-      const int v = e ? atoi(e) : 4;
-      return (use_hyp && form2 && !rst_sync && v >= 1 && v <= 4) ? v : 1;
-    }();
     const size_t o_ms = max_pieces > 1 ? take((size_t)nsub * kHuffHypSlots * (size_t)(max_pieces - 1) * 8) : 0;
     const size_t o_mc = max_pieces > 1 ? take((size_t)nsub * kHuffHypSlots * (size_t)(max_pieces - 1) * 2) : 0;
-    const size_t o_pe = max_pieces > 1 ? take((size_t)nsub * (size_t)max_pieces * 8 + 64) : 0;
-    const size_t o_pc = max_pieces > 1 ? take(((size_t)nsub * (size_t)max_pieces + 4) * 4) : 0;
     const size_t o_st2 = max_pieces > 1 ? take(((size_t)nsub * (size_t)max_pieces / 2048 + 4) * 4) : 0;
     const size_t scan_bytes = form2 ? (size_t)total_blocks * 64 * sizeof(int16_t) : 0;
     const size_t o_cs = form2 ? take(scan_bytes + 256) : 0;
@@ -588,6 +603,15 @@
       auto pass0_zeroes = [&](const Attempt& t) { return form2 && t.levels > 0 && scan_bytes % 16 == 0 && scan_bytes / 16 < 0xFFFFFFFFull; };
       if (form2 && !pass0_zeroes(attempts[0])) HIP_TRY(hipMemsetAsync(y.coef_scan, 0, scan_bytes, c->stream));
       dbg.mark("huffman_decode_dev: fills enqueued");
+      c->huff_pix_taken = false;
+      const bool pix_fits = c->huff_pix.rgb && form2 && a.ncomp == 3 && bpm == 3 && c->huff_pix.w == sc->w && c->huff_pix.h == sc->h;
+      const int staged_env = [] { const char* e = getenv("UHDR_HIP_DECODE_STAGED_MAP"); return e ? atoi(e) : 0; }();
+      bool early_status = form2 && (staged_env == 0 || staged_env == 2);
+      if (early_status) {
+        if (!c->md_stream && hipStreamCreateWithFlags(&c->md_stream, hipStreamNonBlocking) != hipSuccess) { c->md_stream = nullptr; early_status = false; }
+        if (early_status && !c->huff_ev && hipEventCreateWithFlags(&c->huff_ev, hipEventDisableTiming) != hipSuccess) { c->huff_ev = nullptr; early_status = false; }
+      }
+      bool tail_in_flight = false;
       int final_buf = 0;
       uint32_t* fl = c->h_flags;
       for (int q = 0; q < 24; q++) fl[q] = 0;
@@ -596,6 +620,7 @@
         HIP_TRY(hipMemsetAsync(y.flags, 0, 32, c->stream));
         HIP_TRY(hipMemsetAsync(y.flags + kHuffFlagStragglers, 0, 4, c->stream));
         HIP_TRY(hipMemsetAsync(y.nblk, 0, (size_t)nsub * 4 + 4, c->stream));
+        if (max_pieces > 1) HIP_TRY(hipMemsetAsync(sb + o_pc, 0, pc_bytes, c->stream));
         if (form2) {
           if (!pass0_zeroes(next)) HIP_TRY(hipMemsetAsync(y.coef_scan, 0, scan_bytes, c->stream));
         } else {
@@ -644,13 +669,22 @@
               HIP_TRY(launch_huffman_unstuff(data, (uint32_t)data_bytes, (uint32_t*)(sb + o_cnt), y.flags + 8, sb + o_clean, c->stream, rst_map, y.rst_partial,
                                              fills_in_unstuff && ti == 0 ? &init_fill : nullptr));
             unstuffed = true;
-            HIP_TRY(launch_huffman_decode_hyp(y, (int*)(sb + o_dcp), sb + o_ch, sb + o_ch + tiles_off, c->stream));
+            HIP_TRY(launch_huffman_decode_hyp(y, (int*)(sb + o_dcp), sb + o_ch, sb + o_ch + tiles_off, c->stream, pix_fits ? &c->huff_pix : nullptr,
+                                              early_status ? c->huff_ev : nullptr));
           }
           dbg.mark("huffman_decode_dev: hypothesis attempt enqueued");
-          HIP_TRY(hipMemcpyAsync(fl, y.flags, 24 * sizeof(uint32_t), hipMemcpyDeviceToHost, c->stream));
-          HIP_TRY(wait_stream(c));
+          if (early_status) {
+            HIP_TRY(hipStreamWaitEvent(c->md_stream, c->huff_ev, 0));
+            HIP_TRY(hipMemcpyAsync(fl, y.flags, 24 * sizeof(uint32_t), hipMemcpyDeviceToHost, c->md_stream));
+            HIP_TRY(wait_side_stream(c->md_stream));
+            tail_in_flight = true;
+          } else {
+            HIP_TRY(hipMemcpyAsync(fl, y.flags, 24 * sizeof(uint32_t), hipMemcpyDeviceToHost, c->stream));
+            HIP_TRY(wait_stream(c));
+          }
           dbg.mark("huffman_decode_dev: hypothesis attempt finished");
           hyp_done = fl[2] == 0;
+          c->huff_pix_taken = hyp_done && pix_fits;
           if (hyp_done && ti > 0) {
             uhdr_hip_ctx::HuffHint& hint = c->huff_hint[bpm & 15];
             hint.sub_bits = t.sub_bits;
@@ -676,8 +710,10 @@
           HIP_TRY(hipMemcpyAsync(fl, y.flags, 24 * sizeof(uint32_t), hipMemcpyDeviceToHost, c->stream));
           HIP_TRY(wait_stream(c));
           rounds_ran = true;
-        }
-      }
+          tail_in_flight = false;
+        }
+      }
+      if (tail_in_flight && !c->huff_async_tail) HIP_TRY(wait_stream(c));
       const bool settled = hyp_done || fl[4 + max_rounds % 3] == 0;
       if (rst_sync && getenv("UHDR_HIP_HUFF_DEBUG"))
         fprintf(stderr, "uhdr_hip: restart file through the parallel decoder: %s, status bits %#x, %u markers dropped (%d expected), sequence sums %s\n",
@@ -737,6 +773,8 @@
   c->aux->huff_serial_ok = c->huff_serial_ok;
   c->aux->huff_route_log = c->huff_route_log;
   c->aux->huff_two_pass = c->huff_two_pass;
+  c->aux->huff_pix = c->huff_pix;
+  c->aux->huff_async_tail = c->huff_async_tail;
   *out = c->aux;
   return ok_status();
 }
diff --git a/libultrahdr_amd/csrc/api_internal.h b/libultrahdr_amd/csrc/api_internal.h
--- a/libultrahdr_amd/csrc/api_internal.h
+++ b/libultrahdr_amd/csrc/api_internal.h
@@ -136,6 +136,10 @@
     hipEvent_t ev = nullptr;
     bool ev_pending = false;
   } pin;
+  HuffPixelSink huff_pix = {};
+  bool huff_pix_taken = false;
+  bool huff_async_tail = false;
+  hipEvent_t huff_ev = nullptr;
   uint32_t* h_flags = nullptr;
   bool resident_on = false;
   bool resident_lazy = false;
diff --git a/libultrahdr_amd/csrc/api_jpeg.cpp b/libultrahdr_amd/csrc/api_jpeg.cpp
--- a/libultrahdr_amd/csrc/api_jpeg.cpp
+++ b/libultrahdr_amd/csrc/api_jpeg.cpp
@@ -1164,8 +1164,33 @@
         if (h->tables.bits[t][l]) return &h->tables;
     return nullptr;
   };
+  const int staged_env = [] { const char* e = getenv("UHDR_HIP_DECODE_STAGED_MAP"); return e ? atoi(e) : 0; }();
+  const size_t pitch_px = ((size_t)sm.w + 63) & ~(size_t)63;
+  c->huff_pix = HuffPixelSink();
+  if (nm == 3 && (staged_env == 0 || staged_env == 3)) {
+    UHDR_TRY(ensure(c->jpg[4], pitch_px * 4 * sm.h));
+    c->huff_pix.rgb = (uint8_t*)c->jpg[4].p;
+    c->huff_pix.pitch = pitch_px * 4;
+    c->huff_pix.w = sm.w;
+    c->huff_pix.h = sm.h;
+    c->huff_pix.variant = libjpeg_variant;
+    memcpy(c->huff_pix.q[0], map->qtable[0], sizeof c->huff_pix.q[0]);
+    memcpy(c->huff_pix.q[1], map->qtable[1], sizeof c->huff_pix.q[1]);
+  }
+  c->huff_async_tail = true;
   const uhdr_error_info_t hs = uhdr_hip_huffman_decode2_dev(c, &sb, tables_of(base), base_data, base_bytes, &sm, tables_of(map), map_data, map_bytes);
   c->huff_serial_ok = true;
+  c->huff_async_tail = false;
+  c->huff_pix = HuffPixelSink();
+  const bool map_in_pixels = c->aux && c->aux->huff_pix_taken;
+  if (c->aux) {
+    c->aux->huff_pix = HuffPixelSink();
+    c->aux->huff_async_tail = false;
+    c->aux->huff_pix_taken = false;
+    if (!c->aux_ev2) HIP_TRY(hipEventCreateWithFlags(&c->aux_ev2, hipEventDisableTiming));
+    HIP_TRY(hipEventRecord(c->aux_ev2, c->aux->stream));
+    HIP_TRY(hipStreamWaitEvent(c->stream, c->aux_ev2, 0));
+  }
   if (hs.error_code != UHDR_CODEC_OK) return hs;
   uhdr_raw_image_t gm;
   memset(&gm, 0, sizeof gm);
@@ -1174,13 +1199,13 @@
   gm.range = UHDR_CR_FULL_RANGE;
   gm.w = sm.w;
   gm.h = sm.h;
-  const size_t pitch_px = ((size_t)sm.w + 63) & ~(size_t)63;
   if (nm == 3) {
     gm.fmt = UHDR_IMG_FMT_32bppRGBA8888;
     UHDR_TRY(ensure(c->jpg[4], pitch_px * 4 * sm.h));
     gm.planes[0] = c->jpg[4].p;
     gm.stride[0] = (unsigned int)pitch_px;
-    UHDR_TRY(uhdr_hip_idct_dequant_rgb_dev(c, sm.coef[0], sm.coef[1], sm.coef[2], sm.blocks_w[0], sm.blocks_h[0], map->qtable[0], map->qtable[1], libjpeg_variant, &gm));
+    if (!map_in_pixels)
+      UHDR_TRY(uhdr_hip_idct_dequant_rgb_dev(c, sm.coef[0], sm.coef[1], sm.coef[2], sm.blocks_w[0], sm.blocks_h[0], map->qtable[0], map->qtable[1], libjpeg_variant, &gm));
   } else {
     gm.fmt = UHDR_IMG_FMT_8bppYCbCr400;
     const size_t pitch = ((size_t)sm.blocks_w[0] * 8 + 63) & ~(size_t)63;
diff --git a/libultrahdr_amd/csrc/huffman_decode_sync.hip b/libultrahdr_amd/csrc/huffman_decode_sync.hip
--- a/libultrahdr_amd/csrc/huffman_decode_sync.hip
+++ b/libultrahdr_amd/csrc/huffman_decode_sync.hip
@@ -1378,6 +1378,19 @@
   dc_chunk_scan(v, s_sum, tid);
   if (tid == kPlaceChunk - 1) { partial[blockIdx.x * 3] = v[0]; partial[blockIdx.x * 3 + 1] = v[1]; partial[blockIdx.x * 3 + 2] = v[2]; }
 }
+static_assert(kPlaceRgbChunk <= kPlaceChunk && kPlaceRgbChunk % 3 == 0, "one thread per scan position of a chunk of whole MCUs");
+__global__ __launch_bounds__(kPlaceChunk) void dc_partial2_mcu_kernel(const HuffSyncArgs a, int* __restrict__ partial) {
+  __shared__ int s_sum[3 * (kPlaceChunk / 64)];
+  const int tid = (int)threadIdx.x;
+  const uint32_t t = blockIdx.x * (uint32_t)kPlaceRgbChunk + (uint32_t)tid;
+  int v[3] = {0, 0, 0};
+  if (tid < kPlaceRgbChunk && t < a.total_blocks) {
+    const int d = a.coef_scan[(size_t)t * 64], c = tid % 3;
+    v[0] = c == 0 ? d : 0; v[1] = c == 1 ? d : 0; v[2] = c == 2 ? d : 0;
+  }
+  dc_chunk_scan(v, s_sum, tid);
+  if (tid == kPlaceChunk - 1) { partial[blockIdx.x * 3] = v[0]; partial[blockIdx.x * 3 + 1] = v[1]; partial[blockIdx.x * 3 + 2] = v[2]; }
+}
 constexpr int kPlaceSelfPrefix = 4096;
 __global__ __launch_bounds__(kPlaceChunk) void coef_place_kernel(const HuffSyncArgs a, const int* __restrict__ partial, int self_prefix) {
   __shared__ int s_sum[3 * (kPlaceChunk / 64)];
@@ -1590,6 +1603,13 @@
   if (!self_prefix) hipLaunchKernelGGL(dc_scan_partials_kernel, dim3(1), dim3(1024), 0, s, dc_partial, nch);
   hipLaunchKernelGGL(coef_place_kernel, dim3(nch), dim3(kPlaceChunk), 0, s, a, (const int*)dc_partial, self_prefix);
 }
+static hipError_t launch_place_rgb(const HuffSyncArgs& a, const HuffPixelSink& px, int* dc_partial, hipStream_t s) {
+  const int nch = (int)((a.total_blocks + kPlaceRgbChunk - 1) / kPlaceRgbChunk);
+  hipLaunchKernelGGL(dc_partial2_mcu_kernel, dim3(nch), dim3(kPlaceChunk), 0, s, a, dc_partial);
+  const int self_prefix = nch <= kPlaceSelfPrefix ? 1 : 0;
+  if (!self_prefix) hipLaunchKernelGGL(dc_scan_partials_kernel, dim3(1), dim3(1024), 0, s, dc_partial, nch);
+  return launch_coef_place_rgb(a, px, dc_partial, self_prefix, s);
+}
 int huff_place_chunk() { return kPlaceChunk; }
 static void launch_dc(const HuffSyncArgs& a, int* dc_partial, hipStream_t s) {
   const int nch = (int)((a.total_blocks + 1023) / 1024);
@@ -1628,7 +1648,8 @@
   return pre + ntiles * kHuffHypSlots + ((ntiles + 255) & ~(size_t)255);
 }
 
-hipError_t launch_huffman_decode_hyp(const HuffSyncArgs& a, int* dc_partial, uint8_t* chain_prefix, uint8_t* chain_tiles, hipStream_t s) {
+hipError_t launch_huffman_decode_hyp(const HuffSyncArgs& a, int* dc_partial, uint8_t* chain_prefix, uint8_t* chain_tiles, hipStream_t s,
+                                     const HuffPixelSink* pix, hipEvent_t after_write) {
   const uint32_t nsub = huff_sync_max_subsequences(a.nbytes, a.sub_bits);
   const int grid = (int)((nsub + 63) / 64);
   const int threads = 64 * a.hyp_h;
@@ -1700,7 +1721,16 @@
   if (a.coef_scan && !a.rst_map) {
     launch_write2(w, nw, 0, s);
     mark();
-    launch_place(a, dc_partial, s);
+    if (after_write) {
+      const hipError_t e1 = hipEventRecord(after_write, s);
+      if (e1 != hipSuccess) return e1;
+    }
+    if (pix && pix->rgb) {
+      const hipError_t e1 = launch_place_rgb(a, *pix, dc_partial, s);
+      if (e1 != hipSuccess) return e1;
+    } else {
+      launch_place(a, dc_partial, s);
+    }
   } else {
     launch_write(a, nsub, 0, s);
     mark();
diff --git a/libultrahdr_amd/csrc/idct_core.h b/libultrahdr_amd/csrc/idct_core.h
--- a/libultrahdr_amd/csrc/idct_core.h
+++ b/libultrahdr_amd/csrc/idct_core.h
@@ -79,11 +79,9 @@
   }
 }
 
-__device__ __forceinline__ void idct_wave(int* ws, const int v[8], int big, int rr, int rb, uint32_t s[8]) {
+__device__ __forceinline__ void idct_wave_ws(int* ws, int big, int rr, int rb, uint32_t s[8]) {
   const int cb = rr, cc = rb;
   const bool fast = __builtin_amdgcn_ballot_w64(big != 0) == 0;
-#pragma unroll
-  for (int c = 0; c < 8; c++) ws[rb * 72 + rr * 9 + c] = v[c];
   __builtin_amdgcn_wave_barrier();
   __builtin_amdgcn_s_waitcnt(0xc07f);
   int in[8], out[8];
@@ -103,5 +101,17 @@
   __builtin_amdgcn_wave_barrier();
 }
 
+__device__ __forceinline__ void idct_wave(int* ws, const int v[8], int big, int rr, int rb, uint32_t s[8]) {
+#pragma unroll
+  for (int c = 0; c < 8; c++) ws[rb * 72 + rr * 9 + c] = v[c];
+  idct_wave_ws(ws, big, rr, rb, s);
+}
+
+__device__ __forceinline__ void idct_wave_zigzag(int* ws, const int v[8], const int at[8], int big, int rr, int rb, uint32_t s[8]) {
+#pragma unroll
+  for (int c = 0; c < 8; c++) ws[rb * 72 + at[c]] = v[c];
+  idct_wave_ws(ws, big, rr, rb, s);
+}
+
 }
 }
diff --git a/libultrahdr_amd/csrc/jpeg_decode.hip b/libultrahdr_amd/csrc/jpeg_decode.hip
--- a/libultrahdr_amd/csrc/jpeg_decode.hip
+++ b/libultrahdr_amd/csrc/jpeg_decode.hip
@@ -1,4 +1,5 @@
 #include "idct_core.h"
+#include "wg_scan.h"
 #include "uhdr_types.h"
 
 namespace uhdr {
@@ -221,6 +222,109 @@
             if constexpr (BPP == 4) dst[c * BPP + 3] = 255;
           }
         }
+      }
+    }
+  }
+}
+
+struct PlaceRgbArgs {
+  const int16_t* coef_scan;
+  const uint8_t* zigzag;
+  const int* partial;
+  uint8_t* rgb;
+  size_t pitch;
+  uint32_t w, h, total_mcus;
+  int mcus_per_row, bw, bh, self_prefix;
+  int k_cr_g, k_cb_g;
+  uint16_t q[2][64];
+};
+static_assert(kPlaceRgbChunk == 3 * 64 && kPlaceRgbChunk <= kBlock, "64 MCUs per workgroup: two units of eight for each of the four waves");
+
+__global__ __launch_bounds__(kBlock) void coef_place_rgb_kernel(const PlaceRgbArgs a) {
+  __shared__ int s_ws[kBlock / 64][8 * 8 * 9];
+  __shared__ int s_sum[3 * (kBlock / 64)];
+  __shared__ int16_t s_dc[kPlaceRgbChunk];
+  const int tid = (int)threadIdx.x, lane = tid & 63, wv = tid >> 6;
+  const int rr = lane >> 3, rb = lane & 7;
+  const uint32_t m0 = blockIdx.x * (uint32_t)(kPlaceRgbChunk / 3), t0 = m0 * 3u;
+  const int comp = tid % 3;
+  int v[3] = {0, 0, 0};
+  if (tid < kPlaceRgbChunk && (t0 + (uint32_t)tid) / 3u < a.total_mcus) {
+    const int d = a.coef_scan[(size_t)(t0 + (uint32_t)tid) * 64];
+    v[0] = comp == 0 ? d : 0; v[1] = comp == 1 ? d : 0; v[2] = comp == 2 ? d : 0;
+  }
+  int carry[3];
+  if (a.self_prefix) {
+    int part[3] = {0, 0, 0};
+    for (uint32_t i = (uint32_t)tid; i < blockIdx.x; i += (uint32_t)kBlock) {
+      part[0] += a.partial[i * 3];
+      part[1] += a.partial[i * 3 + 1];
+      part[2] += a.partial[i * 3 + 2];
+    }
+    wg_incl_scan<kBlock, 3>(part, s_sum, carry);
+  } else {
+    carry[0] = a.partial[blockIdx.x * 3];
+    carry[1] = a.partial[blockIdx.x * 3 + 1];
+    carry[2] = a.partial[blockIdx.x * 3 + 2];
+  }
+  int all[3];
+  wg_incl_scan<kBlock, 3>(v, s_sum, all);
+  if (tid < kPlaceRgbChunk) s_dc[tid] = (int16_t)(comp == 0 ? carry[0] + v[0] : (comp == 1 ? carry[1] + v[1] : carry[2] + v[2]));
+  int at[8], ql[8], qc[8];
+#pragma unroll
+  for (int c = 0; c < 8; c++) {
+    const int n = a.zigzag[rr * 8 + c];
+    at[c] = (n >> 3) * 9 + (n & 7);
+    ql[c] = a.q[0][n];
+    qc[c] = a.q[1][n];
+  }
+  const bool vec_ok = ((a.pitch | (uintptr_t)a.rgb) & 15) == 0;
+  int* ws = s_ws[wv];
+  __syncthreads();
+
+  for (int k = 0; k < 2; k++) {
+    const int u = wv * 2 + k;
+    const uint32_t m = m0 + (uint32_t)(u * 8 + rb);
+    const bool ok = m < a.total_mcus;
+    uint4 raw[3];
+#pragma unroll
+    for (int j = 0; j < 3; j++) raw[j] = ok ? *(const uint4*)(a.coef_scan + ((size_t)m * 3 + j) * 64 + rr * 8) : make_uint4(0, 0, 0, 0);
+    uint32_t s[3][8];
+#pragma unroll
+    for (int j = 0; j < 3; j++) {
+      const uint32_t w4[4] = {raw[j].x, raw[j].y, raw[j].z, raw[j].w};
+      int x[8], big = 0;
+#pragma unroll
+      for (int c = 0; c < 4; c++) {
+        int lo = (int)(int16_t)(w4[c] & 0xffff);
+        if (c == 0 && rr == 0) lo = s_dc[(u * 8 + rb) * 3 + j];
+        x[2 * c] = __mul24(lo, j ? qc[2 * c] : ql[2 * c]);
+        x[2 * c + 1] = __mul24((int)(int16_t)(w4[c] >> 16), j ? qc[2 * c + 1] : ql[2 * c + 1]);
+      }
+      const int mx = max(max(max(x[0], x[1]), max(x[2], x[3])), max(max(x[4], x[5]), max(x[6], x[7])));
+      const int mn = min(min(min(x[0], x[1]), min(x[2], x[3])), min(min(x[4], x[5]), min(x[6], x[7])));
+      big = (int)(mx > 8191) | (int)(mn < -8191);
+      if (!ok) {
+#pragma unroll
+        for (int c = 0; c < 8; c++) x[c] = 0;
+        big = 0;
+      }
+      idct_wave_zigzag(ws, x, at, big, rr, rb, s[j]);
+    }
+    const uint32_t my = m / (uint32_t)a.mcus_per_row, mxb = m - my * (uint32_t)a.mcus_per_row;
+    const uint32_t y = my * 8u + (uint32_t)rr, x0 = mxb * 8u;
+    if (ok && (int)my < a.bh && (int)mxb < a.bw && y < a.h && x0 < a.w) {
+      uint32_t px[8];
+#pragma unroll
+      for (int c = 0; c < 8; c++) px[c] = ycc_to_rgb_px(s[0][c], s[1][c], s[2][c], a.k_cr_g, a.k_cb_g);
+      uint8_t* dst = a.rgb + (size_t)y * a.pitch + (size_t)x0 * 4;
+      if (vec_ok && x0 + 8 <= a.w) {
+        *(uint4*)dst = make_uint4(px[0], px[1], px[2], px[3]);
+        *(uint4*)(dst + 16) = make_uint4(px[4], px[5], px[6], px[7]);
+      } else {
+#pragma unroll
+        for (int c = 0; c < 8; c++)
+          if (x0 + c < a.w) *(uint32_t*)(dst + c * 4) = px[c];
       }
     }
   }
@@ -267,6 +371,28 @@
   const int grid = resident_grid((uint32_t)(total + 3) / 4, 8);
   if (bpp == 4) hipLaunchKernelGGL((idct_dequant_rgb_kernel<4>), dim3(grid), dim3(kBlock), 0, s, a);
   else hipLaunchKernelGGL((idct_dequant_rgb_kernel<3>), dim3(grid), dim3(kBlock), 0, s, a);
+  return hipGetLastError();
+}
+
+hipError_t launch_coef_place_rgb(const HuffSyncArgs& h, const HuffPixelSink& px, const int* partial, int self_prefix, hipStream_t s) {
+  if (h.blocks_per_mcu != 3 || h.total_blocks % 3u || !h.coef_scan || !px.rgb || (px.pitch & 3) || ((uintptr_t)px.rgb & 3) || (size_t)px.w * 4 > px.pitch ||
+      px.w > (uint32_t)h.bw[0] * 8u || px.h > (uint32_t)h.bh[0] * 8u)
+    return hipErrorInvalidValue;
+  PlaceRgbArgs a = {};
+  a.coef_scan = h.coef_scan;
+  a.zigzag = h.zigzag;
+  a.partial = partial;
+  a.rgb = px.rgb;
+  a.pitch = px.pitch;
+  a.w = px.w; a.h = px.h;
+  a.total_mcus = h.total_blocks / 3u;
+  a.mcus_per_row = h.mcus_per_row; a.bw = h.bw[0]; a.bh = h.bh[0];
+  a.self_prefix = self_prefix;
+  a.k_cr_g = px.variant ? FIX16(0.714136286) : FIX16(0.71414);
+  a.k_cb_g = px.variant ? FIX16(0.344136286) : FIX16(0.34414);
+  for (int i = 0; i < 64; i++) { a.q[0][i] = px.q[0][i]; a.q[1][i] = px.q[1][i]; }
+  const int nch = (int)((h.total_blocks + kPlaceRgbChunk - 1) / kPlaceRgbChunk);
+  hipLaunchKernelGGL(coef_place_rgb_kernel, dim3(nch), dim3(kBlock), 0, s, a);
   return hipGetLastError();
 }
 
diff --git a/libultrahdr_amd/csrc/uhdr_types.h b/libultrahdr_amd/csrc/uhdr_types.h
--- a/libultrahdr_amd/csrc/uhdr_types.h
+++ b/libultrahdr_amd/csrc/uhdr_types.h
@@ -348,7 +348,17 @@
 constexpr int kHuffFlagStragglers = 20;
 constexpr int kHuffFlagStray = 21;
 size_t huff_hyp_chain_bytes(uint64_t nbytes, uint32_t sub_bits, size_t* tiles_offset);
-hipError_t launch_huffman_decode_hyp(const HuffSyncArgs& a, int* dc_partial, uint8_t* chain_prefix, uint8_t* chain_tiles, hipStream_t s);
+constexpr int kPlaceRgbChunk = 192;
+struct HuffPixelSink {
+  uint8_t* rgb;
+  size_t pitch;
+  uint32_t w, h;
+  int variant;
+  uint16_t q[2][64];
+};
+hipError_t launch_coef_place_rgb(const HuffSyncArgs& a, const HuffPixelSink& px, const int* partial, int self_prefix, hipStream_t s);
+hipError_t launch_huffman_decode_hyp(const HuffSyncArgs& a, int* dc_partial, uint8_t* chain_prefix, uint8_t* chain_tiles, hipStream_t s,
+                                     const HuffPixelSink* pix = nullptr, hipEvent_t after_write = nullptr);
 int huff_sync_chunks(uint64_t nbytes);
 uint32_t huff_sync_max_subsequences(uint64_t nbytes, uint32_t sub_bits);
 struct HuffInitFill {
```

Measured after the change: 12240 Mpixels/s (median of 5 runs). Within noise of the previous version (+1.1%).
